# AtharvBhat/otters

Measured on AMD Instinct MI355X. Metric: GB/s scanned + queries/sec, exact cosine top-10 over 10M x 768 f32 rows per GPU, higher is better.
Workload: dtype f32; 1 GPU; 10000000x768 f32 VecStore per GPU, single query, Metric::Cosine, take(10); rows_per_gpu=10000000, dim=768, k=10, nq=1, processes=1

## Files before the change

bindings/rust/otters-hip-sys/src/lib.rs:

```rust
#![allow(non_camel_case_types)]

use std::os::raw::{c_char, c_int, c_void};

pub const OTT_ABI_VERSION: c_int = 4;
pub const OTT_COMM_ID_BYTES: usize = 128;
pub const OTT_GROUP_SIZE_MAX: u32 = 16;
pub const OTT_MAXSIM_BATCH_MAX: u32 = 4096;
pub const OTT_MMR_MAX_FETCH: u32 = 1024;
pub const OTT_RECOMMEND_MAX_EXAMPLES: u32 = 64;
pub const OTT_DISCOVER_MAX_PAIRS: u32 = 32;
pub const OTT_NO_ROW: u64 = u64::MAX;
pub const OTT_NO_MASK: u32 = 4294967295;
pub const OTT_MASK_SLOT_BASE: u32 = 2147483648;
pub const OTT_MASK_SLOTS: u32 = 64;
pub const OTT_MASKS_MAX_QUERIES: u32 = 1024;
pub const OTT_BOOST_MAX_TERMS: u32 = 8;
pub const OTT_BOOST_MAX_QUERIES: u32 = 1024;
pub const OTT_FUSE_MAX_LEGS: u32 = 16;
pub const OTT_FUSE_MAX_FETCH: u32 = 512;
pub const OTT_FUSE_MAX_ENTRIES: u32 = 8192;
pub const OTT_FUSE_MAX_REQUESTS: u32 = 1024;
pub const OTT_FUSE_RRF: u32 = 0;
pub const OTT_FUSE_DBSF: u32 = 1;
pub const OTT_FUSE_MINMAX: u32 = 2;
// ... 81 lines not shown
    pub vectors_compared: u64,
    pub prune_ns: u64,
    pub score_ns: u64,
    pub merge_ns: u64,
    pub total_ns: u64,
    pub bytes_scanned: u64,
    pub path_used: u32,
    pub passes: u32,
    pub rescored: u64,
    pub retries: u32,
    pub refined: u32,
    pub err_ratio_max: f32,
    pub gate_failed: u32,
    pub bound_violations: u32,
    pub i8_refined: u32,
    pub exchange_ns: u64,
}

#[repr(C)]
#[derive(Clone, Copy, Debug)]
pub struct ott_leaf {
    pub column: u32,
    pub op: u32,
    pub clause: u32,
    pub reserved: u32,
    pub lit_i64: i64,
    pub lit_f64: f64,
}

#[repr(C)]
#[derive(Clone, Copy, Debug)]
pub struct ott_boost_term {
    pub kind: u32,
    pub source: u32,
    pub weight: f32,
    pub scale: f32,
    pub origin: f64,
    pub missing: f32,
    pub reserved: u32,
}

#[repr(C)]
pub struct ott_store {
    _opaque: [u8; 0],
}

#[repr(C)]
pub struct ott_comm {
    _opaque: [u8; 0],
}

pub type ott_allgather_fn = Option<unsafe extern "C" fn(user: *mut c_void, send: *const c_void, recv: *mut c_void, bytes: u64) -> c_int>;

extern "C" {
    pub fn ott_abi_version() -> c_int;
    pub fn ott_last_error() -> *const c_char;
    pub fn ott_device_count(out: *mut c_int) -> c_int;

    pub fn ott_store_create(dim: u32, device: c_int, out: *mut *mut ott_store) -> c_int;
    pub fn ott_store_create_multi(dim: u32, n_dev: u32, dev_ids: *const c_int, out: *mut *mut ott_store) -> c_int;
    pub fn ott_multi_plan(n_rows: u64, chunk_size: u64, n_dev: u32, out_first_rows: *mut u64) -> c_int;
    pub fn ott_store_shard_count(s: *const ott_store) -> c_int;
    pub fn ott_store_shard_info(s: *const ott_store, shard: u32, device: *mut c_int, first_row: *mut u64, n_rows: *mut u64) -> c_int;
    pub fn ott_store_transport(s: *const ott_store) -> *const c_char;
    pub fn ott_store_destroy(s: *mut ott_store) -> c_int;
    pub fn ott_store_reserve(s: *mut ott_store, n_rows: u64) -> c_int;
    pub fn ott_store_append(s: *mut ott_store, rows_host: *const f32, n_rows: u64) -> c_int;
    pub fn ott_store_append_device(s: *mut ott_store, rows_dev: *const c_void, n_rows: u64) -> c_int;
    pub fn ott_store_append_random(s: *mut ott_store, n_rows: u64, seed: u64) -> c_int;
    pub fn ott_store_append_clustered(s: *mut ott_store, n_rows: u64, seed: u64, n_clusters: u32, spread: f32, aniso: f32) -> c_int;
    pub fn ott_store_write_rows(s: *mut ott_store, first_row: u64, rows_host: *const f32, n_rows: u64) -> c_int;
    pub fn ott_store_len(s: *const ott_store) -> u64;
    pub fn ott_store_delete_rows(s: *mut ott_store, rows_host: *const u64, n: u64, n_changed: *mut u64) -> c_int;
    pub fn ott_store_restore_rows(s: *mut ott_store, rows_host: *const u64, n: u64, n_changed: *mut u64) -> c_int;
    pub fn ott_store_live_len(s: *const ott_store) -> u64;
    pub fn ott_store_read_live_mask(s: *const ott_store, out_host: *mut u64) -> c_int;
    pub fn ott_store_compact(s: *mut ott_store, out_new_index: *mut u64) -> c_int;
    pub fn ott_store_dim(s: *const ott_store) -> u32;
    pub fn ott_store_device(s: *const ott_store) -> c_int;
    pub fn ott_store_set_chunk_size(s: *mut ott_store, chunk_size: u64) -> c_int;
    pub fn ott_store_set_batch_image(s: *mut ott_store, enabled: c_int) -> c_int;
    pub fn ott_store_prepare_batch(s: *mut ott_store) -> c_int;
    pub fn ott_store_batch_ready(s: *const ott_store) -> c_int;
    pub fn ott_store_set_option(s: *mut ott_store, name: *const c_char, value: i64) -> c_int;
    pub fn ott_store_set_base_offset(s: *mut ott_store, base: u64) -> c_int;
    pub fn ott_store_set_reduce_order(s: *mut ott_store, reduce: u32) -> c_int;
    pub fn ott_store_read_rows(s: *const ott_store, first_row: u64, n_rows: u64, out_host: *mut f32) -> c_int;
    pub fn ott_store_read_inv_norms(s: *const ott_store, first_row: u64, n_rows: u64, out_host: *mut f32) -> c_int;
    pub fn ott_store_add_column(s: *mut ott_store, dtype: u32, values_host: *const c_void, nulls: *const u64, n: u64, out_column_id: *mut u32) -> c_int;
    pub fn ott_store_zone_stats(s: *mut ott_store, column: u32, chunk_size: u64, out_min: *mut c_void, out_max: *mut c_void, out_non_null: *mut u64) -> c_int;
    pub fn ott_store_eval_row_mask(s: *mut ott_store, leaves: *const ott_leaf, n_leaves: u32, n_clauses: u32, out_host: *mut u64) -> c_int;

    pub fn ott_query(s: *mut ott_store, d: *const ott_query_desc, out: *mut ott_hit, cap: u64, n_out: *mut u64, n_per_query: *mut u64, stats: *mut ott_stats) -> c_int;
    pub fn ott_query_masks(s: *mut ott_store, d: *const ott_query_desc, masks: *const u64, n_masks: u32, mask_bits: u64, mask_of_query: *const c_void, out: *mut ott_hit, cap: u64, n_out: *mut u64, n_per_query: *mut u64, stats: *mut ott_stats) -> c_int;
    pub fn ott_store_eval_row_mask_slot(s: *mut ott_store, slot: u32, leaves: *const ott_leaf, n_leaves: u32, n_clauses: u32, out_host: *mut u64) -> c_int;
    pub fn ott_store_write_row_mask_slot(s: *mut ott_store, slot: u32, bits: *const u64, n_bits: u64) -> c_int;
    pub fn ott_store_clear_row_mask_slots(s: *mut ott_store) -> c_int;
    pub fn ott_query_boost(s: *mut ott_store, d: *const ott_query_desc, combine: u32, score_weight: f32, terms: *const c_void, n_terms: u32, out: *mut ott_hit, cap: u64, n_out: *mut u64, n_per_query: *mut u64, stats: *mut ott_stats) -> c_int;
    pub fn ott_query_ids(s: *mut ott_store, d: *const ott_query_desc, ids: *const u64, n_ids: u64, out: *mut ott_hit, cap: u64, n_out: *mut u64, n_per_query: *mut u64, stats: *mut ott_stats) -> c_int;
    pub fn ott_store_score_rows(s: *mut ott_store, queries: *const f32, nq: u32, metric: u32, ids: *const u64, n_ids: u64, out_scores: *mut f32) -> c_int;
    pub fn ott_query_fuse(s: *mut ott_store, d: *const ott_query_desc, legs_per_request: *const c_void, n_requests: u32, fusion: u32, rrf_k: f32, leg_weights: *const f32, fetch: u64, out: *mut ott_hit, cap: u64, n_out: *mut u64, n_per_request: *mut u64, stats: *mut ott_stats) -> c_int;
    pub fn ott_store_set_sparse(s: *mut ott_store, indptr: *const u64, indices: *const c_void, values: *const f32, n: u64, vocab: u32) -> c_int;
    pub fn ott_store_clear_sparse(s: *mut ott_store) -> c_int;
    pub fn ott_store_sparse_info(s: *const ott_store, vocab: *mut u32, nnz: *mut u64, padded_entries: *mut u64, bytes: *mut u64) -> c_int;
    pub fn ott_store_read_sparse(s: *const ott_store, first_row: u64, n_rows: u64, indptr_out: *mut u64, indices_out: *mut c_void, values_out: *mut f32, entry_cap: u64) -> c_int;
    pub fn ott_query_sparse(s: *mut ott_store, d: *const ott_query_desc, q_indptr: *const u64, q_indices: *const c_void, q_values: *const f32, out: *mut ott_hit, cap: u64, n_out: *mut u64, n_per_query: *mut u64, stats: *mut ott_stats) -> c_int;
    pub fn ott_query_mmr(s: *mut ott_store, d: *const ott_query_desc, ids: *const u64, n_ids: u64, fetch_k: u64, lambda: f32, out: *mut ott_hit, cap: u64, n_out: *mut u64, n_per_query: *mut u64, out_values: *mut f32, stats: *mut ott_stats) -> c_int;
    pub fn ott_query_recommend(s: *mut ott_store, d: *const ott_query_desc, positive: *const u64, n_positive: u64, negative: *const u64, n_negative: u64, flags: u32, out: *mut ott_hit, cap: u64, n_out: *mut u64, side_of_hit: *mut u32, stats: *mut ott_stats) -> c_int;
    pub fn ott_query_recommend_strategy(s: *mut ott_store, d: *const ott_query_desc, strategy: u32, positive: *const u64, n_positive: u64, negative: *const u64, n_negative: u64, flags: u32, out: *mut ott_hit, cap: u64, n_out: *mut u64, side_of_hit: *mut u32, stats: *mut ott_stats) -> c_int;
    pub fn ott_query_discover(s: *mut ott_store, d: *const ott_query_desc, target_row: u64, positive: *const u64, negative: *const u64, n_pairs: u64, min_wins: u32, flags: u32, out: *mut ott_hit, cap: u64, n_out: *mut u64, wins_of_hit: *mut u32, stats: *mut ott_stats) -> c_int;
    pub fn ott_store_set_groups(s: *mut ott_store, gid_host: *const c_void, n: u64, n_groups: u32) -> c_int;
    pub fn ott_store_clear_groups(s: *mut ott_store) -> c_int;
    pub fn ott_store_group_count(s: *const ott_store) -> u32;
    pub fn ott_query_groups(s: *mut ott_store, d: *const ott_query_desc, out: *mut ott_hit, cap: u64, n_out: *mut u64, n_per_query: *mut u64, stats: *mut ott_stats) -> c_int;
    pub fn ott_query_groups_top(s: *mut ott_store, d: *const ott_query_desc, group_size: u32, out: *mut ott_hit, cap: u64, n_out: *mut u64, n_per_query: *mut u64, group_of_hit: *mut u32, stats: *mut ott_stats) -> c_int;
    pub fn ott_query_maxsim(s: *mut ott_store, d: *const ott_query_desc, out: *mut ott_hit, cap: u64, n_out: *mut u64, stats: *mut ott_stats) -> c_int;
    pub fn ott_query_maxsim_groups(s: *mut ott_store, d: *const ott_query_desc, groups: *const c_void, n_groups_listed: u64, out: *mut ott_hit, cap: u64, n_out: *mut u64, stats: *mut ott_stats) -> c_int;
    pub fn ott_store_group_index_builds(s: *const ott_store) -> u64;
    pub fn ott_query_maxsim_groups_batch(s: *mut ott_store, d: *const ott_query_desc, tokens_per_query: *const c_void, listed_per_query: *const u64, n_queries: u32, groups: *const c_void, out: *mut ott_hit, cap: u64, n_out: *mut u64, n_per_query: *mut u64, stats: *mut ott_stats) -> c_int;
    pub fn ott_query_device(s: *mut ott_store, d: *const ott_query_desc, out_dev: *mut c_void, cap: u64, n_out_dev: *mut c_void, stats: *mut ott_stats) -> c_int;
    pub fn ott_store_sync(s: *mut ott_store) -> c_int;
    pub fn ott_store_stream(s: *mut ott_store) -> *mut c_void;
    pub fn ott_merge_hits_device(s: *mut ott_store, lists_dev: *const c_void, n_lists: u64, list_len: u64, take: u32, k: u64, out_host: *mut ott_hit, n_out: *mut u64) -> c_int;
    pub fn ott_merge_hits_device_grouped(s: *mut ott_store, lists_dev: *const c_void, n_lists: u64, n_groups: u64, list_len: u64, take: u32, k: u64, out_host: *mut ott_hit, n_out: *mut u64, n_per_group: *mut u64) -> c_int;

    pub fn ott_comm_unique_id(id_out: *mut c_void) -> c_int;
    pub fn ott_comm_create(unique_id: *const c_void, rank: c_int, world: c_int, device: c_int, out: *mut *mut ott_comm) -> c_int;
    pub fn ott_comm_create_host(rank: c_int, world: c_int, r#fn: ott_allgather_fn, user: *mut c_void, out: *mut *mut ott_comm) -> c_int;
    pub fn ott_comm_destroy(c: *mut ott_comm) -> c_int;
    pub fn ott_comm_rank(c: *const ott_comm) -> c_int;
    pub fn ott_comm_world(c: *const ott_comm) -> c_int;
    pub fn ott_comm_transport(c: *const ott_comm) -> *const c_char;
    pub fn ott_comm_info(c: *const ott_comm, nranks: *mut c_int, version: *mut c_int) -> c_int;
    pub fn ott_comm_set_timeout_ms(c: *mut ott_comm, timeout_ms: i64) -> c_int;
    pub fn ott_comm_all_gather_host(c: *mut ott_comm, send_host: *const c_void, recv_host: *mut c_void, bytes: u64) -> c_int;
    pub fn ott_query_sharded(s: *mut ott_store, c: *mut ott_comm, d: *const ott_query_desc, out: *mut ott_hit, cap: u64, n_out: *mut u64, n_per_query: *mut u64, stats: *mut ott_stats) -> c_int;
}

pub fn last_error() -> String {
    unsafe {
        let p = ott_last_error();
        if p.is_null() {
            String::new()
        } else {
            std::ffi::CStr::from_ptr(p).to_string_lossy().into_owned()
        }
    }
}

pub fn check(rc: c_int) -> Result<(), String> {
    if rc == OTT_OK {
        Ok(())
    } else {
        Err(last_error())
    }
}

const _: () = {
    assert!(std::mem::size_of::<ott_hit>() == 16);
    assert!(std::mem::size_of::<ott_query_desc>() == 72);
    assert!(std::mem::size_of::<ott_stats>() == 120);
    assert!(std::mem::size_of::<ott_leaf>() == 32);
    assert!(std::mem::size_of::<ott_boost_term>() == 32);
};

#[cfg(test)]
// ... 9 lines not shown
```

include/otters_hip.h:

```cpp
#ifndef OTTERS_HIP_H
#define OTTERS_HIP_H

#include <stddef.h>
#include <stdint.h>

#ifdef __cplusplus
extern "C" {
#endif

#define OTT_ABI_VERSION 4

typedef enum {
    OTT_OK = 0,
    OTT_ERR_INVALID = -1,
    OTT_ERR_HIP = -2,
    OTT_ERR_OOM = -3,
    OTT_ERR_UNSUPPORTED = -4
} ott_status;

typedef enum { OTT_METRIC_COSINE = 0, OTT_METRIC_EUCLIDEAN = 1, OTT_METRIC_DOT = 2, OTT_METRIC_MANHATTAN = 3 } ott_metric;
typedef enum { OTT_TAKE_MIN = 0, OTT_TAKE_MAX = 1 } ott_take;
typedef enum { OTT_CMP_NONE = 0, OTT_CMP_LT = 1, OTT_CMP_GT = 2, OTT_CMP_LTE = 3, OTT_CMP_GTE = 4, OTT_CMP_EQ = 5 } ott_cmp;
typedef enum { OTT_OP_EQ = 0, OTT_OP_NEQ = 1, OTT_OP_LT = 2, OTT_OP_LTE = 3, OTT_OP_GT = 4, OTT_OP_GTE = 5 } ott_op;
typedef enum { OTT_DT_INT32 = 0, OTT_DT_INT64 = 1, OTT_DT_FLOAT32 = 2, OTT_DT_FLOAT64 = 3, OTT_DT_DATETIME = 5 } ott_dtype;
// ... 2 lines not shown

typedef enum { OTT_PATH_AUTO = 0, OTT_PATH_EXACT = 1, OTT_PATH_MFMA = 2 } ott_path;

typedef enum { OTT_REDUCE_AVX = 0, OTT_REDUCE_SEQ4 = 1 } ott_reduce;

typedef struct {
    uint64_t index;
    float score;
    uint32_t query;
} ott_hit;

typedef struct {
    const float* queries;
    uint32_t nq;
    uint32_t metric;
    uint32_t take;
    uint32_t filter_cmp;
    float filter_thr;
    uint32_t mode;
    uint64_t k;
    const uint64_t* chunk_mask;
    const uint64_t* row_mask;
    uint64_t row_mask_bits;
    uint32_t use_device_row_mask;
    uint32_t path;
} ott_query_desc;

typedef struct {
    uint64_t total_chunks, pruned_chunks, evaluated_chunks, vectors_compared;
    uint64_t prune_ns, score_ns, merge_ns, total_ns;
    uint64_t bytes_scanned;
    uint32_t path_used;
    uint32_t passes;
    uint64_t rescored;
    uint32_t retries;
    uint32_t refined;
    float err_ratio_max;
    uint32_t gate_failed;
    uint32_t bound_violations;
    uint32_t i8_refined;
    uint64_t exchange_ns;
} ott_stats;

typedef struct {
    uint32_t column;
    uint32_t op;
    uint32_t clause;
    uint32_t reserved;
    int64_t lit_i64;
    double lit_f64;
} ott_leaf;

typedef struct ott_store ott_store;

int ott_abi_version(void);
const char* ott_last_error(void);
int ott_device_count(int* out);

int ott_store_create(uint32_t dim, int device, ott_store** out);
int ott_store_create_multi(uint32_t dim, uint32_t n_dev, const int* dev_ids, ott_store** out);
int ott_multi_plan(uint64_t n_rows, uint64_t chunk_size, uint32_t n_dev, uint64_t* out_first_rows);
int ott_store_shard_count(const ott_store* s);
int ott_store_shard_info(const ott_store* s, uint32_t shard, int* device, uint64_t* first_row, uint64_t* n_rows);
const char* ott_store_transport(const ott_store* s);
int ott_store_destroy(ott_store* s);
int ott_store_reserve(ott_store* s, uint64_t n_rows);
int ott_store_append(ott_store* s, const float* rows_host, uint64_t n_rows);
int ott_store_append_device(ott_store* s, const void* rows_dev, uint64_t n_rows);
int ott_store_append_random(ott_store* s, uint64_t n_rows, uint64_t seed);
int ott_store_append_clustered(ott_store* s, uint64_t n_rows, uint64_t seed, uint32_t n_clusters, float spread, float aniso);
int ott_store_write_rows(ott_store* s, uint64_t first_row, const float* rows_host, uint64_t n_rows);
uint64_t ott_store_len(const ott_store* s);
uint32_t ott_store_dim(const ott_store* s);
int ott_store_device(const ott_store* s);
int ott_store_delete_rows(ott_store* s, const uint64_t* rows_host, uint64_t n, uint64_t* n_changed);
int ott_store_restore_rows(ott_store* s, const uint64_t* rows_host, uint64_t n, uint64_t* n_changed);
uint64_t ott_store_live_len(const ott_store* s);
int ott_store_read_live_mask(const ott_store* s, uint64_t* out_host);
int ott_store_compact(ott_store* s, uint64_t* out_new_index);
int ott_store_set_chunk_size(ott_store* s, uint64_t chunk_size);
int ott_store_set_batch_image(ott_store* s, int enabled);
int ott_store_prepare_batch(ott_store* s);
int ott_store_batch_ready(const ott_store* s);

int ott_store_set_option(ott_store* s, const char* name, int64_t value);

int ott_store_set_base_offset(ott_store* s, uint64_t base);
int ott_store_set_reduce_order(ott_store* s, uint32_t reduce );
int ott_store_read_rows(const ott_store* s, uint64_t first_row, uint64_t n_rows, float* out_host);
int ott_store_read_inv_norms(const ott_store* s, uint64_t first_row, uint64_t n_rows, float* out_host);

int ott_store_add_column(ott_store* s, uint32_t dtype, const void* values_host, const uint64_t* nulls,
                         uint64_t n, uint32_t* out_column_id);
int ott_store_zone_stats(ott_store* s, uint32_t column, uint64_t chunk_size, void* out_min, void* out_max,
                         uint64_t* out_non_null);

int ott_store_eval_row_mask(ott_store* s, const ott_leaf* leaves, uint32_t n_leaves, uint32_t n_clauses,
                            uint64_t* out_host);

int ott_query(ott_store* s, const ott_query_desc* d, ott_hit* out, uint64_t cap, uint64_t* n_out,
              uint64_t* n_per_query, ott_stats* stats);

int ott_query_ids(ott_store* s, const ott_query_desc* d, const uint64_t* ids, uint64_t n_ids, ott_hit* out, uint64_t cap,
                  uint64_t* n_out, uint64_t* n_per_query, ott_stats* stats);
int ott_store_score_rows(ott_store* s, const float* queries, uint32_t nq, uint32_t metric, const uint64_t* ids, uint64_t n_ids,
                         float* out_scores);

#define OTT_NO_MASK 4294967295u
#define OTT_MASK_SLOT_BASE 2147483648u
#define OTT_MASK_SLOTS 64
#define OTT_MASKS_MAX_QUERIES 1024
int ott_query_masks(ott_store* s, const ott_query_desc* d, const uint64_t* masks, uint32_t n_masks, uint64_t mask_bits,
                    const void* mask_of_query , ott_hit* out, uint64_t cap, uint64_t* n_out, uint64_t* n_per_query,
                    ott_stats* stats);
int ott_store_eval_row_mask_slot(ott_store* s, uint32_t slot, const ott_leaf* leaves, uint32_t n_leaves, uint32_t n_clauses,
                                 uint64_t* out_host);
int ott_store_write_row_mask_slot(ott_store* s, uint32_t slot, const uint64_t* bits, uint64_t n_bits);
int ott_store_clear_row_mask_slots(ott_store* s);

#define OTT_BOOST_MAX_TERMS 8
#define OTT_BOOST_MAX_QUERIES 1024
typedef enum { OTT_BOOST_SUM = 0, OTT_BOOST_MULT = 1 } ott_boost_combine;
typedef enum { OTT_BOOST_VALUE = 0, OTT_BOOST_LIN_DECAY = 1, OTT_BOOST_MASK = 2 } ott_boost_kind;
typedef struct {
    uint32_t kind;
    uint32_t source;
    float    weight;
    float    scale;
    double   origin;
    float    missing;
    uint32_t reserved;
} ott_boost_term;
int ott_query_boost(ott_store* s, const ott_query_desc* d, uint32_t combine, float score_weight,
                    const void* terms , uint32_t n_terms,
                    ott_hit* out, uint64_t cap, uint64_t* n_out, uint64_t* n_per_query, ott_stats* stats);

typedef enum { OTT_FUSE_RRF = 0, OTT_FUSE_DBSF = 1, OTT_FUSE_MINMAX = 2 } ott_fusion;
#define OTT_FUSE_MAX_LEGS 16
#define OTT_FUSE_MAX_FETCH 512
#define OTT_FUSE_MAX_ENTRIES 8192
#define OTT_FUSE_MAX_REQUESTS 1024
int ott_query_fuse(ott_store* s, const ott_query_desc* d, const void* legs_per_request , uint32_t n_requests,
                   uint32_t fusion , float rrf_k, const float* leg_weights , uint64_t fetch,
                   ott_hit* out, uint64_t cap, uint64_t* n_out, uint64_t* n_per_request, ott_stats* stats);

#define OTT_MMR_MAX_FETCH 1024
int ott_query_mmr(ott_store* s, const ott_query_desc* d, const uint64_t* ids, uint64_t n_ids,
                  uint64_t fetch_k, float lambda, ott_hit* out, uint64_t cap, uint64_t* n_out, uint64_t* n_per_query,
                  float* out_values , ott_stats* stats);

#define OTT_RECOMMEND_MAX_EXAMPLES 64
#define OTT_RECOMMEND_FILL 1u
int ott_query_recommend(ott_store* s, const ott_query_desc* d, const uint64_t* positive, uint64_t n_positive, const uint64_t* negative,
                        uint64_t n_negative, uint32_t flags, ott_hit* out, uint64_t cap, uint64_t* n_out,
                        uint32_t* side_of_hit , ott_stats* stats);

typedef enum { OTT_RECOMMEND_BEST_SCORE = 0, OTT_RECOMMEND_AVERAGE_VECTOR = 1, OTT_RECOMMEND_SUM_SCORES = 2 } ott_recommend_strategy;
int ott_query_recommend_strategy(ott_store* s, const ott_query_desc* d, uint32_t strategy, const uint64_t* positive,
                                 uint64_t n_positive, const uint64_t* negative, uint64_t n_negative, uint32_t flags, ott_hit* out,
                                 uint64_t cap, uint64_t* n_out, uint32_t* side_of_hit , ott_stats* stats);

#define OTT_DISCOVER_MAX_PAIRS 32
#define OTT_NO_ROW UINT64_MAX
int ott_query_discover(ott_store* s, const ott_query_desc* d, uint64_t target_row, const uint64_t* positive, const uint64_t* negative,
                       uint64_t n_pairs, uint32_t min_wins, uint32_t flags, ott_hit* out, uint64_t cap, uint64_t* n_out,
                       uint32_t* wins_of_hit , ott_stats* stats);
// ... 68 lines not shown
```

otters_amd/_native.py:

```python
from __future__ import annotations

import ctypes as C
import os
import subprocess

import numpy as np

_CSRC = os.path.join(os.path.dirname(os.path.abspath(__file__)), "csrc")
LIB_PATH = os.environ.get("OTT_LIB_PATH") or os.path.join(_CSRC, "libotters_hip.so")


class OttersError(Exception):
    """Error type of the host layer: str(e) is the reference's `Err(String)` payload."""


class Hit(C.Structure):
    _fields_ = [("index", C.c_uint64), ("score", C.c_float), ("query", C.c_uint32)]


HIT_DTYPE = np.dtype([("index", "<u8"), ("score", "<f4"), ("query", "<u4")])


class QueryDesc(C.Structure):
    _fields_ = [
# ... 42 lines not shown
FUSE_MAX_LEGS = 16
FUSE_MAX_FETCH = 512
FUSE_MAX_ENTRIES = 8192
FUSE_MAX_REQUESTS = 1024
FUSE_RRF, FUSE_DBSF, FUSE_MINMAX = 0, 1, 2
SPARSE_MAX_VOCAB = 1 << 20
SPARSE_MAX_QUERIES = 1024

_lib = None


def build(force: bool = False) -> str:
    srcs = [os.path.join(_CSRC, f) for f in os.listdir(_CSRC) if f.endswith((".hip", ".h", ".inc"))]
    srcs.append(os.path.join(_CSRC, "..", "..", "include", "otters_hip.h"))
    stale = not os.path.exists(LIB_PATH) or any(os.path.getmtime(s) > os.path.getmtime(LIB_PATH) for s in srcs)
    if force or stale:
        subprocess.check_call(["make", "-C", _CSRC, "-j", "8", "-s"])
    return LIB_PATH


def _preload_torch_hip() -> None:
    try:
        import importlib.util
        spec = importlib.util.find_spec("torch")
        if spec is None or not spec.submodule_search_locations:
            return
        libdir = os.path.join(list(spec.submodule_search_locations)[0], "lib")
        cand = os.path.join(libdir, "libamdhip64.so")
        if os.path.exists(cand):
            C.CDLL(cand, mode=C.RTLD_GLOBAL)
    except Exception:
        pass


def preload_torch_rccl() -> None:
    try:
        import torch
    except Exception:
        pass


def lib() -> C.CDLL:
    global _lib
    if _lib is not None:
        return _lib
    if not os.path.exists(LIB_PATH):
        raise OttersError(
            f"libotters_hip.so not found at {LIB_PATH}: build it with `python -c 'import __graft_entry__ as g; g.build()'` "
            "(there is no CPU fallback)")
    _preload_torch_hip()
    L = C.CDLL(LIB_PATH)
    vp, u64, u32, i32 = C.c_void_p, C.c_uint64, C.c_uint32, C.c_int
    sig = {
        "ott_abi_version": (i32, []),
        "ott_last_error": (C.c_char_p, []),
        "ott_device_count": (i32, [vp]),
        "ott_store_create": (i32, [u32, i32, vp]),
        "ott_store_create_multi": (i32, [u32, u32, vp, vp]),
        "ott_multi_plan": (i32, [u64, u64, u32, vp]),
        "ott_store_shard_count": (i32, [vp]),
        "ott_store_shard_info": (i32, [vp, u32, vp, vp, vp]),
        "ott_store_transport": (C.c_char_p, [vp]),
        "ott_store_destroy": (i32, [vp]),
        "ott_store_reserve": (i32, [vp, u64]),
        "ott_store_append": (i32, [vp, vp, u64]),
        "ott_store_append_device": (i32, [vp, vp, u64]),
        "ott_store_append_random": (i32, [vp, u64, u64]),
        "ott_store_append_clustered": (i32, [vp, u64, u64, u32, C.c_float, C.c_float]),
        "ott_store_write_rows": (i32, [vp, u64, vp, u64]),
        "ott_store_delete_rows": (i32, [vp, vp, u64, vp]),
        "ott_store_restore_rows": (i32, [vp, vp, u64, vp]),
        "ott_store_live_len": (u64, [vp]),
        "ott_store_read_live_mask": (i32, [vp, vp]),
        "ott_store_compact": (i32, [vp, vp]),
        "ott_store_len": (u64, [vp]),
        "ott_store_dim": (u32, [vp]),
        "ott_store_device": (i32, [vp]),
        "ott_store_set_chunk_size": (i32, [vp, u64]),
        "ott_store_set_base_offset": (i32, [vp, u64]),
        "ott_store_set_reduce_order": (i32, [vp, u32]),
        "ott_store_set_batch_image": (i32, [vp, i32]),
        "ott_store_prepare_batch": (i32, [vp]),
        "ott_store_batch_ready": (i32, [vp]),
        "ott_store_read_rows": (i32, [vp, u64, u64, vp]),
        "ott_store_read_inv_norms": (i32, [vp, u64, u64, vp]),
        "ott_store_add_column": (i32, [vp, u32, vp, vp, u64, vp]),
        "ott_store_eval_row_mask": (i32, [vp, vp, u32, u32, vp]),
        "ott_store_zone_stats": (i32, [vp, u32, u64, vp, vp, vp]),
        "ott_query": (i32, [vp, vp, vp, u64, vp, vp, vp]),
        "ott_query_ids": (i32, [vp, vp, vp, u64, vp, u64, vp, vp, vp]),
        "ott_store_score_rows": (i32, [vp, vp, u32, u32, vp, u64, vp]),
        "ott_query_masks": (i32, [vp, vp, vp, u32, u64, vp, vp, u64, vp, vp, vp]),
        "ott_store_eval_row_mask_slot": (i32, [vp, u32, vp, u32, u32, vp]),
        "ott_store_write_row_mask_slot": (i32, [vp, u32, vp, u64]),
        "ott_store_clear_row_mask_slots": (i32, [vp]),
        "ott_query_boost": (i32, [vp, vp, u32, C.c_float, vp, u32, vp, u64, vp, vp, vp]),
        "ott_query_fuse": (i32, [vp, vp, vp, u32, u32, C.c_float, vp, u64, vp, u64, vp, vp, vp]),
        "ott_query_mmr": (i32, [vp, vp, vp, u64, u64, C.c_float, vp, u64, vp, vp, vp, vp]),
        "ott_query_recommend": (i32, [vp, vp, vp, u64, vp, u64, u32, vp, u64, vp, vp, vp]),
        "ott_query_recommend_strategy": (i32, [vp, vp, u32, vp, u64, vp, u64, u32, vp, u64, vp, vp, vp]),
        "ott_query_discover": (i32, [vp, vp, u64, vp, vp, u64, u32, u32, vp, u64, vp, vp, vp]),
        "ott_store_set_groups": (i32, [vp, vp, u64, u32]),
        "ott_store_clear_groups": (i32, [vp]),
        "ott_store_group_count": (u32, [vp]),
        "ott_query_groups": (i32, [vp, vp, vp, u64, vp, vp, vp]),
        "ott_query_groups_top": (i32, [vp, vp, u32, vp, u64, vp, vp, vp, vp]),
        "ott_query_maxsim": (i32, [vp, vp, vp, u64, vp, vp]),
        "ott_query_maxsim_groups": (i32, [vp, vp, vp, u64, vp, u64, vp, vp]),
        "ott_store_group_index_builds": (u64, [vp]),
        "ott_query_maxsim_groups_batch": (i32, [vp, vp, vp, vp, u32, vp, vp, u64, vp, vp, vp]),
        "ott_query_device": (i32, [vp, vp, vp, u64, vp, vp]),
        "ott_store_sync": (i32, [vp]),
        "ott_store_stream": (vp, [vp]),
        "ott_merge_hits_device": (i32, [vp, vp, u64, u64, u32, u64, vp, vp]),
        "ott_merge_hits_device_grouped": (i32, [vp, vp, u64, u64, u64, u32, u64, vp, vp, vp]),
        "ott_store_set_option": (i32, [vp, C.c_char_p, C.c_int64]),
        "ott_comm_unique_id": (i32, [vp]),
        "ott_comm_create": (i32, [vp, i32, i32, i32, vp]),
        "ott_comm_create_host": (i32, [i32, i32, ALLGATHER_FN, vp, vp]),
        "ott_comm_destroy": (i32, [vp]),
        "ott_comm_rank": (i32, [vp]),
        "ott_comm_world": (i32, [vp]),
        "ott_comm_transport": (C.c_char_p, [vp]),
        "ott_comm_info": (i32, [vp, vp, vp]),
        "ott_comm_set_timeout_ms": (i32, [vp, C.c_int64]),
        "ott_comm_all_gather_host": (i32, [vp, vp, vp, u64]),
        "ott_query_sharded": (i32, [vp, vp, vp, vp, u64, vp, vp, vp]),
        "ott_store_set_sparse": (i32, [vp, vp, vp, vp, u64, u32]),
        "ott_store_clear_sparse": (i32, [vp]),
        "ott_store_sparse_info": (i32, [vp, vp, vp, vp, vp]),
        "ott_store_read_sparse": (i32, [vp, u64, u64, vp, vp, vp, u64]),
        "ott_query_sparse": (i32, [vp, vp, vp, vp, vp, vp, u64, vp, vp, vp]),
    }
    for name, (res, args) in sig.items():
        fn = getattr(L, name)
        fn.restype = res
        fn.argtypes = args
    if L.ott_abi_version() != ABI_VERSION:
        raise OttersError("libotters_hip.so ABI version mismatch")
    _lib = L
    return L


def check(rc: int) -> None:
    if rc != 0:
        msg = lib().ott_last_error()
        err = OttersError(msg.decode("utf-8", "replace") if msg else f"libotters_hip error {rc}")
        err.status = int(rc)
        raise err


def ptr(a):
    return None if a is None else a.ctypes.data_as(C.c_void_p)


def pack_bits(bools) -> np.ndarray:
    b = np.ascontiguousarray(bools, dtype=bool).ravel()
    n = b.size
    nwords = max((n + 63) // 64, 1)
    buf = np.zeros(nwords * 8, dtype=np.uint8)
    if n:
        by = np.packbits(b, bitorder="little")
        buf[: by.size] = by
    return buf.view("<u8")


# ... 3 lines not shown
```

otters_amd/csrc/ott_api.hip:

```cpp
#include <math.h>
#include <string.h>

#include <algorithm>

#include "ott_internal.h"
#include "ott_prune.h"

using namespace ott;

namespace ott {

float host_inv_norm_exact(const float* v, uint32_t dim) {
    volatile float s = 0.0f;
    for (uint32_t i = 0; i < dim; i++) {
        volatile float sq = v[i] * v[i];
        s = s + sq;
    }
    float norm = sqrtf(s);
    return norm != 0.0f ? 1.0f / norm : 0.0f;
}

std::vector<uint32_t> tile_prefix(const RunPlan& pl, uint32_t tile_rows) {
    std::vector<uint32_t> pre;
    pre.push_back(0);
    uint64_t tiles = 0;
    for (const auto& r : pl.runs) {
        tiles += (r.count + tile_rows - 1) / tile_rows;
        pre.push_back((uint32_t)tiles);
    }
    return pre;
}

}


namespace ott {

int upload_exact_inputs(ott_store* s, const float* queries, uint32_t nq, const RunPlan& pl, const std::vector<uint32_t>& prefix) {
    const uint32_t nq_pad = (nq + 7u) & ~7u;
    const size_t q_bytes = (size_t)nq_pad * s->dimq * 4, qi_bytes = (size_t)nq_pad * 4;
    const size_t run_bytes = pl.runs.size() * sizeof(ott_run), pre_bytes = prefix.size() * 4;
    size_t off_q = 0, off_qi = off_q + q_bytes, off_run = (off_qi + qi_bytes + 15) & ~(size_t)15;
    size_t off_pre = off_run + run_bytes, total = off_pre + pre_bytes;
    int rc = s->h_stage.ensure(total);
    if (rc) return rc;
    char* hs = (char*)s->h_stage.p;
    float* hq = (float*)(hs + off_q);
    memset(hq, 0, q_bytes + qi_bytes);
    for (uint32_t i = 0; queries != nullptr && i < nq; i++) {
        memcpy(hq + (size_t)i * s->dimq, queries + (size_t)i * s->dim, (size_t)s->dim * 4);
        ((float*)(hs + off_qi))[i] = host_inv_norm_exact(queries + (size_t)i * s->dim, s->dim);
    }
    memcpy(hs + off_run, pl.runs.data(), run_bytes);
    memcpy(hs + off_pre, prefix.data(), pre_bytes);
    if ((rc = s->d_queries.ensure(total))) return rc;
    OTT_HIP(hipMemcpyAsync(s->d_queries.p, hs, total, hipMemcpyHostToDevice, s->stream));
    s->in_off_qinv = off_qi;
    s->in_off_runs = off_run;
    s->in_off_prefix = off_pre;
    return OTT_OK;
}

void fill_exact_params(ott_store* s, const ott_query_desc* d, const RunPlan& pl, uint32_t nq, const uint64_t* d_mask, uint64_t mask_bits,
                       uint32_t n_tiles, ExactParams& p) {
    memset(&p, 0, sizeof(p));
    p.rows = s->d_rows;
    p.inv = s->d_inv;
    p.queries = (const float*)s->d_queries.p;
    p.qinv = (const float*)((const char*)s->d_queries.p + s->in_off_qinv);
    p.row_mask = d_mask;
    p.row_mask_bits = mask_bits;
    p.runs = (const ott_run*)((const char*)s->d_queries.p + s->in_off_runs);
    p.tile_prefix = (const uint32_t*)((const char*)s->d_queries.p + s->in_off_prefix);
    p.ld = s->ld;
    p.dim = s->dim;
    p.dimq = s->dimq;
    p.n_runs = (uint32_t)pl.runs.size();
    p.n_tiles = n_tiles;
    p.nq_total = nq;
    p.metric = d->metric;
    p.take_max = d->take == OTT_TAKE_MAX;
    p.cmp = d->filter_cmp;
    p.thr = d->filter_thr;
    p.reduce = s->reduce;
    p.tie_sh = s->cur_tie_sh;
    p.tie_off = s->cur_tie_off;
    p.flat = s->cur_flat ? 1u : 0u;
}

// ... 31 lines not shown
        if (keep) {
            const uint64_t start = c * cs;
            const uint64_t len = (n - start) < cs ? (n - start) : cs;
            if (open) pl.runs.back().count += len;
            else pl.runs.push_back({start, len});
            open = true;
            pl.evaluated++;
            pl.rows_scored += len;
        } else {
            open = false;
        }
    }
}

}

namespace ott {
void make_run_plan(const ott_store* s, const uint64_t* chunk_mask, RunPlan& pl) { build_plan(s, chunk_mask, pl); }

int check_desc_enums(const char* who, const ott_query_desc* d) {
    const auto unknown = [who](const char* what) { return fail(OTT_ERR_INVALID, std::string(who) + ": unknown " + what); };
    if (d->metric > OTT_METRIC_MANHATTAN) return unknown("metric");
    if (d->take > OTT_TAKE_MAX) return unknown("take type");
    if (d->filter_cmp > OTT_CMP_EQ) return unknown("filter comparator");
    if (d->mode > OTT_MODE_PER_QUERY) return unknown("mode");
    if (d->path > OTT_PATH_MFMA) return unknown("path");
    return OTT_OK;
}

int check_device_row_mask(const char* who, const ott_store* s, const ott_query_desc* d) {
    if (d->use_device_row_mask && s->evalmask_bits == 0 && s->n)
        return fail(OTT_ERR_INVALID, std::string(who) + ": use_device_row_mask set but ott_store_eval_row_mask was not called");
    return OTT_OK;
}

int validate_query(const ott_store* s, const ott_query_desc* d) {
    int rc;
    if (!s) return fail(OTT_ERR_INVALID, "ott_query: store is NULL");
    if (!d) return fail(OTT_ERR_INVALID, "ott_query: desc is NULL");
    if (d->nq == 0) return fail(OTT_ERR_INVALID, "No queries provided");
    if (!d->queries) return fail(OTT_ERR_INVALID, "ott_query: queries is NULL");
    if ((rc = check_desc_enums("ott_query", d))) return rc;
    if (d->path == OTT_PATH_MFMA && d->metric == OTT_METRIC_MANHATTAN)
        return fail(OTT_ERR_UNSUPPORTED, "ott_query: the MFMA path does not score the Manhattan metric; use path AUTO or EXACT");
    return check_device_row_mask("ott_query", s, d);
}

void read_exact_events(ott_store* s, ott_stats* st) {
    float ms = 0.f;
    if (hipEventElapsedTime(&ms, s->ev[3], s->ev[4]) == hipSuccess) st->score_ns = (uint64_t)(ms * 1e6);
    if (hipEventElapsedTime(&ms, s->ev[4], s->ev[5]) == hipSuccess) st->merge_ns = (uint64_t)(ms * 1e6);
}
}

namespace {

__global__ void sum_counts_kernel(const uint64_t* counts, uint32_t n, uint64_t* out) {
    uint64_t t = 0;
    for (uint32_t i = threadIdx.x; i < n; i += 64) t += counts[i];
    for (int o = 32; o > 0; o >>= 1) t += __shfl_xor(t, o);
    if (threadIdx.x == 0) *out = t;
}

struct ExactCtx {
    ott_store* s;
    const float* queries;
    uint32_t nq;
    const ott_query_desc* d;
    bool perq;
    const RunPlan& pl;
    uint64_t k_eff;
    bool fetch, timing;
    const std::vector<uint32_t>& prefix;
    ExactPlan x;
    uint32_t groups;
    PrunePlan prune{0, false, 0};
    RunPlan plA, plB;
    std::vector<uint32_t> preA, preB;
    int gridA = 0, gridB = 0;
    double qt = 0.0, qn = 0.0, q1 = 0.0;
    PruneQuant qq{0, 0.0f, 0.0f, 0.0, 0};
    bool head = false;
    bool seed_est = false;
    ExactResult res{0, 0, 0};
    uint64_t* d_counts = nullptr;
    ott_hit* d_hits = nullptr;
    ExactParams p;
};

void plan_pruned_sweep(ExactCtx& c) {
    ott_store* s = c.s;
    const PruneIn in{s->dim, s->ld, c.d->metric, c.perq, c.x.lean, s->cur_flat, c.x.variant, s->opt.exact_prune, s->opt.exact_sketch,
                     SketchState{s->d_sketch != nullptr, s->sk_n >= s->n, s->sk_bits, s->sk_words, s->sk_stage0}, c.pl.rows_scored, c.x.E};
    PrunePlan pp = prune_plan(in);
    bool quant_ok = false;
    if (prune_plan_needs_quant(in, pp) && !(quant_ok = prune_query_quant(c.queries, s->dim, pp.c * 32, &c.qq))) pp = prune_plan_quant_refused(in);
    if (!pp.c) return;
#ifdef OTT_SK4_DECODE_F32
    const bool head = false;
#else
    const bool head = prune_plan_head(in, pp, quant_ok, HeadState{s->d_head != nullptr, s->head_n >= s->n, s->opt.exact_sketch_head});
#endif
    const uint32_t m = head ? 0u : pp.c * 32;
    if (head) (void)prune_query_quant(c.queries, s->dim, 0, &c.qq);
    const uint64_t est_rows = prune_plan_seed_est(in, pp, head, c.d->filter_cmp != OTT_CMP_NONE);
    split_plan(c.pl, est_rows ? est_rows : pp.seed, c.plA, c.plB);
    const bool two_runs_each = c.plA.runs.size() <= 2 && c.plB.runs.size() <= 2 && c.plB.rows_scored > 0;
    if (!two_runs_each || !prune_query_bounds(c.queries, s->dim, m, &c.qt, &c.qn)) return;
    c.prune = pp;
    c.head = head;
    c.seed_est = est_rows != 0;
    if (c.seed_est) c.plB = c.pl;
    c.q1 = prune_query_l1(c.queries, s->dim, m);
    c.preA = tile_prefix(c.plA, 64);
    c.preB = tile_prefix(c.plB, 64);
    c.gridA = exact_grid(s, c.preA.back());
    c.gridB = exact_grid(s, c.preB.back());
}

int ensure_exact_result(ExactCtx& c) {
    ott_store* s = c.s;
    int rc;
    if (!c.x.lean && (rc = upload_exact_inputs(s, c.queries, c.nq, c.pl, c.prefix))) return rc;
    const size_t n_lists_total = exact_n_lists(c.x, c.nq, c.perq, c.prune.c != 0, c.gridA, c.gridB);
    if ((rc = s->d_lists.ensure(n_lists_total * c.x.KS * sizeof(Cand)))) return rc;
    c.res = exact_result_layout(c.groups, c.x.KS);
    char* res_dev = nullptr;
    if (c.fetch) {
        if ((rc = s->h_hits.ensure(c.res.host_bytes))) return rc;
        void* mapped = nullptr;
        OTT_HIP(hipHostGetDevicePointer(&mapped, s->h_hits.p, 0));
        res_dev = (char*)mapped;
    } else {
        if ((rc = s->d_hits.ensure(c.res.bytes))) return rc;
        res_dev = (char*)s->d_hits.p;
    }
    c.d_counts = (uint64_t*)res_dev;
    c.d_hits = (ott_hit*)(res_dev + c.res.cnt_pad);
    return OTT_OK;
}

void fill_exact_call(ExactCtx& c, const uint64_t* d_mask, uint64_t mask_bits) {
    ott_store* s = c.s;
    fill_exact_params(s, c.d, c.pl, c.nq, d_mask, mask_bits, c.prefix.back(), c.p);
    c.p.k = (uint32_t)c.k_eff;
    c.p.perq = c.perq;
    c.p.list_stride = c.x.KS;
    c.p.small = c.x.variant;
    if (c.x.lean) embed_exact_inputs(c.p, c.queries, (size_t)s->dim * 4, host_inv_norm_exact(c.queries, s->dim), c.pl, c.prefix);
}

ExactParams part_params(const ExactCtx& c, const RunPlan& sub, const std::vector<uint32_t>& pre, Cand* dst) {
    ExactParams q = c.p;
    q.n_runs = (uint32_t)sub.runs.size();
    q.n_tiles = pre.back();
    embed_exact_inputs(q, c.queries, (size_t)c.s->dim * 4, c.p.eqinv, sub, pre);
    q.lists = dst;
    return q;
}

int pruned_sweep(ExactCtx& c) {
    ott_store* s = c.s;
    const uint32_t KS = c.x.KS;
    int rc;
    if ((rc = s->d_prune.ensure(64 + (size_t)KS * sizeof(ott_hit)))) return rc;
    uint64_t* seed_res = (uint64_t*)s->d_prune.p;
    unsigned long long* tails_dev = nullptr;
    if (c.fetch) {
        if (!s->d_tails.p) {
            if ((rc = s->d_tails.ensure(8))) return rc;
            OTT_HIP(hipMemsetAsync(s->d_tails.p, 0, 8, s->stream));
            s->tails_seen = 0;
        }
        tails_dev = (unsigned long long*)s->d_tails.p;
    }
    ExactParams pa = part_params(c, c.plA, c.preA, (Cand*)s->d_lists.p);
    auto sketch_inputs = [&](ExactParams& q) {
        q.prune_stage = c.prune.c;
        q.prune_qt = c.qt;
        q.prune_qn = c.qn;
        if (!c.prune.sketch) return;
        q.prune_sketch = s->d_sketch;
        q.sk_pitch = s->sk_pitch;
        q.sk_stage0 = s->sk_stage0;
        q.sk_bits = s->sk_bits;
        q.prune_q1 = c.q1;
        q.prune_qe1 = c.qq.qe1;
        q.prune_qscale = c.qq.scale;
        q.prune_qinv_scale = c.qq.inv_scale;
        q.prune_qsum = c.qq.qsum;
        if (c.head) {
            q.prune_head_codes = reinterpret_cast<const uint32_t*>(s->d_head);
            q.prune_head_rho = reinterpret_cast<const float*>(s->d_head + s->cap * (size_t)16);
        }
    };
    if (c.seed_est) {
        sketch_inputs(pa);
        pa.seed_est = 1;
        pa.seed_keep = prune_seed_keep(c.k_eff);
    }
    if ((rc = launch_exact(s, pa, 1, c.x.E, c.gridA))) return rc;
    if ((rc = launch_merge(s, (const Cand*)s->d_lists.p, (uint32_t)c.gridA, KS, 0, 1, (uint32_t)c.k_eff, c.x.E, c.p.take_max != 0, tie_base(s),
                           (ott_hit*)(seed_res + 8), KS, seed_res, s->cur_tie_sh)))
        return rc;
    ExactParams pb = part_params(c, c.plB, c.preB, (Cand*)s->d_lists.p + (size_t)c.gridA * KS);
    sketch_inputs(pb);
    pb.prune_seed = seed_res;
    pb.prune_tails = tails_dev;
    return launch_exact(s, pb, 1, c.x.E, c.gridB);
}

int plain_passes(ExactCtx& c) {
    ott_store* s = c.s;
    const uint32_t tile = c.x.tile;
    int rc;
    for (uint32_t ps = 0; ps < c.x.passes; ps++) {
        c.p.q0 = ps * tile;
        c.p.lists = (Cand*)s->d_lists.p + ((c.perq && tile > 1) ? 0 : (size_t)ps * c.x.grid * c.x.KS);
        if ((rc = launch_exact(s, c.p, (int)tile, c.x.E, c.x.grid))) return rc;
    }
    return OTT_OK;
}

int merge_exact(ExactCtx& c) {
    ott_store* s = c.s;
    const uint32_t KS = c.x.KS, grid = (uint32_t)c.x.grid;
    if (c.seed_est)
        return launch_merge(s, (const Cand*)s->d_lists.p + (size_t)c.gridA * KS, (uint32_t)c.gridB, KS, 0, c.groups, (uint32_t)c.k_eff, c.x.E,
                            c.p.take_max != 0, tie_base(s), c.d_hits, KS, c.d_counts, s->cur_tie_sh);
    const uint32_t n_lists = c.perq ? grid : (uint32_t)exact_n_lists(c.x, c.nq, false, c.prune.c != 0, c.gridA, c.gridB);
    return launch_merge(s, (const Cand*)s->d_lists.p, n_lists, KS, c.perq ? (uint64_t)grid * KS : 0, c.groups, (uint32_t)c.k_eff, c.x.E,
                        c.p.take_max != 0, tie_base(s), c.d_hits, KS, c.d_counts, s->cur_tie_sh);
}

int fetch_exact(ExactCtx& c, std::vector<std::vector<ott_hit>>& lists, ott_stats& st) {
    ott_store* s = c.s;
    const uint32_t KS = c.x.KS;
    char* hh = (char*)s->h_hits.p;
    if (c.prune.c) OTT_HIP(hipMemcpyAsync(hh + c.res.bytes, s->d_tails.p, 8, hipMemcpyDeviceToHost, s->stream));
    OTT_HIP(hipStreamSynchronize(s->stream));
    if (c.prune.c) {
        uint64_t total;
        memcpy(&total, hh + c.res.bytes, 8);
        st.rescored += total - s->tails_seen;
        s->tails_seen = total;
    }
    const uint64_t* counts = (const uint64_t*)hh;
    const ott_hit* hits = (const ott_hit*)(hh + c.res.cnt_pad);
    lists.assign(c.groups, {});
    for (uint32_t g = 0; g < c.groups; g++) lists[g].assign(hits + (size_t)g * KS, hits + (size_t)g * KS + counts[g]);
    float ms = 0.f;
    if (c.timing && hipEventElapsedTime(&ms, s->ev[3], s->ev[4]) == hipSuccess) st.score_ns += (uint64_t)(ms * 1e6);
    if (c.timing && hipEventElapsedTime(&ms, s->ev[4], s->ev[5]) == hipSuccess) st.merge_ns += (uint64_t)(ms * 1e6);
    return OTT_OK;
}

int run_exact(ott_store* s, const float* queries, uint32_t nq, const ott_query_desc* d, bool perq, const RunPlan& pl, uint64_t k_eff,
              const uint64_t* d_mask, uint64_t mask_bits, bool fetch, std::vector<std::vector<ott_hit>>& lists, ott_stats& st,
              bool timing = true, ott_hit* hits_dev_direct = nullptr, uint32_t direct_stride = 0) {
    switch (lists_or_sort(k_eff, nq, pl.rows_scored, s->opt.large_k_from, fetch)) {
        case EXACT_REFUSED: return fail(OTT_ERR_UNSUPPORTED, "ott_query_device: k > 512 is host-output only");
        case EXACT_SORT: return run_large_k(s, queries, nq, d, perq, pl, k_eff, d_mask, mask_bits, lists, st);
        case EXACT_LISTS: break;
    }
    const std::vector<uint32_t> prefix = tile_prefix(pl, 64);
    ExactCtx c{s, queries, nq, d, perq, pl, k_eff, fetch, timing, prefix,
               exact_plan(k_eff, nq, perq, s->dimq, prefix.back(), pl.runs.size(), s->opt.exact_small, exact_grid(s, prefix.back())), perq ? nq : 1u};
    plan_pruned_sweep(c);
    int rc;
    if ((rc = ensure_exact_result(c))) return rc;
    if (!fetch && hits_dev_direct != nullptr && direct_stride == c.x.KS) c.d_hits = hits_dev_direct;
    fill_exact_call(c, d_mask, mask_bits);

    if (timing) OTT_HIP(hipEventRecord(s->ev[3], s->stream));
    if ((rc = c.prune.c ? pruned_sweep(c) : plain_passes(c))) return rc;
    if (timing) OTT_HIP(hipEventRecord(s->ev[4], s->stream));
    if ((rc = merge_exact(c))) return rc;
    if (timing) OTT_HIP(hipEventRecord(s->ev[5], s->stream));
    st.passes += c.x.passes;
    st.bytes_scanned += exact_bytes_scanned(c.x.passes, pl.rows_scored, s->dim, d->metric);
    return fetch ? fetch_exact(c, lists, st) : OTT_OK;
}

}

int ott::compose_row_mask(ott_store* s, const ott_query_desc* d, const uint64_t** d_mask_out, uint64_t* mask_bits_out) {
    int rc;
    const uint64_t* d_mask = nullptr;
    uint64_t mask_bits = 0;
    if (d->use_device_row_mask) {
        d_mask = (const uint64_t*)s->d_evalmask.p;
        mask_bits = s->evalmask_bits;
    } else if (d->row_mask && d->row_mask_bits) {
        const size_t words = (size_t)((d->row_mask_bits + 63) / 64);
        if ((rc = s->d_rowmask.ensure(words * 8))) return rc;
        OTT_HIP(hipMemcpyAsync(s->d_rowmask.p, d->row_mask, words * 8, hipMemcpyHostToDevice, s->stream));
        d_mask = (const uint64_t*)s->d_rowmask.p;
        mask_bits = d->row_mask_bits;
    }
    if (s->cur_idmask) {
        if (d_mask) {
            uint64_t* both = s->cur_idmask + (s->n + 63) / 64;
            if ((rc = mask_and(s, s->cur_idmask, d_mask, mask_bits, s->n, both))) return rc;
            d_mask = both;
        } else {
            d_mask = s->cur_idmask;
        }
        mask_bits = s->n;
    }
    if (s->cur_qmask && (rc = masks_join(s, &d_mask, &mask_bits))) return rc;
    if (s->n_dead && (rc = live_compose(s, &d_mask, &mask_bits))) return rc;
    *d_mask_out = d_mask;
    *mask_bits_out = mask_bits;
    return OTT_OK;
}

int ott::query_on(ott_store* s, const ott_query_desc* d, ott_hit* out_host, void* out_dev, uint64_t cap, uint64_t* n_out,
                  uint64_t* n_per_query, void* n_out_dev, ott_stats* stats_out, bool nosync, bool* events_pending) {
    CoreOpts co;
    if (s->opt.tie_order != 0) {
        if (out_host && !out_dev) {
            if (events_pending) *events_pending = false;
            return query_ref_ties(s, d, out_host, cap, n_out, n_per_query, stats_out);
        }
        co.tie_sh = 3;
    }
    return query_core(s, d, out_host, out_dev, cap, n_out, n_per_query, n_out_dev, stats_out, nosync, events_pending, co);
}
// ... 483 lines not shown
```

otters_amd/csrc/ott_exact.hip:

```cpp
#include <atomic>

#include "ott_internal.h"
#include "ott_prune.h"
#include "ott_exact_dev.h"

namespace ott {

constexpr int KC = 32;
constexpr int WAVES = 4;
constexpr int STAGE_FLOATS = 64 * KC;
constexpr int EXACT_SMEM = WAVES * STAGE_FLOATS * 4;
constexpr int DUMP_QCAP = 128;
constexpr int EXACT_SMEM_DUMP = EXACT_SMEM + WAVES * DUMP_QCAP * 12;
constexpr int PQ_CAP = 128;
constexpr int PQ_WORDS = 10;
constexpr int QD_WORDS = (int)(OTT_QEMB_MAX / KC) * 12;
constexpr int EXACT_SMEM_PRUNE = EXACT_SMEM + WAVES * PQ_CAP * PQ_WORDS * 4 + QD_WORDS * 4;
#ifdef OTT_SK4_DECODE_F32
constexpr bool SK4_INT = false;
#else
constexpr bool SK4_INT = true;
#endif
constexpr int SK_MAXW = (int)OTT_SKETCH1_MAX_WORDS;
constexpr int SK3_MAXST = (int)OTT_SKETCH_MAX_WORDS / 3;
constexpr int SK3_XP = ((int)OTT_SKETCH_MAX_WORDS + 2 + 3) / 4 - 8;
#ifndef OTT_X_BLOCKS_PER_CU
#define OTT_X_BLOCKS_PER_CU 2
#endif
constexpr int BLOCKS_PER_CU = OTT_X_BLOCKS_PER_CU;
constexpr int SMALL_RING = 8;
constexpr uint32_t SMALL_QMAX = 2048;
[[maybe_unused]] constexpr int EXACT_SMEM_SMALL = SMALL_RING * STAGE_FLOATS * 4 + SMALL_QMAX * 4;

__device__ __forceinline__ void exact_glds16(const char* sbase, uint32_t voff, uint32_t lds_addr) {
    uint32_t keep;
    lds_addr = (uint32_t)__builtin_amdgcn_readfirstlane((int)lds_addr);
    asm volatile(
        "s_nop 4\n\t"
        "s_mov_b32 %0, m0\n\t"
        "s_mov_b32 m0, %3\n\t"
        "s_nop 0\n\t"
        "global_load_lds_dwordx4 %1, %2\n\t"
        "s_mov_b32 m0, %0"
        : "=&s"(keep)
        : "v"(voff), "s"(sbase), "s"(lds_addr)
        : "memory");
}


template <int MK, int NQ, int E, bool PERQ, bool DUMP = false, bool SMALL = false, bool BLK = (E > 1), bool I8 = false, bool PRUNE = false, int SK = 0, bool SEED = false>
__global__ __launch_bounds__(SMALL ? 64 : 256) void exact_kernel(ExactParams p) {
    static_assert(!I8 || (NQ == 1 && MK == MK_DOT && !PERQ && !DUMP && !SMALL), "the int8 sweep takes one query, cosine / dot, merged");
    static_assert(!PRUNE || (NQ == 1 && MK == MK_DOT && !PERQ && !DUMP && !SMALL && !I8), "the pruned sweep takes one query, cosine / dot, merged");
    static_assert((SK == 0 || PRUNE) && (SK == 0 || SK == 1 || SK == 3 || SK == 4 || SK == 5), "the sketch is the pruned sweep's: none, one, three or four bits per dim (5: four with a head)");
    constexpr bool HD = SK == 5;
    constexpr bool SK4 = SK == 4 || SK == 5;
    static_assert(!HD || SK4_INT, "the head form decodes by integer dot products only");
    static_assert(!SEED || (HD && E == 1), "the estimate pass is the head form's, one list entry per lane");
    extern __shared__ __attribute__((aligned(16))) float smem[];
    const int lane = threadIdx.x & 63;
    const int wave = __builtin_amdgcn_readfirstlane(threadIdx.x >> 6);
    constexpr int BW = SMALL ? 1 : WAVES;
    float* st = SMALL ? smem : smem + wave * STAGE_FLOATS;
    float* sQ = smem + SMALL_RING * STAGE_FLOATS;
    constexpr int NL = PERQ ? NQ : 1;
    constexpr int KS = 64 * E;

    WaveList<E> L[NL];
    uint64_t tk[NL];
    uint32_t tq[NL];
    bool fresh[NL];
#pragma unroll
    for (int i = 0; i < NL; i++) {
        wl_init(L[i]);
        tk[i] = 0;
        tq[i] = 0xFFFFFFFFu;
        fresh[i] = true;
    }

    const bool take_max = p.take_max != 0;
    const uint32_t nq_here = (p.nq_total - p.q0) < (uint32_t)NQ ? (p.nq_total - p.q0) : (uint32_t)NQ;
    typedef __attribute__((address_space(4))) const float* CF32;
    typedef __attribute__((address_space(4))) const uint32_t* CU32;
    typedef __attribute__((address_space(4))) const ott_run* CRUN;
    typedef __attribute__((address_space(4))) const char* CCH;
    const CCH karg = (CCH)__builtin_amdgcn_kernarg_segment_ptr();
    const CF32 Q = p.embedded ? (CF32)(karg + __builtin_offsetof(ExactParams, qemb)) : (CF32)(p.queries + (size_t)p.q0 * p.dimq);
    const CU32 tile_prefix = p.embedded ? (CU32)(karg + __builtin_offsetof(ExactParams, eprefix)) : (CU32)p.tile_prefix;
    const CRUN runs = p.embedded ? (CRUN)(karg + __builtin_offsetof(ExactParams, eruns)) : (CRUN)p.runs;
    float qinv[NQ];
#pragma unroll
    for (int q = 0; q < NQ; q++) qinv[q] = (uint32_t)q < nq_here ? (p.embedded ? p.eqinv : p.qinv[p.q0 + q]) : 0.0f;
    uint32_t dgate[NQ];
#pragma unroll
    for (int q = 0; q < NQ; q++) dgate[q] = (DUMP && p.dump_gate != nullptr && (uint32_t)q < nq_here) ? p.dump_gate[p.q0 + q] : 0u;
    uint64_t* dq_key = reinterpret_cast<uint64_t*>(smem + WAVES * STAGE_FLOATS) + wave * DUMP_QCAP;
    uint32_t* dq_q = reinterpret_cast<uint32_t*>(smem + WAVES * STAGE_FLOATS + WAVES * DUMP_QCAP * 2) + wave * DUMP_QCAP;
    uint32_t dqn = 0;
    auto dq_flush = [&]() {
        if (dqn == 0) return;
        wave_sync();
        unsigned long long base = 0;
        if (lane == 0) base = atomicAdd(p.dump_cursor, (unsigned long long)dqn);
        base = rl64(base, 0);
        for (uint32_t i = lane; i < dqn; i += 64) {
            const uint64_t at = base + i;
            if (at < p.dump_cap) {
                p.dump_keys[at] = dq_key[i];
                p.dump_q[at] = dq_q[i];
            }
        }
        wave_sync();
        dqn = 0;
    };

    if constexpr (SMALL) {
        for (uint32_t i = threadIdx.x; i < p.dimq; i += 64 * BW) sQ[i] = Q[i];
        __syncthreads();
    }
    const uint32_t gw = blockIdx.x * BW + wave, nw = gridDim.x * BW;
    const int sw = (lane >> 1) & 7;
    const uint32_t nstages = (p.ld + KC - 1) / KC;
    [[maybe_unused]] uint32_t* qd = reinterpret_cast<uint32_t*>(smem + WAVES * STAGE_FLOATS + WAVES * PQ_CAP * PQ_WORDS);
    if constexpr (SK4 && SK4_INT) {
        const uint32_t nqs = nstages < (uint32_t)(QD_WORDS / 12) ? nstages : (uint32_t)(QD_WORDS / 12);
        for (uint32_t i = threadIdx.x; i < nqs * 4; i += 64 * BW) {
            float q8[8];
#pragma unroll
            for (int j = 0; j < 8; j++) q8[j] = (8 * i + j < p.dim) ? Q[8 * i + j] : 0.0f;
            uint32_t d3[3];
            prune_quant_word(q8, p.prune_qinv_scale, d3);
#pragma unroll
            for (int d = 0; d < 3; d++) qd[(i >> 2) * 12 + d * 4 + (i & 3)] = d3[d];
        }
        __syncthreads();
    }
    const int lrow = lane >> 3;
    const int lslot = lane & 7;
    const uint32_t lsl4 = ((uint32_t)lslot * 4 < p.ld) ? (uint32_t)lslot * 4 : 0u;

    const uint32_t pstage = HD ? 0u : p.prune_stage;
    const uint32_t s_end = PRUNE ? pstage : nstages;
    uint32_t theta = 0;
    if constexpr (PRUNE && !SEED) {
        if (p.prune_seed[0] >= p.k) theta = ord_of(reinterpret_cast<const ott_hit*>(p.prune_seed + 8)[p.k - 1].score, take_max);
    }
    float* pq = smem + WAVES * STAGE_FLOATS + wave * (PQ_CAP * PQ_WORDS);
    uint32_t* pq_row = reinterpret_cast<uint32_t*>(pq + 9 * PQ_CAP);
    uint32_t pq_head = 0, pq_n = 0;
    uint32_t tails_done = 0;
    auto pq_finish = [&](uint32_t n) {
        wave_sync();
        const bool valid = (uint32_t)lane < n;
        const uint32_t e = (pq_head + (valid ? (uint32_t)lane : 0u)) & (PQ_CAP - 1);
        float acc[8];
#pragma unroll
        for (int l = 0; l < 8; l++) acc[l] = pq[l * PQ_CAP + e];
        const float vinv = pq[8 * PQ_CAP + e];
        const uint32_t my_row = pq_row[e];
        float tail = 0.0f;
        const float* rp[8];
        bool rok[8];
#pragma unroll
        for (int m = 0; m < 8; m++) {
            const uint32_t i = 8 * m + lrow;
            rok[m] = i < n;
            rp[m] = p.rows + (uint64_t)pq_row[(pq_head + (rok[m] ? i : 0u)) & (PQ_CAP - 1)] * p.ld + lsl4;
        }
        v4f R[8];
        auto load_stage = [&](uint32_t s) {
            const uint32_t soff = (s * KC + lslot * 4 < p.ld) ? s * KC : 0u;
#pragma unroll
            for (int m = 0; m < 8; m++) R[m] = __builtin_nontemporal_load(reinterpret_cast<const v4f*>(rp[m] + soff));
        };
        load_stage(pstage);
        for (uint32_t s = pstage; s < nstages; s++) {
            const bool cok = s * KC + lslot * 4 < p.ld;
#pragma unroll
            for (int m = 0; m < 8; m++) {
                const int row = 8 * m + lrow;
                const bool ok = rok[m] & cok;
                const v4f v = R[m];
                *reinterpret_cast<float4*>(st + row * KC + ((lslot ^ ((row >> 1) & 7)) << 2)) =
                    make_float4(ok ? v.x : 0.f, ok ? v.y : 0.f, ok ? v.z : 0.f, ok ? v.w : 0.f);
            }
            wave_sync();
            if (s + 1 < nstages) load_stage(s + 1);
#pragma unroll
            for (int j = 0; j < KC / 8; j++) {
                const uint32_t col = s * KC + 8 * j;
                if (col < p.dim) {
                    const float4 a = *reinterpret_cast<const float4*>(st + lane * KC + (((2 * j) ^ sw) << 2));
                    const float4 b = *reinterpret_cast<const float4*>(st + lane * KC + (((2 * j + 1) ^ sw) << 2));
                    const float x[8] = {a.x, a.y, a.z, a.w, b.x, b.y, b.z, b.w};
                    if (col + 8 <= p.dim) {
#pragma unroll
                        for (int l = 0; l < 8; l++) acc[l] = __fadd_rn(acc[l], exact_term<MK>(Q[col + l], x[l]));
                    } else {
                        const uint32_t nt = p.dim - col;
#pragma unroll
                        for (int l = 0; l < 7; l++)
                            if ((uint32_t)l < nt) tail = __fadd_rn(tail, exact_term<MK>(Q[col + l], x[l]));
                    }
                }
            }
            wave_sync();
        }
        float sc = __fadd_rn(reduce8(acc, p.reduce), tail);
        if (p.metric == OTT_METRIC_COSINE) sc = __fmul_rn(__fmul_rn(sc, qinv[0]), vinv);
        const bool pass = valid && !(sc != sc) && cmp_holds(sc, p.cmp, p.thr);
        const uint64_t key = ((uint64_t)ord_of(sc, take_max) << 32) | (uint32_t)(~(my_row + p.tie_off));
        if (fresh[0]) {
            wl_fill_sorted(L[0], tk[0], tq[0], p.k, pass, key, p.q0, lane, p.tie_sh);
            fresh[0] = false;
        } else if constexpr (!BLK) {
            wl_offer(L[0], tk[0], tq[0], p.k, pass, key, p.q0, lane, p.tie_sh);
        } else {
            wl_offer_block(L[0], tk[0], tq[0], p.k, pass, key, p.q0, lane, p.tie_sh);
        }
        pq_head = (pq_head + n) & (PQ_CAP - 1);
        pq_n -= n;
        tails_done += n;
    };

    if constexpr (HD) {
        typedef uint32_t v4u __attribute__((ext_vector_type(4)));
        const uint32_t np = p.sk_pitch >> 2;
        auto locate = [&](uint32_t t, uint64_t& row0, uint32_t& cnt, uint64_t& vm) {
            uint32_t lo = 0, hi = p.n_runs;
            while (hi - lo > 1) {
                uint32_t mid = (lo + hi) >> 1;
                if (tile_prefix[mid] <= t) lo = mid;
                else hi = mid;
            }
            const uint64_t rs = runs[lo].start, rc = runs[lo].count;
            const uint64_t off = (uint64_t)(t - tile_prefix[lo]) * 64;
            row0 = rs + off;
            cnt = (rc - off) < 64 ? (uint32_t)(rc - off) : 64u;
            const uint64_t r = row0 + lane;
            bool valid = (uint32_t)lane < cnt;
            if (p.row_mask != nullptr && valid && r < p.row_mask_bits) valid = (p.row_mask[r >> 6] >> (r & 63)) & 1;
            vm = __ballot(valid);
        };
        auto next_tile = [&](uint32_t t, uint64_t& row0, uint32_t& cnt, uint64_t& vm) -> uint32_t {
            for (; t < p.n_tiles; t += nw) {
                locate(t, row0, cnt, vm);
                if (vm != 0) break;
            }
            return t;
        };
        v4f R[8];
        v4u hc = {0u, 0u, 0u, 0u};
        float hrho = __builtin_inff(), hinv = 0.0f;
        auto load_line = [&](uint64_t row0, uint32_t cnt, uint32_t f) {
            const uint32_t pc = (8 * f + (uint32_t)lslot < np) ? 8 * f + (uint32_t)lslot : np - 1;
            const uint32_t* lb = p.prune_sketch + row0 * (uint64_t)p.sk_pitch + 4 * pc;
#pragma unroll
            for (int m = 0; m < 8; m++) {
                const uint32_t row = 8 * m + lrow;
                R[m] = __builtin_nontemporal_load(reinterpret_cast<const v4f*>(lb + (row < cnt ? row : cnt - 1) * p.sk_pitch));
            }
        };
        auto load_head = [&](uint64_t row0, uint32_t cnt) {
            const uint64_t r = row0 + ((uint32_t)lane < cnt ? (uint32_t)lane : cnt - 1);
            hc = __builtin_nontemporal_load(reinterpret_cast<const v4u*>(p.prune_head_codes) + r);
            hrho = __builtin_nontemporal_load(p.prune_head_rho + r);
            hinv = __builtin_nontemporal_load(p.inv + r);
        };
        uint64_t row0 = 0, vm = 0;
        uint32_t cnt = 0;
        uint32_t t = next_tile(gw, row0, cnt, vm);
        bool pf = false;
        while (t < p.n_tiles) {
            uint32_t gate = theta;
            const uint32_t own = (uint32_t)(tk[0] >> 32);
            if (own > gate) gate = own;
            const uint64_t my_row = row0 + lane;
            const bool valid = (vm >> lane) & 1;
            uint64_t row0n = 0, vmn = 0;
            uint32_t cntn = 0;
            const uint32_t tn = next_tile(t + nw, row0n, cntn, vmn);
            bool keep = valid;
            float vinv = 0.0f;
            if (SEED || gate != 0) {
                if (!pf) {
                    load_line(row0, cnt, 0);
                    load_head(row0, cnt);
                }
                const v4u c0 = hc;
                const float rho_all = hrho;
                vinv = hinv;
                pf = false;
                int K0 = 0, K1 = 0, K2 = 0;
                float sk_a = 0.0f;
                for (uint32_t f = 0; 8 * f < np; f++) {
#pragma unroll
                    for (int m = 0; m < 8; m++) {
                        const int row = 8 * m + lrow;
                        const v4f v = R[m];
                        *reinterpret_cast<float4*>(st + row * KC + ((lslot ^ ((row >> 1) & 7)) << 2)) = make_float4(v.x, v.y, v.z, v.w);
                    }
                    wave_sync();
                    if (8 * (f + 1) < np) {
                        load_line(row0, cnt, f + 1);
                    } else if (tn < p.n_tiles) {
                        load_line(row0n, cntn, 0);
                        load_head(row0n, cntn);
                        pf = true;
                    }
                    for (uint32_t j = 0; j < 8 && 8 * f + j < np; j++) {
                        const float4 w4 = *reinterpret_cast<const float4*>(st + lane * KC + (((int)j ^ sw) << 2));
                        const uint32_t piece = 8 * f + j;
                        if (piece == 0) {
                            sk_a = w4.x;
                            continue;
                        }
                        const uint32_t sj = p.sk_stage0 + piece - 1u;
                        if (sj < nstages) {
                            const uint32_t w[4] = {__float_as_uint(w4.x), __float_as_uint(w4.y), __float_as_uint(w4.z), __float_as_uint(w4.w)};
                            const v4u* dp = reinterpret_cast<const v4u*>(qd + sj * 12);
                            const v4u d0 = dp[0], d1 = dp[1], d2 = dp[2];
#pragma unroll
                            for (int i = 0; i < 4; i++) {
                                K0 = __builtin_amdgcn_sdot8((int)w[i], (int)d0[i], K0, false);
                                K1 = __builtin_amdgcn_sdot8((int)w[i], (int)d1[i], K1, false);
                                K2 = __builtin_amdgcn_sdot8((int)w[i], (int)d2[i], K2, false);
                            }
                        }
                    }
                    wave_sync();
                }
                {
                    const v4u* dp = reinterpret_cast<const v4u*>(qd);
                    const v4u d0 = dp[0], d1 = dp[1], d2 = dp[2];
#pragma unroll
                    for (int i = 0; i < 4; i++) {
                        K0 = __builtin_amdgcn_sdot8((int)c0[i], (int)d0[i], K0, false);
                        K1 = __builtin_amdgcn_sdot8((int)c0[i], (int)d1[i], K1, false);
                        K2 = __builtin_amdgcn_sdot8((int)c0[i], (int)d2[i], K2, false);
                    }
                }
                if constexpr (SEED) {
                    const int K = 2 * (256 * K2 + 16 * K1 + K0) + p.prune_qsum;
                    const float est = prune_score_est_sketchq(vinv, sk_a, rho_all, K, p.prune_qscale, qinv[0], p.metric == OTT_METRIC_COSINE);
                    const bool offer = valid && est - est == 0.0f;
                    const uint64_t key = ((uint64_t)ord_of(est, take_max) << 32) | (uint32_t)(~(uint32_t)my_row);
                    if (fresh[0]) {
                        wl_fill_sorted(L[0], tk[0], tq[0], p.seed_keep, offer, key, p.q0, lane, 0u);
                        fresh[0] = false;
                    } else {
                        wl_offer(L[0], tk[0], tq[0], p.seed_keep, offer, key, p.q0, lane, 0u);
                    }
                    keep = false;
                } else if (valid) {
                    const float zero[8] = {0.f, 0.f, 0.f, 0.f, 0.f, 0.f, 0.f, 0.f};
                    const int K = 2 * (256 * K2 + 16 * K1 + K0) + p.prune_qsum;
                    const float b = prune_score_bound_sketchq(zero, vinv, sk_a, rho_all, K, p.prune_qscale, p.dim, p.prune_qt, p.prune_qe1, p.prune_qn, qinv[0],
                                                              p.metric == OTT_METRIC_COSINE, take_max);
                    keep = !(b == b && ord_of(b, take_max) < gate);
                }
            } else if (valid) {
                vinv = p.inv[my_row];
            }
            const uint64_t km = SEED ? 0ull : __ballot(keep);
            if (!SEED && keep) {
                const uint32_t at = (pq_head + pq_n + (uint32_t)__popcll(km & ((1ull << lane) - 1ull))) & (PQ_CAP - 1);
#pragma unroll
                for (int l = 0; l < 8; l++) pq[l * PQ_CAP + at] = 0.0f;
                pq[8 * PQ_CAP + at] = vinv;
                pq_row[at] = (uint32_t)my_row;
            }
            pq_n += (uint32_t)__popcll(km);
            if (!SEED && pq_n >= 64) {
                pq_finish(64);
                if (pf) {
                    load_line(row0n, cntn, 0);
                    load_head(row0n, cntn);
                }
            }
            t = tn;
            row0 = row0n;
            cnt = cntn;
            vm = vmn;
        }
        if constexpr (SEED) {
            const bool have = (uint32_t)lane < p.seed_keep && L[0].key[0] != 0ull;
            const uint64_t hm = __ballot(have);
            if (have) {
                const uint32_t r = ~(uint32_t)L[0].key[0];
                const uint32_t at = (uint32_t)__popcll(hm & ((1ull << lane) - 1ull));
#pragma unroll
                for (int l = 0; l < 8; l++) pq[l * PQ_CAP + at] = 0.0f;
                pq[8 * PQ_CAP + at] = p.inv[r];
                pq_row[at] = r;
            }
            pq_n = (uint32_t)__popcll(hm);
            wl_init(L[0]);
            tk[0] = 0;
            tq[0] = 0xFFFFFFFFu;
            fresh[0] = true;
        }
    } else
    for (uint32_t t = gw; t < p.n_tiles; t += nw) {
        uint32_t lo = 0, hi = p.n_runs;
        while (hi - lo > 1) {
            uint32_t mid = (lo + hi) >> 1;
            if (tile_prefix[mid] <= t) lo = mid;
            else hi = mid;
        }
        ott_run run;
        run.start = runs[lo].start;
        run.count = runs[lo].count;
        const uint64_t off = (uint64_t)(t - tile_prefix[lo]) * 64;
        const uint64_t row0 = run.start + off;
        const uint32_t cnt = (run.count - off) < 64 ? (uint32_t)(run.count - off) : 64u;
        const uint64_t my_row = row0 + lane;
        bool valid = (uint32_t)lane < cnt;
        if (p.row_mask != nullptr && valid && my_row < p.row_mask_bits)
            valid = (p.row_mask[my_row >> 6] >> (my_row & 63)) & 1;
        if (__ballot(valid) == 0) continue;

        float vinv = 0.0f;
        if ((PRUNE || p.metric == OTT_METRIC_COSINE) && valid) vinv = p.inv[my_row];
        float vsq = 0.0f;
        typedef uint32_t v4u __attribute__((ext_vector_type(4)));
        [[maybe_unused]] uint32_t skl[2 + SK_MAXW];
        [[maybe_unused]] uint32_t gate3 = 0;
        if constexpr (SK >= 3) {
            gate3 = theta;
            const uint32_t own = (uint32_t)(tk[0] >> 32);
            if (own > gate3) gate3 = own;
        }
        if constexpr (SK == 1) {
#pragma unroll
            for (int i = 0; i < 2 + SK_MAXW; i++) skl[i] = 0u;
            skl[1] = 0x7F800000u;
            if (valid) {
                const v4u* sp = reinterpret_cast<const v4u*>(p.prune_sketch + my_row * (uint64_t)p.sk_pitch);
                const v4u l0 = __builtin_nontemporal_load(sp);
                v4u l1 = {0u, 0u, 0u, 0u}, l2 = {0u, 0u, 0u, 0u};
                if (p.sk_pitch > 4) l1 = __builtin_nontemporal_load(sp + 1);
                if (p.sk_pitch > 8) l2 = __builtin_nontemporal_load(sp + 2);
                skl[0] = l0.x; skl[1] = l0.y; skl[2] = l0.z; skl[3] = l0.w;
                skl[4] = l1.x; skl[5] = l1.y; skl[6] = l1.z; skl[7] = l1.w;
                skl[8] = l2.x; skl[9] = l2.y; skl[10] = l2.z; skl[11] = l2.w;
            }
        }
        float i8_rf = 0.0f;
        bool i8_forced = false;
        if constexpr (I8) {
            if (valid) {
                i8_rf = ((p.metric == OTT_METRIC_COSINE ? vinv : 1.0f) * p.i8_scale[my_row]) * p.i8_qscale;
                i8_forced = (p.flag[my_row] & 5u) != 0;
            }
        }
        int iacc[2] = {0, 0};
        float acc[NQ][8];
// ... 264 lines not shown
            } else if constexpr (SK == 1) {
                if (gate != 0) {
                    float D = 0.0f;
#pragma unroll
                    for (int j = 0; j < SK_MAXW; j++) {
                        const uint32_t sj = p.sk_stage0 + (uint32_t)j;
                        if (sj >= p.prune_stage && sj < nstages) {
                            const uint32_t w = skl[2 + j];
#pragma unroll
                            for (int b = 0; b < 32; b++) {
                                const float sg = __uint_as_float(((w << (31 - b)) & 0x80000000u) | 0x3F800000u);
                                D = fmaf(sg, Q[sj * KC + b], D);
                            }
                        }
                    }
                    if (valid) {
                        const float b = prune_score_bound_sketch(acc[0], vinv, __uint_as_float(skl[0]), __uint_as_float(skl[1]), D, p.prune_stage * KC,
                                                                 p.dim, p.prune_qt, p.prune_q1, p.prune_qn, qinv[0], p.metric == OTT_METRIC_COSINE, take_max);
                        keep = !(b == b && ord_of(b, take_max) < gate);
                    }
                }
            } else if (valid && gate != 0) {
                const float b = prune_score_bound(acc[0], vsq, vinv, p.prune_stage * KC, p.dim, p.prune_qt, p.prune_qn, qinv[0],
                                                  p.metric == OTT_METRIC_COSINE, take_max);
                keep = !(b == b && ord_of(b, take_max) < gate);
            }
            const uint64_t km = __ballot(keep);
            if (keep) {
                const uint32_t at = (pq_head + pq_n + (uint32_t)__popcll(km & ((1ull << lane) - 1ull))) & (PQ_CAP - 1);
#pragma unroll
                for (int l = 0; l < 8; l++) pq[l * PQ_CAP + at] = acc[0][l];
                pq[8 * PQ_CAP + at] = vinv;
                pq_row[at] = (uint32_t)my_row;
            }
            pq_n += (uint32_t)__popcll(km);
            if (pq_n >= 64) pq_finish(64);
            continue;
        }

#pragma unroll
        for (int q = 0; q < NQ; q++) {
            if ((uint32_t)q < nq_here) {
                float s = __fadd_rn(reduce8(acc[q], p.reduce), tail[q]);
                if (p.metric == OTT_METRIC_COSINE) s = __fmul_rn(__fmul_rn(s, qinv[q]), vinv);
                bool pass = valid && !(s != s) && cmp_holds(s, p.cmp, p.thr);
                if constexpr (I8) {
                    s = (float)(iacc[0] + iacc[1]) * i8_rf;
                    pass = valid && !(s != s) && cmp_holds(s, p.cmp, p.thr);
                    if (i8_forced) {
                        s = take_max ? __builtin_inff() : -__builtin_inff();
                        pass = valid;
                    }
                }
                const uint64_t key = ((uint64_t)ord_of(p.flat ? 0.0f : s, take_max) << 32) | (uint32_t)(~((uint32_t)my_row + p.tie_off));
                if (DUMP) {
                    const bool keep = pass && (uint32_t)(key >> 32) >= dgate[q];
                    const uint64_t m = __ballot(keep);
                    if (m) {
                        const uint32_t c = (uint32_t)__popcll(m);
                        if (dqn + c > DUMP_QCAP) dq_flush();
                        if (keep) {
                            const uint32_t at = dqn + (uint32_t)__popcll(m & ((1ull << lane) - 1ull));
                            dq_key[at] = key;
                            dq_q[at] = p.q0 + q;
                        }
                        dqn += c;
                    }
                } else {
                    constexpr int li_max = NL - 1;
                    const int li = PERQ ? q : 0;
                    const int lx = li <= li_max ? li : 0;
                    if (fresh[lx]) {
                        wl_fill_sorted(L[lx], tk[lx], tq[lx], p.k, pass, key, p.q0 + q, lane, p.tie_sh);
                        fresh[lx] = false;
                        continue;
                    }
                    if constexpr (!BLK) wl_offer(L[lx], tk[lx], tq[lx], p.k, pass, key, p.q0 + q, lane, p.tie_sh);
                    else wl_offer_block(L[lx], tk[lx], tq[lx], p.k, pass, key, p.q0 + q, lane, p.tie_sh);
                }
            }
        }
    }

    if constexpr (PRUNE) {
        if (pq_n) pq_finish(pq_n);
        if (p.prune_tails != nullptr && tails_done != 0 && lane == 0) atomicAdd(p.prune_tails, (unsigned long long)tails_done);
    }
    if (DUMP) {
        dq_flush();
        return;
    }
    Cand* sl = reinterpret_cast<Cand*>(smem);
#pragma unroll
    for (int i = 0; i < NL; i++) {
        __syncthreads();
        if (wave > 0) {
#pragma unroll
            for (int e = 0; e < E; e++) {
                Cand c;
                c.key = L[i].key[e];
                c.q = L[i].q[e];
                c.pad = 0;
                sl[(wave - 1) * KS + e * 64 + lane] = c;
            }
        }
        __syncthreads();
        if (wave == 0) {
            for (int w = 0; w < BW - 1; w++) {
#pragma unroll
                for (int e = 0; e < E; e++) {
                    const uint32_t ppos = e * 64 + lane;
                    const Cand c = sl[w * KS + ppos];
                    const bool real = ppos < p.k && c.key != 0;
                    if constexpr (!BLK) {
                        wl_offer(L[i], tk[i], tq[i], p.k, real, c.key, c.q, lane, p.tie_sh);
                    } else {
                        const bool pass = real && before(c.key, c.q, tk[i], tq[i], p.tie_sh);
                        if (__popcll(__ballot(pass)) < WL_BLOCK_MIN) {
                            wl_offer(L[i], tk[i], tq[i], p.k, pass, c.key, c.q, lane, p.tie_sh);
                        } else {
                            wl_merge_sorted(L[i], real ? c.key : 0ull, real ? c.q : 0xFFFFFFFFu, lane, p.tie_sh);
                            wl_tau(L[i], p.k, tk[i], tq[i]);
                        }
                    }
                }
            }
            Cand* dst;
            if (PERQ) dst = p.lists + ((size_t)(p.q0 + i) * gridDim.x + blockIdx.x) * p.list_stride;
            else dst = p.lists + (size_t)blockIdx.x * p.list_stride;
            if (!PERQ || (uint32_t)i < nq_here) {
#pragma unroll
                for (int e = 0; e < E; e++) {
                    Cand c;
                    c.key = L[i].key[e];
                    c.q = L[i].q[e];
                    c.pad = 0;
                    dst[e * 64 + lane] = c;
                }
            }
        }
    }
}

constexpr int R8_WAVES = 8;
constexpr int R8_UNROLL = 12;
constexpr int R8_SMEM_MAX = (8 * (int)SMALL_QMAX + 8 * 64 + 64) * 4;

template <int MK, int E, int NQ, bool PERQ>
__global__ __launch_bounds__(64 * R8_WAVES) void exact_rows8_kernel(ExactParams p) {
    extern __shared__ __attribute__((aligned(16))) float smem[];
    float* sQ = smem;
    float* sS = smem + (size_t)NQ * p.dimq;
    uint32_t* sV = reinterpret_cast<uint32_t*>(sS + NQ * 64);
    const int lane = threadIdx.x & 63;
    const int wave = __builtin_amdgcn_readfirstlane(threadIdx.x >> 6);
    const int grp = lane >> 3, c = lane & 7;
    typedef __attribute__((address_space(4))) const float* CF32;
    typedef __attribute__((address_space(4))) const uint32_t* CU32;
    typedef __attribute__((address_space(4))) const ott_run* CRUN;
    typedef __attribute__((address_space(4))) const char* CCH;
    const CCH karg = (CCH)__builtin_amdgcn_kernarg_segment_ptr();
    const CF32 Q = p.embedded ? (CF32)(karg + __builtin_offsetof(ExactParams, qemb)) : (CF32)(p.queries + (size_t)p.q0 * p.dimq);
    const CU32 tile_prefix = p.embedded ? (CU32)(karg + __builtin_offsetof(ExactParams, eprefix)) : (CU32)p.tile_prefix;
    const CRUN runs = p.embedded ? (CRUN)(karg + __builtin_offsetof(ExactParams, eruns)) : (CRUN)p.runs;
    const uint32_t nq_here = (p.nq_total - p.q0) < (uint32_t)NQ ? (p.nq_total - p.q0) : (uint32_t)NQ;
    float qinv[NQ];
#pragma unroll
// ... 587 lines not shown
            s_ctl[3] = 0;
        }
        __syncthreads();
        const uint32_t sel = n_vals >= kk ? block_select_kth_largest(s_vals, n_vals, kk, s_hist, s_ctl, tid) : 0u;
        if (tid == 0) s_ctl[0] = sel;
        __syncthreads();
        const uint32_t bound = s_ctl[0];
        for (uint32_t l = tid; l < n_lists; l += 1024) {
            for (uint32_t pos = 0; pos < depth_max; pos++) {
                const ott_hit h = lists[(size_t)l * gstride + pos];
                if (h.index == ~0ull) break;
                if (h.score != h.score) {
                    s_ctl[3] = 1u;
                    break;
                }
                const uint32_t o = ord_of(h.score, take_max != 0);
                if (o < bound) break;
                const uint32_t at = atomicAdd(&s_ctl[2], 1u);
                if (at < MS_CAP) s_key[at] = ((uint64_t)o << 32) | (uint32_t)(~(l * list_len + pos));
            }
        }
        __syncthreads();
        const uint32_t C = s_ctl[2];
        if (C <= MS_CAP && s_ctl[3] == 0) {
            for (uint32_t i = tid; i < C; i += 1024) {
                const uint64_t me = s_key[i];
                uint32_t r = 0;
#pragma unroll 8
                for (uint32_t x = 0; x < C; x++) r += s_key[x] > me ? 1u : 0u;
                if (r < kk) {
                    const uint32_t id = ~(uint32_t)(me & 0xFFFFFFFFull);
                    out_all[(size_t)grp * KS + r] = lists[(size_t)(id / list_len) * gstride + id % list_len];
                }
            }
            const uint32_t total = C < kk ? C : kk;
            for (uint32_t i = total + tid; i < KS; i += 1024) {
                ott_hit h;
                h.index = ~0ull;
                h.score = __uint_as_float(0xFFFFFFFFu);
                h.query = 0xFFFFFFFFu;
                out_all[(size_t)grp * KS + i] = h;
            }
            if (tid == 0) count[grp] = total;
            return;
        }
        __syncthreads();
    }
    merge_hits_walk<E>(smem, lists_all, n_lists, n_groups, list_len, k, take_max, out_all, count, gstride);
}

int launch_merge_hits(ott_store* s, const ott_hit* lists, uint32_t n_lists, uint32_t n_groups, uint32_t list_len, uint32_t k, int E,
                      bool take_max, ott_hit* out, uint64_t* count, uint32_t hdr_slots, ott_hit* hdr_out) {
    const uint32_t rank_stride = n_groups * list_len + hdr_slots;
    const size_t smem_w = (size_t)(MERGE_WAVES - 1) * 64 * E * sizeof(Cand);
    const size_t smem_r = (size_t)(MS_NVAL + 256 + 8) * 4 + (size_t)MS_CAP * 8;
    const size_t smem = smem_w > smem_r ? smem_w : smem_r;
    const uint32_t walk = s->opt.merge_walk ? 1u : 0u;
#define OTT_MH(Ev)                                                                                                   \
    if (E == Ev) {                                                                                                   \
        if (smem > 64 * 1024) {                                                                                      \
            static std::atomic<uint64_t> attr_set{0};                                                                \
            if (ott::attr_needed(attr_set, s->device)) {                                                         \
                OTT_HIP(hipFuncSetAttribute((const void*)merge_hits_kernel<Ev>, hipFuncAttributeMaxDynamicSharedMemorySize, (int)smem)); \
                ott::attr_done(attr_set, s->device);                                                     \
            }                                                                                                        \
        }                                                                                                            \
        hipLaunchKernelGGL((merge_hits_kernel<Ev>), dim3(n_groups), dim3(64 * MERGE_WAVES), smem, s->stream, lists, n_lists, \
                           n_groups, list_len, k, take_max ? 1u : 0u, out, count, walk, rank_stride, hdr_slots, hdr_out); \
        OTT_HIP(hipGetLastError());                                                                                  \
        return OTT_OK;                                                                                               \
    }
    OTT_MH(1) OTT_MH(2) OTT_MH(4) OTT_MH(8)
#undef OTT_MH
    return fail(OTT_ERR_INVALID, "launch_merge_hits: bad E");
}

int exact_grid(const ott_store* s, uint32_t n_tiles) {
    uint32_t want = (n_tiles + WAVES - 1) / WAVES;
    uint32_t cap = (uint32_t)s->n_cu * BLOCKS_PER_CU;
    if (want < 1) want = 1;
    return (int)(want < cap ? want : cap);
}

template <int E, bool BLK, int SK, bool SEED = false>
static int launch_prune(ott_store* s, const ExactParams& p, int grid) {
    auto kern = exact_kernel<MK_DOT, 1, E, false, false, false, BLK, false, true, SK, SEED>;
    static std::atomic<uint64_t> attr_set{0};
    if (ott::attr_needed(attr_set, s->device)) {
        OTT_HIP(hipFuncSetAttribute((const void*)kern, hipFuncAttributeMaxDynamicSharedMemorySize, EXACT_SMEM_PRUNE));
        ott::attr_done(attr_set, s->device);
    }
    hipLaunchKernelGGL(kern, dim3(grid), dim3(256), EXACT_SMEM_PRUNE, s->stream, p);
    OTT_HIP(hipGetLastError());
    return OTT_OK;
}

template <int E, bool BLK>
static int launch_prune_head(ott_store* s, const ExactParams& p, int grid) {
    if constexpr (SK4_INT && E == 1) {
        if (p.seed_est != 0) return launch_prune<E, BLK, 5, true>(s, p, grid);
    }
    if (p.seed_est != 0) return fail(OTT_ERR_INVALID, "launch_exact: the estimate pass needs the integer decode and a list of k <= 64");
    if constexpr (SK4_INT && E <= 4) return launch_prune<E, BLK, 5>(s, p, grid);
    else return fail(OTT_ERR_INVALID, "launch_exact: the head form needs the integer decode and a list of k <= 256");
}

template <int MK, int NQ, int E, bool PERQ>
static int launch_one(ott_store* s, const ExactParams& p, int grid) {
    if constexpr (MK == MK_DOT && NQ == 1 && !PERQ) {
        if (p.prune_stage != 0) {
            uint32_t sk = p.prune_sketch != nullptr ? p.sk_bits : 0u;
            if (p.prune_head_codes != nullptr) {
                if (sk != 4 || p.prune_head_rho == nullptr || !SK4_INT) return fail(OTT_ERR_INVALID, "launch_exact: the head belongs to the four-bit sketch and its integer decode");
                sk = 5;
            }
            if (sk != 0 && sk != 1 && sk != 3 && sk != 4 && sk != 5) return fail(OTT_ERR_INVALID, "launch_exact: a tail sketch has one, three or four bits per dim");
            if constexpr (E == 1) {
                if (p.k > 16)
                    return sk == 5 ? launch_prune_head<1, true>(s, p, grid) : sk == 4 ? launch_prune<1, true, 4>(s, p, grid) : sk == 3 ? launch_prune<1, true, 3>(s, p, grid) : sk == 1 ? launch_prune<1, true, 1>(s, p, grid) : launch_prune<1, true, 0>(s, p, grid);
            }
            return sk == 5 ? launch_prune_head<E, (E > 1)>(s, p, grid) : sk == 4 ? launch_prune<E, (E > 1), 4>(s, p, grid) : sk == 3 ? launch_prune<E, (E > 1), 3>(s, p, grid) : sk == 1 ? launch_prune<E, (E > 1), 1>(s, p, grid) : launch_prune<E, (E > 1), 0>(s, p, grid);
        }
    }
    if (p.prune_stage != 0) return fail(OTT_ERR_INVALID, "launch_exact: the pruned sweep takes one query, cosine / dot, merged");
#ifdef OTT_MFMA_DEBUG_BUILD
    if constexpr (NQ == 1 && E <= 2 && !PERQ) {
        if (p.small == 1) {
            static std::atomic<uint64_t> attr_set{0};
            auto kern = exact_kernel<MK, NQ, E, PERQ, false, true>;
            if (ott::attr_needed(attr_set, s->device)) {
                OTT_HIP(hipFuncSetAttribute((const void*)kern, hipFuncAttributeMaxDynamicSharedMemorySize, EXACT_SMEM_SMALL));
                ott::attr_done(attr_set, s->device);
            }
            hipLaunchKernelGGL(kern, dim3(grid), dim3(64), EXACT_SMEM_SMALL, s->stream, p);
            OTT_HIP(hipGetLastError());
            return OTT_OK;
        }
    }
#else
    if (p.small == 1) return fail(OTT_ERR_UNSUPPORTED, "exact_small = 1 (the one-wave LDS-DMA variant) exists in the diagnostic build only");
#endif
    if constexpr (E == 1) {
        if (p.k > 16) {
            hipLaunchKernelGGL((exact_kernel<MK, NQ, E, PERQ, false, false, true>), dim3(grid), dim3(256), EXACT_SMEM, s->stream, p);
            OTT_HIP(hipGetLastError());
            return OTT_OK;
        }
    }
    hipLaunchKernelGGL((exact_kernel<MK, NQ, E, PERQ>), dim3(grid), dim3(256), EXACT_SMEM, s->stream, p);
    OTT_HIP(hipGetLastError());
    return OTT_OK;
}

template <int MK>
static int launch_pass(ott_store* s, const ExactParams& p, int nq_tile, int E, int grid) {
    const bool perq = p.perq != 0 && nq_tile > 1;
#define OTT_CASE(NQv, Ev, PQ) \
    if (nq_tile == NQv && E == Ev && perq == PQ) return launch_one<MK, NQv, Ev, PQ>(s, p, grid);
    OTT_CASE(1, 1, false) OTT_CASE(2, 1, false) OTT_CASE(4, 1, false)
    OTT_CASE(1, 2, false) OTT_CASE(2, 2, false) OTT_CASE(4, 2, false)
    OTT_CASE(1, 4, false) OTT_CASE(1, 8, false)
    OTT_CASE(2, 1, true) OTT_CASE(4, 1, true)
    OTT_CASE(2, 2, true) OTT_CASE(4, 2, true)
#undef OTT_CASE
    return fail(OTT_ERR_INVALID, "launch_exact: no kernel for this (nq_tile, E, mode)");
}

int launch_exact_dump(ott_store* s, const ExactParams& p, int nq_tile, int grid) {
#define OTT_DUMP(MKv)                                                                                                                     \
    if (nq_tile == 1) hipLaunchKernelGGL((exact_kernel<MKv, 1, 1, false, true>), dim3(grid), dim3(256), EXACT_SMEM_DUMP, s->stream, p); \
    else hipLaunchKernelGGL((exact_kernel<MKv, 4, 1, false, true>), dim3(grid), dim3(256), EXACT_SMEM_DUMP, s->stream, p);
    switch (metric_kind(p.metric)) {
        case MK_L2: OTT_DUMP(MK_L2) break;
        case MK_L1: OTT_DUMP(MK_L1) break;
        default: OTT_DUMP(MK_DOT) break;
    }
#undef OTT_DUMP
    OTT_HIP(hipGetLastError());
    return OTT_OK;
}

template <int MK>
static int launch_rows8(ott_store* s, const ExactParams& p, int nq_tile, int E, int grid) {
    const bool perq = p.perq != 0 && nq_tile > 1;
    const size_t smem = ((size_t)nq_tile * p.dimq + (size_t)nq_tile * 64 + 64) * 4;
// ... 103 lines not shown
```

otters_amd/csrc/ott_exact_plan.h:

```cpp
#pragma once
#include <stddef.h>

#include "../../include/otters_hip.h"

namespace ott {

constexpr uint32_t OTT_QEMB_MAX = 896;
constexpr uint32_t OTT_SKETCH_MAX_WORDS = 54;
constexpr uint32_t OTT_SKETCH1_MAX_WORDS = 10;
constexpr uint32_t OTT_SKETCH4_MAX_WORDS = 108;

inline int list_E(uint64_t k) { return k <= 64 ? 1 : k <= 128 ? 2 : k <= 256 ? 4 : 8; }
inline uint32_t list_stride(int E) { return 64u * (uint32_t)E; }

enum ExactRoute {
    EXACT_LISTS,
    EXACT_SORT,
    EXACT_REFUSED,
};
inline ExactRoute lists_or_sort(uint64_t k_eff, uint32_t nq, uint64_t rows_scored, int large_k_from, bool fetch) {
    if (k_eff > 512) return fetch ? EXACT_SORT : EXACT_REFUSED;
    const uint64_t pairs = rows_scored * nq;
    const uint64_t from = large_k_from > 0 ? (uint64_t)large_k_from : ((nq == 1 || pairs <= (1ull << 19)) ? 512u : 128u);
    return k_eff > from && fetch && pairs <= (1ull << 28) ? EXACT_SORT : EXACT_LISTS;
// ... 18 lines not shown
    return p2 < most ? p2 : most;
}
inline bool exact_lean(uint32_t nq, uint32_t dimq, size_t n_runs) { return nq == 1 && dimq <= OTT_QEMB_MAX && n_runs <= 2; }

struct ExactPlan {
    int E;
    uint32_t KS;
    uint32_t variant;
    uint32_t tile;
    uint32_t passes;
    int grid;
    bool lean;
};
inline ExactPlan exact_plan(uint64_t k_eff, uint32_t nq, bool perq, uint32_t dimq, uint32_t n_tiles, size_t n_runs, int exact_small, int stream_grid) {
    ExactPlan x;
    x.E = list_E(k_eff);
    x.KS = list_stride(x.E);
    x.variant = exact_variant(exact_small, nq, perq, x.E, dimq, n_tiles);
    x.tile = queries_per_pass(nq, x.E, x.variant);
    x.passes = (nq + x.tile - 1) / x.tile;
    x.grid = x.variant ? (int)n_tiles : stream_grid;
    x.lean = exact_lean(nq, dimq, n_runs);
    return x;
}
inline size_t exact_n_lists(const ExactPlan& x, uint32_t nq, bool perq, bool pruned, int gridA, int gridB) {
    return pruned ? (size_t)(gridA + gridB) : perq ? (size_t)nq * x.grid : (size_t)x.passes * x.grid;
}

#ifndef OTT_X_SEED_DIV
#define OTT_X_SEED_DIV 32
#endif
struct SketchState {
    bool present;
    bool covers;
    uint32_t bits, words, stage0;
};
struct PruneIn {
    uint32_t dim, ld, metric;
    bool perq, lean, flat;
    uint32_t variant;
    int exact_prune, exact_sketch;
    SketchState sk;
    uint64_t rows_scored;
    int E;
};
struct PrunePlan {
    uint32_t c;
    bool sketch;
    uint64_t seed;
};
inline PrunePlan prune_plan(const PruneIn& in) {
    const PrunePlan off{0, false, 0};
    if (!(in.lean && !in.perq && in.variant == 0 && !in.flat && in.exact_prune != 0 && (in.metric == OTT_METRIC_COSINE || in.metric == OTT_METRIC_DOT)))
        return off;
    const uint32_t nst = (in.ld + 31) / 32;
    uint32_t c = nst * 7 / 8;
    while (c > 0 && c * 32 > in.dim - in.dim % 8) c--;
    bool sketch = false;
    if (in.exact_sketch != 0 && in.sk.present && in.sk.covers &&
        in.sk.words <= (in.sk.bits == 4 ? OTT_SKETCH4_MAX_WORDS : in.sk.bits == 3 ? OTT_SKETCH_MAX_WORDS : OTT_SKETCH1_MAX_WORDS)) {
        const uint32_t cs = in.sk.stage0;
        if (cs >= 1 && cs < nst && cs * 32 <= in.dim - in.dim % 8) {
            c = cs;
            sketch = true;
        }
    }
    const bool worth = in.exact_prune == 1 || (nst >= 8 && in.rows_scored >= (1ull << 20));
    if (!(worth && c >= 1 && c < nst)) return off;
    uint64_t seed = in.rows_scored / 10;
    if (sketch && in.sk.bits >= 3 && in.E == 1 && seed > 131072) seed = in.rows_scored / OTT_X_SEED_DIV > 131072 ? in.rows_scored / OTT_X_SEED_DIV : 131072;
    seed = (seed + 63) & ~63ull;
    if (seed < 64) seed = 64;
    return PrunePlan{c, sketch, seed};
}
inline bool prune_plan_needs_quant(const PruneIn& in, const PrunePlan& pp) { return pp.c != 0 && pp.sketch && in.sk.bits == 4; }
struct HeadState {
    bool present;
    bool covers;
    int option;
};
inline bool prune_plan_head(const PruneIn& in, const PrunePlan& pp, bool quant_ok, const HeadState& hd) {
    return prune_plan_needs_quant(in, pp) && quant_ok && hd.present && hd.covers && hd.option != 0 && in.E <= 4;
}
#ifndef OTT_X_SEED_EST
#define OTT_X_SEED_EST 1
#endif
#ifndef OTT_X_SEED_EST_DIV
#define OTT_X_SEED_EST_DIV 0
#endif
#ifndef OTT_X_SEED_KEEP
#define OTT_X_SEED_KEEP 0
#endif
constexpr uint64_t SEED_EST_MIN_ROWS = 131072;
constexpr uint32_t SEED_EST_KEEP_MAX = 16;
inline uint64_t prune_plan_seed_est(const PruneIn& in, const PrunePlan& pp, bool head, bool filtered) {
    if (!OTT_X_SEED_EST || !head || in.E != 1 || filtered || pp.c == 0 || in.rows_scored / 10 < SEED_EST_MIN_ROWS) return 0;
    uint64_t rows = pp.seed;
    if (OTT_X_SEED_EST_DIV > 0) {
        rows = (in.rows_scored / (uint64_t)(OTT_X_SEED_EST_DIV > 0 ? OTT_X_SEED_EST_DIV : 1) + 63) & ~63ull;
        if (rows < SEED_EST_MIN_ROWS) rows = SEED_EST_MIN_ROWS;
    }
    return rows;
}
inline uint32_t prune_seed_keep(uint64_t k) {
    if (OTT_X_SEED_KEEP > 0) return OTT_X_SEED_KEEP < 64 ? (uint32_t)OTT_X_SEED_KEEP : 64u;
    return k < SEED_EST_KEEP_MAX ? (uint32_t)k : SEED_EST_KEEP_MAX;
}
inline PrunePlan prune_plan_quant_refused(PruneIn in) {
    in.exact_sketch = 0;
    return prune_plan(in);
}

struct ExactResult {
    size_t cnt_pad;
    size_t bytes;
    size_t host_bytes;
};
inline ExactResult exact_result_layout(uint32_t groups, uint32_t KS) {
    const size_t cnt_pad = (((size_t)groups * sizeof(uint64_t)) + 63) & ~(size_t)63;
    const size_t bytes = cnt_pad + (size_t)groups * KS * sizeof(ott_hit);
    return ExactResult{cnt_pad, bytes, bytes + 8};
}

inline uint64_t exact_bytes_scanned(uint32_t passes, uint64_t rows_scored, uint32_t dim, uint32_t metric) {
    return (uint64_t)passes * rows_scored * ((uint64_t)dim * 4 + (metric == OTT_METRIC_COSINE ? 4 : 0));
}

}
```

otters_amd/csrc/ott_internal.h:

```cpp
#pragma once

#include <hip/hip_runtime.h>
#include <stdint.h>

#include <atomic>
#include <chrono>
#include <condition_variable>
#include <functional>
#include <mutex>
#include <shared_mutex>
#include <string>
#include <vector>

#include "../../include/otters_hip.h"
#include "ott_host.h"
#include "ott_policy.h"
#include "ott_plane_policy.h"
#include "ott_mfma_plan.h"
#include "ott_maxsim_gather_plan.h"
#include "ott_exact_plan.h"
#include "ott_discover_plan.h"
#include "ott_recommend_plan.h"
#include "ott_mmr_plan.h"
#include "ott_masks_plan.h"
#include "ott_sparse_plan.h"
#include "ott_sort_plan.h"
#ifdef OTT_DEVICE_AUDIT
#include "ott_audit.h"
#endif

namespace ott {

void set_error(const std::string& msg);
int fail(int code, const std::string& msg);

#define OTT_HIP(expr)                                                                              \
    do {                                                                                           \
        hipError_t _e = (expr);                                                                    \
        if (_e != hipSuccess) {                                                                    \
            (void)hipGetLastError();  \
            return ::ott::fail(_e == hipErrorOutOfMemory ? OTT_ERR_OOM : OTT_ERR_HIP,              \
                               std::string(#expr) + ": " + hipGetErrorString(_e));                 \
        }                                                                                          \
    } while (0)

#ifndef OTT_DEVICE_AUDIT
#define OTT_AUDIT_PTR(ptr, store) ((void)0)
inline hipError_t use_device_raw(int device, int ) { return hipSetDevice(device); }
#endif

inline bool attr_needed(const std::atomic<uint64_t>& seen, int device) {
    return device > 63 || !((seen.load(std::memory_order_acquire) >> (device & 63)) & 1ull);
}
inline void attr_done(std::atomic<uint64_t>& seen, int device) {
    if (device <= 63) seen.fetch_or(1ull << (device & 63), std::memory_order_release);
}

inline uint64_t now_ns() {
    return (uint64_t)std::chrono::duration_cast<std::chrono::nanoseconds>(std::chrono::steady_clock::now().time_since_epoch()).count();
}

inline uint32_t grid_blocks(uint64_t items, uint32_t per_block, int n_cu, uint32_t per_cu = 8) {
    const uint64_t want = (items + per_block - 1) / per_block, most = (uint64_t)n_cu * per_cu;
    return (uint32_t)(want < 1 ? 1 : want < most ? want : most);
}

struct DevBuf {
    void* p = nullptr;
    size_t cap = 0;
    int ensure(size_t bytes);
    void release();
};
struct PinBuf {
    void* p = nullptr;
    size_t cap = 0;
    int ensure(size_t bytes);
    void release();
};

struct Options {
    int exact_small = -1;
    int exact_prune = -1;
    int exact_sketch = -1;
    int exact_sketch_bits = 4;
    int exact_sketch_head = -1;
    int force_fallback = 0;
    bool mfma_f32 = false;
    bool no_hi_pass = false;
    bool no_batch_image = false;
    int mfma_wg = 0;
    int mfma_growth = 8;
    bool mfma_no_dense = false;
    bool mfma_debug = false;
    int mfma_abl = 0;
    int mfma_spec = -1;
    int mfma_coop = -1;
    int tie_order = 0;
    int hi_fmt = -1;
    int hi_tmin = 0;
    int merge_rank1 = -1;
    bool merge_walk = false;
    int large_k_from = 0;
    int large_k_pre = -1;
    int hi_prebuild = -1;
    int stage_appends = -1;
    int small_sort = -1;
    int eps_scale_ppm = 1000000;
    int multi_transport = 0;
    int multi_rebalance = 1;
    bool multi_fake_distinct = false;
    int id_gather = -1;
    int group_gather = -1;
    int masks_sweep = 2;
    int maxsim_fold = -1;
    int multi_min_shard_rows = 32768;
    int fuse_device = -1;
    int sparse_table = -1;
};
void options_from_env(Options& o);
int option_set(Options& o, const char* name, long long value);

struct NcclId {
    char internal[OTT_COMM_ID_BYTES];
};
struct Rccl {
    void* handle = nullptr;
    int (*GetUniqueId)(NcclId*) = nullptr;
    int (*CommInitRank)(void**, int, NcclId, int) = nullptr;
    int (*CommInitAll)(void**, int, const int*) = nullptr;
    int (*CommDestroy)(void*) = nullptr;
    int (*CommCount)(void*, int*) = nullptr;
    int (*GetVersion)(int*) = nullptr;
    int (*GroupStart)() = nullptr;
    int (*GroupEnd)() = nullptr;
    int (*AllGather)(const void*, void*, size_t, int, void*, hipStream_t) = nullptr;
    const char* (*GetErrorString)(int) = nullptr;
    std::string why;
};
constexpr int kNcclUint8 = 1;
Rccl* rccl();

struct Plane {
    void* d = nullptr;
    uint64_t rows = 0;
    bool off = false;
    uint32_t* d_rel = nullptr;
    float rel = 0.0f;
};
struct PlaneSet {
    std::mutex mu;
    Plane split;
    Plane hi;
    HiFormat hi_format{false, 1.0f};
    Plane i8;
    float* d_i8_scale = nullptr;
};

struct Column {
    uint32_t dtype;
    void* d_vals;
    uint64_t* d_nulls;
    uint64_t n;
};

}

struct ott_run {
    uint64_t start;
    uint64_t count;
};

struct ott_multi;

struct ott_store {
    ott_multi* multi = nullptr;
    int device = 0;
    int logical = 0;
    uint32_t dim = 0;
    uint32_t ld = 0;
    uint32_t dimq = 0;
    uint64_t n = 0, cap = 0;
    uint64_t chunk_size = 1024;
    uint64_t base_offset = 0;
    uint32_t reduce = OTT_REDUCE_AVX;
    int n_cu = 256;
    float min_pos_inv = __builtin_inff();
    ott::Options opt;

    float* d_rows = nullptr;
    float* d_inv = nullptr;
    uint32_t* d_sketch = nullptr;
    uint64_t sk_n = 0;
    uint32_t sk_words = 0, sk_pitch = 0, sk_stage0 = 0;
    uint32_t sk_bits = 0;
    char* d_head = nullptr;
    uint64_t head_n = 0;
    uint8_t* d_flag = nullptr;
    ott::PlaneSet planes;
    ott::CascadeState cascade;

    hipStream_t stream = nullptr;
    hipEvent_t ev[7] = {};

    ott::DevBuf d_queries, d_qinv, d_rowmask, d_runs, d_prefix, d_lists, d_lists2, d_hits, d_count, d_cand, d_misc;
    ott::DevBuf d_prune;
    ott::DevBuf d_tails;
    uint64_t tails_seen = 0;
    ott::DevBuf d_minpos;
    ott::DevBuf m_Q, m_qinv, m_qnorm, m_tau, m_cntA, m_cntB, m_candA, m_candB, m_over, m_out, m_outcnt, m_uncert, m_prefix;
    ott::DevBuf l_keysA, l_keysB, l_qA, l_qB, l_tmp, l_cursor, l_hist, l_gate;
    ott::DevBuf l_ctl;
    bool l_ctl_clean = false;
    ott_hit* direct_out = nullptr;
    uint64_t direct_cap = 0;
    bool direct_done = false;
    std::vector<uint64_t> direct_counts;
    ott::DevBuf x_send, x_recv;
    ott::DevBuf d_evalmask;
    uint64_t evalmask_bits = 0;
    ott::DevBuf d_mslot[OTT_MASK_SLOTS];
    uint64_t mslot_bits[OTT_MASK_SLOTS] = {};
    ott::DevBuf d_qmasks;
    const uint64_t* cur_qmask = nullptr;
    uint64_t cur_qmask_bits = 0;
    uint64_t* d_live = nullptr;
    uint64_t n_dead = 0;
    ott::DevBuf d_livefx;
    ott::DevBuf d_idmask, d_gather;
    uint64_t* cur_idmask = nullptr;
    ott::DevBuf d_mmr;
    ott::DevBuf d_rectable;
    bool rectable_clean = false;
    ott::DevBuf d_disc;
    ott::PinBuf h_disc;
    uint32_t* d_gid = nullptr;
    uint64_t gid_n = 0;
    uint32_t n_groups = 0;
    ott::DevBuf d_gtable, d_gctl;
    bool gtable_clean = false;
    ott::DevBuf d_mstable;
    bool mstable_clean = false;
    uint32_t* d_gix = nullptr;
    std::vector<uint32_t> gix_start;
    std::atomic<bool> gix_ready{false};
    std::atomic<uint64_t> gix_builds{0};
    ott::PinBuf h_pend;
    ott::host::StagedRows pend;
    ott::PinBuf h_stage, h_hits, h_hdr;
    size_t in_off_qinv = 0, in_off_runs = 0, in_off_prefix = 0;
    uint32_t cur_tie_sh = 0, cur_tie_off = 0;
    bool cur_flat = false;

    ott::host::QuietWorker* builder = nullptr;
    std::vector<ott::Column> columns;
    ott::host::RwGate rw;
    std::mutex mu;
    ott::host::ContextPool<ott_store> pool;
    bool is_worker = false;
    ott_store* owner = nullptr;
    ott::DevBuf d_fuse;
    ott::PinBuf h_fuse;
    char* d_sparse = nullptr;
    uint64_t sparse_n = 0, sparse_nnz = 0;
    uint32_t sparse_vocab = 0;
    ott::SparseLayout sparse_lay{};
    std::vector<uint64_t> sparse_base;
    ott::DevBuf d_spq, d_sptable;
    ott::PinBuf h_spq;
    bool sptable_clean = false;
};

namespace ott {
inline hipError_t use_device(const ott_store* s) { return use_device_raw(s->device, s->logical); }
int store_create(uint32_t dim, int device, int logical, ott_store** out);
enum AppendKind { APPEND_HOST = 0, APPEND_DEVICE = 1, APPEND_RANDOM = 2, APPEND_CLUSTERED = 3 };
struct AppendArgs {
    int kind = APPEND_HOST;
    const void* rows = nullptr;
    uint64_t seed = 0;
    uint32_t n_clusters = 0;
    float spread = 0.f, aniso = 0.f;
};
int multi_destroy(ott_store* ms);
int multi_reserve(ott_store* ms, uint64_t n_rows);
int multi_append(ott_store* ms, const AppendArgs& a, uint64_t n_rows);
int multi_write_rows(ott_store* ms, uint64_t first_row, const float* rows_host, uint64_t n_rows);
int multi_set_live(ott_store* ms, bool live, const uint64_t* rows_host, uint64_t n, uint64_t* n_changed);
uint64_t multi_live_len(const ott_store* ms);
int multi_read_live_mask(const ott_store* ms, uint64_t* out_host);
int multi_read(const ott_store* ms, bool inv_norms, uint64_t first_row, uint64_t n_rows, float* out_host);
int multi_set_chunk_size(ott_store* ms, uint64_t chunk_size);
int multi_set_base_offset(ott_store* ms, uint64_t base);
int multi_set_reduce_order(ott_store* ms, uint32_t reduce);
int multi_set_batch_image(ott_store* ms, int enabled);
int multi_set_option(ott_store* ms, const char* name, int64_t value);
int multi_prepare_batch(ott_store* ms);
int multi_sync(ott_store* ms);
int multi_batch_ready(ott_store* ms);
int multi_add_column(ott_store* ms, uint32_t dtype, const void* values_host, const uint64_t* nulls, uint64_t n, uint32_t* out_column_id);
int multi_eval_row_mask(ott_store* ms, const ott_leaf* leaves, uint32_t n_leaves, uint32_t n_clauses, uint64_t* out_host);
int multi_zone_stats(ott_store* ms, uint32_t column, uint64_t chunk_size, void* out_min, void* out_max, uint64_t* out_non_null);
int multi_query(ott_store* ms, const ott_query_desc* d, ott_hit* out, uint64_t cap, uint64_t* n_out, uint64_t* n_per_query, ott_stats* stats);
void mfma_warm(hipStream_t stream, int device);
void kick_plane_build(ott_store* s);
inline uint64_t store_rows(const ott_store* s) { return s->n + s->pend.count(); }
int store_flush(ott_store* s);
int store_flush_locked(ott_store* s);
int store_adopt(ott_store* s, float* rows, float* inv, uint8_t* flag, uint32_t* sketch, uint32_t sketch_bits, char* head, uint64_t n, uint64_t cap);

constexpr size_t OTT_MAX_WORKERS = 15;
ott_store* ctx_acquire(ott_store* s);
void ctx_release(ott_store* w);
struct CtxLease {
    ott_store* c;
    explicit CtxLease(ott_store* owner) : c(ctx_acquire(owner)) {}
    ~CtxLease() { ctx_release(c); }
    CtxLease(const CtxLease&) = delete;
    CtxLease& operator=(const CtxLease&) = delete;
};
inline int lock_store_shared(ott_store* s, ott::host::SharedLock& rd) {
    return ott::host::lock_shared_clean(s->rw, rd, [s] { return s->pend.count() != 0; }, [s] { return store_flush(s); });
}
struct IdMaskGuard {
    ott_store* c;
    ~IdMaskGuard() { c->cur_idmask = nullptr; }
};
void planes_drop(ott_store* own);
bool planes_any(ott_store* own);
void planes_release(ott_store* own);
int planes_rewrite(ott_store* s, uint64_t first, uint64_t n);
int planes_clear_marks(ott_store* s, uint64_t n);
void planes_enable(ott_store* own, bool enabled);
void planes_set_options(ott_store* own, const Options& o);
int ensure_batch_image(ott_store* ctx, const uint16_t** img_out);
int ensure_hi_plane(ott_store* ctx, const uint16_t** img_out, float* rel_max_out, bool* f16_out = nullptr, float* scale_out = nullptr);
bool hi_plane_ready(ott_store* ctx);
inline bool i8_wanted(const Options& o) { return i8_wanted(o.hi_fmt, o.mfma_f32, o.no_hi_pass, o.no_batch_image); }
int ensure_first_plane(ott_store* ctx);
bool first_plane_ready(ott_store* ctx);
struct PlaneSnapshot {
    bool have_i8, i8_off, have_hi, hi_f16, hi_off, img_off;
    uint64_t i8_rows, hi_rows;
};
PlaneSnapshot plane_snapshot(const ott_store* s);
int ensure_i8_plane(ott_store* ctx, const int8_t** img_out, const float** scale_out, float* rel_max_out);
bool i8_plane_ready(ott_store* ctx);
int launch_i8_rows(hipStream_t stream, const float* rows, uint32_t ld, uint32_t dim, uint32_t ld8, uint64_t first, uint64_t n, int8_t* out,
                   const float* pre, float common_scale, float* scale_out, float* rel_out, uint32_t* rel_max, const uint8_t* flag, float rel_flag,
                   uint8_t* flag_rw, int n_cu);
int launch_hi_rows(hipStream_t stream, const float* rows, uint32_t ld, uint32_t dim, uint32_t ldh, uint64_t n, uint16_t* out,
                   const float* scale, float* rel_out, int n_cu, bool f16 = false, float gscale = 1.0f);
int launch_split_rows(hipStream_t stream, const float* rows, uint32_t ld, uint32_t dim, uint32_t ldi, uint64_t n, uint16_t* out,
                      const float* scale, int n_cu);
}

namespace ott {

__host__ __device__ inline uint32_t total_key(float f) {
    uint32_t b;
#if defined(__HIP_DEVICE_COMPILE__)
    b = __float_as_uint(f);
#else
    __builtin_memcpy(&b, &f, 4);
#endif
    return (b & 0x80000000u) ? ~b : (b | 0x80000000u);
}
__host__ __device__ inline uint32_t ord_of(float f, bool take_max) {
    uint32_t k = total_key(f);
    return take_max ? k : ~k;
}
__host__ __device__ inline float score_of(uint32_t ord, bool take_max) {
    uint32_t k = take_max ? ord : ~ord;
    uint32_t b = (k & 0x80000000u) ? (k & 0x7FFFFFFFu) : ~k;
    float f;
#if defined(__HIP_DEVICE_COMPILE__)
    f = __uint_as_float(b);
#else
    __builtin_memcpy(&f, &b, 4);
#endif
    return f;
}

struct Cand {
    uint64_t key;
    uint32_t q;
    uint32_t pad;
};

struct ExactParams {
    const float* rows;
    const float* inv;
    const float* queries;
    const float* qinv;
    const uint64_t* row_mask;
    const ott_run* runs;
    const uint32_t* tile_prefix;
    Cand* lists;
    uint64_t row_mask_bits;
    uint32_t ld, dim, dimq;
    uint32_t n_runs, n_tiles;
    uint32_t q0, nq_total;
    uint32_t metric, take_max, cmp, reduce;
    float thr;
    uint32_t k;
    uint32_t perq;
    uint32_t list_stride;
    uint32_t tie_sh;
    uint32_t tie_off;
    uint32_t flat;
    uint32_t embedded;
    uint32_t small;
    float eqinv;
    uint32_t eprefix[3];
    ott_run eruns[2];
    uint64_t* dump_keys;
    uint32_t* dump_q;
    unsigned long long* dump_cursor;
    uint64_t dump_cap;
    const uint32_t* dump_gate;
    uint32_t i8;
    float i8_qscale;
    const float* i8_scale;
    const uint8_t* flag;
    uint32_t prune_stage;
    uint32_t sk_pitch, sk_stage0, sk_bits;
    const uint64_t* prune_seed;
    const uint32_t* prune_sketch;
    const uint32_t* prune_head_codes;
    const float* prune_head_rho;
    unsigned long long* prune_tails;
    double prune_qt, prune_qn, prune_q1;
    double prune_qe1;
    float prune_qscale, prune_qinv_scale;
    int32_t prune_qsum;
    uint32_t seed_est, seed_keep;
    float qemb[OTT_QEMB_MAX];
};
static_assert(sizeof(ExactParams) <= 4096, "kernel arguments are limited to 4 KB");

int launch_exact(ott_store* s, const ExactParams& p, int nq_tile, int E, int grid);
int launch_exact_i8(ott_store* s, const ExactParams& p, int E, int grid);
int launch_exact_dump(ott_store* s, const ExactParams& p, int nq_tile, int grid);
int exact_grid(const ott_store* s, uint32_t n_tiles);
int launch_merge(ott_store* s, const Cand* lists, uint32_t n_lists, uint32_t list_stride, uint64_t group_stride,
                 uint32_t groups, uint32_t k, int E, bool take_max, uint64_t base_offset, ott_hit* out_hits,
                 uint64_t out_stride, uint64_t* out_counts, uint32_t tie_sh);

int launch_merge_hits(ott_store* s, const ott_hit* lists, uint32_t n_lists, uint32_t n_groups, uint32_t list_len, uint32_t k, int E,
                      bool take_max, ott_hit* out, uint64_t* count, uint32_t hdr_slots = 0, ott_hit* hdr_out = nullptr);

int live_grow(ott_store* s, uint64_t ncap);
void live_drop(ott_store* s);
int live_load(ott_store* s, const uint64_t* words_host);
int live_read(const ott_store* s, uint64_t* out_host);
int live_compose(ott_store* ctx, const uint64_t** d_mask, uint64_t* mask_bits);
int mask_and(ott_store* ctx, const uint64_t* keep, const uint64_t* caller, uint64_t caller_bits, uint64_t n_bits, uint64_t* out);
int store_after_compact(ott_store* s, uint64_t new_n);
int launch_inv_norms(ott_store* s, uint64_t first_row, uint64_t n_rows);
bool store_wants_sketch(const ott_store* s);
int update_min_pos_inv(ott_store* s, uint64_t first_row, uint64_t n_rows);

struct RunPlan {
    std::vector<ott_run> runs;
    uint64_t rows_scored = 0, total_chunks = 0, evaluated = 0;
};
std::vector<uint32_t> tile_prefix(const RunPlan& pl, uint32_t tile_rows);
void split_plan(const RunPlan& pl, uint64_t m_rows, RunPlan& a, RunPlan& b);

int run_large_k(ott_store* s, const float* queries, uint32_t nq, const ott_query_desc* d, bool perq, const RunPlan& pl, uint64_t k_eff,
                const uint64_t* d_mask, uint64_t mask_bits, std::vector<std::vector<ott_hit>>& lists, ott_stats& st);
void fill_exact_params(ott_store* s, const ott_query_desc* d, const RunPlan& pl, uint32_t nq, const uint64_t* d_mask, uint64_t mask_bits,
                       uint32_t n_tiles, ExactParams& p);
float host_inv_norm_exact(const float* v, uint32_t dim);
void embed_exact_inputs(ExactParams& p, const void* query, size_t query_bytes, float inv_norm, const RunPlan& pl, const std::vector<uint32_t>& prefix);
int upload_exact_inputs(ott_store* s, const float* queries, uint32_t nq, const RunPlan& pl, const std::vector<uint32_t>& prefix);

int run_mfma(ott_store* s, const ott_query_desc* d, const RunPlan& pl, uint64_t k_q, const uint64_t* d_mask, uint64_t mask_bits,
             std::vector<std::vector<ott_hit>>& out, std::vector<uint32_t>& uncertified, ott_stats& st, int level, uint32_t t_min,
             bool spec_gate);
int launch_rand_fill(ott_store* s, uint64_t first_row, uint64_t n_rows, uint64_t seed);
int run_i8_single(ott_store* s, const ott_query_desc* d, const RunPlan& pl, uint64_t k_q, const uint64_t* d_mask, uint64_t mask_bits,
                  std::vector<std::vector<ott_hit>>& out, std::vector<uint32_t>& uncertified, ott_stats& st, uint32_t t_min);

struct CanonLess {
    bool tmax;
    uint32_t sh = 0;
    uint64_t base = 0;
    bool operator()(const ott_hit& a, const ott_hit& b) const {
        const uint32_t ka = ord_of(a.score, tmax), kb = ord_of(b.score, tmax);
        if (ka != kb) return ka > kb;
        if (sh) {
            const uint64_t ba = (a.index - base) >> sh, bb = (b.index - base) >> sh;
            if (ba != bb) return ba < bb;
            if (a.query != b.query) return a.query < b.query;
            return a.index < b.index;
        }
        if (a.index != b.index) return a.index < b.index;
        return a.query < b.query;
    }
};
inline void merge_heads(std::vector<const ott_hit*>& head, const std::vector<const ott_hit*>& end, const CanonLess& less, ott_hit* dst, uint64_t n) {
    const size_t G = head.size();
    std::vector<size_t> act(G);
    std::vector<uint32_t> key(G);
    size_t n_act = 0;
    for (size_t g = 0; g < G; g++)
        if (head[g] != end[g]) {
            key[n_act] = ~ord_of(head[g]->score, less.tmax);
            act[n_act++] = g;
        }
    for (uint64_t i = 0; i < n; i++) {
        size_t bi = 0;
        for (size_t a = 1; a < n_act; a++)
            if (key[a] < key[bi] || (key[a] == key[bi] && less(*head[act[a]], *head[act[bi]]))) bi = a;
        const size_t b = act[bi];
        dst[i] = *head[b]++;
        if (head[b] == end[b]) {
            --n_act;
// ... 119 lines not shown
```

otters_amd/csrc/ott_mfma.hip:

```cpp
#include <math.h>
#include <stdio.h>
#include <stdlib.h>
#include <string.h>
#include <time.h>

#include <algorithm>
#include <atomic>
#include <mutex>
#include <utility>
#include <vector>

#include "ott_internal.h"

namespace ott {

typedef float f32x16 __attribute__((ext_vector_type(16)));
typedef float f32x4 __attribute__((ext_vector_type(4)));
typedef __bf16 bf16x8 __attribute__((ext_vector_type(8)));
typedef _Float16 f16x8 __attribute__((ext_vector_type(8)));
typedef int i32x16 __attribute__((ext_vector_type(16)));
typedef int i32x4 __attribute__((ext_vector_type(4)));

template <bool MICRO, bool I8 = false> struct AccT { typedef f32x16 type; };
template <> struct AccT<true, false> { typedef f32x4 type; };
template <> struct AccT<false, true> { typedef i32x16 type; };
typedef __attribute__((address_space(1))) void* GPTR;
typedef __attribute__((address_space(3))) void* LPTR;

#ifndef OTT_STAGE_STAMPS
#define OTT_STAGE_STAMPS 1
#endif
constexpr int BM = 256;
constexpr int MKC = 32;
constexpr int A_FLOATS = BM * MKC;
__host__ __device__ constexpr uint32_t mfma_qw(int nb) { return nb == -1 ? 128u : nb == 0 ? 200u : nb == 1 ? 256u : nb == 2 ? 160u : 288u; }
__host__ __device__ constexpr int mfma_nbuf(int nb) { return nb <= 0 ? 4 : nb == 4 ? 2 : 3; }

constexpr uint32_t CNT_STRIDE = 32;

struct CandEntry {
    uint32_t row;
    float score;
};

struct MfmaParams {
    const float* rows;
    const uint16_t* img;
    const float* inv;
    const float* i8_scale;
    float i8_qscale;
    const uint8_t* flag;
    const float* Q;
    const float* qinv;
    const float* tau;
    uint32_t* cnt;
    CandEntry* cand;
    const ott_run* runs;
    const uint32_t* tile_prefix;
    const uint64_t* row_mask;
    uint64_t row_mask_bits;
    uint32_t cap;
    uint32_t ld, dim, ldq;
    uint32_t n_runs, tile_begin, tile_end;
    uint32_t q_base;
    uint32_t n_qblk;
    uint32_t coop;
    uint32_t dense;
    uint32_t metric, take_max;
    float flo, fhi;
    uint32_t dbg_wgs;
    uint32_t dbg_abl;
    unsigned long long* dbg;
};

template <bool NT = false>
__device__ __forceinline__ void glds16(const char* sbase, uint32_t voff, uint32_t lds_addr) {
    uint32_t keep;
    lds_addr = (uint32_t)__builtin_amdgcn_readfirstlane((int)lds_addr);
    {
        const unsigned long long b = (unsigned long long)sbase;
        const unsigned long long lo = (uint32_t)__builtin_amdgcn_readfirstlane((int)(uint32_t)b);
        const unsigned long long hi = (uint32_t)__builtin_amdgcn_readfirstlane((int)(uint32_t)(b >> 32));
        sbase = (const char*)((hi << 32) | lo);
    }
    if constexpr (NT) {
        asm volatile(
            "s_nop 4\n\t"
            "s_mov_b32 %0, m0\n\t"
            "s_mov_b32 m0, %3\n\t"
            "s_nop 0\n\t"
            "global_load_lds_dwordx4 %1, %2 nt\n\t"
            "s_mov_b32 m0, %0"
            : "=&s"(keep)
            : "v"(voff), "s"(sbase), "s"(lds_addr)
            : "memory");
// ... 1385 lines not shown
        std::swap(cnt_cur, cnt_oth);
        std::swap(cand_cur, cand_oth);
        width *= (begin == 0 && wg_per_cu == 2 && growth == 8) ? 16 : growth;
        begin = end;
    }
    OTT_HIP(hipEventRecord(s->ev[1], s->stream));
    if (dbg_on && (rc = dump_tile_timing(s, slots))) return rc;

    const FinalParams f = fill_final_params(s, d, level, nq, k, bud, ldq, em, mx_norm, qb, hh_dev, rb, cand_cur, cnt_cur);
    if ((rc = launch_finalize(s->stream, nq, bud.E, bud.wide, f))) return rc;
    OTT_HIP(hipEventRecord(s->ev[2], s->stream));
    const double hm2 = host_ms();
    OTT_HIP(hipStreamSynchronize(s->stream));
    const double hm3 = host_ms();
    unpack_results(s, d, rb, k, bud.T, qnorm.data(), g.passes(), pl.rows_scored, out, uncertified, st);
    if (dbg_on) fprintf(stderr, "[ott mfma dbg] host ms: prepare %.3f  enqueue %.3f  wait %.3f  unpack %.3f\n", hm1 - hm0, hm2 - hm1, hm3 - hm2, host_ms() - hm3);
    return OTT_OK;
}


static int launch_finalize(hipStream_t stream, uint32_t nq, int E, bool wide, const FinalParams& f) {
#define OTT_FIN(Ev, TCAPv) hipLaunchKernelGGL((finalize_kernel<Ev, TCAPv>), dim3(nq), dim3(64 * FIN_WAVES), 0, stream, f)
    switch (wide ? -E : E) {
        case -1: OTT_FIN(1, 4096); break;
        case -2: OTT_FIN(2, 4096); break;
        case -4: OTT_FIN(4, 4096); break;
        case -8: OTT_FIN(8, 4096); break;
        case 1: OTT_FIN(1, 64); break;
        case 2: OTT_FIN(2, 128); break;
        case 4: OTT_FIN(4, 256); break;
        default: OTT_FIN(8, 512); break;
    }
#undef OTT_FIN
    OTT_HIP(hipGetLastError());
    return OTT_OK;
}


__global__ void i8_hits_to_cand_kernel(const ott_hit* hits, const uint64_t* count, uint32_t T, uint32_t take_max, CandEntry* cand, uint32_t* cnt,
                                       float* tau, float* gate, uint32_t* overflow) {
    const uint32_t n = (uint32_t)(count[0] < T ? count[0] : T);
    for (uint32_t i = threadIdx.x; i < n; i += blockDim.x) {
        CandEntry e;
        e.row = (uint32_t)hits[i].index;
        e.score = hits[i].score;
        cand[i] = e;
    }
    if (threadIdx.x == 0) {
        cnt[0] = n;
        const float open = take_max ? -__builtin_inff() : __builtin_inff();
        float t = open;
        if (n == T && T > 0) {
            const float last = hits[T - 1].score;
            t = (last - last == 0.0f) ? last : __uint_as_float(0x7FC00000u);
        }
        tau[0] = t;
        gate[0] = t;
        overflow[0] = 0u;
    }
}

int run_i8_single(ott_store* s, const ott_query_desc* d, const RunPlan& pl, uint64_t k_q, const uint64_t* d_mask, uint64_t mask_bits,
                  std::vector<std::vector<ott_hit>>& out, std::vector<uint32_t>& uncertified, ott_stats& st, uint32_t t_min) {
    if (d->nq != 1 || d->metric == OTT_METRIC_EUCLIDEAN || d->filter_cmp == OTT_CMP_EQ) return fail(OTT_ERR_UNSUPPORTED, "run_i8_single: one query, cosine / dot, no equality filter");
    constexpr int level = 2;
    const int8_t* img8 = nullptr;
    const float* i8_scale = nullptr;
    float i8_rel = 0.0f;
    int rc = ensure_i8_plane(s, &img8, &i8_scale, &i8_rel);
    if (rc) return rc;
    if (!img8) return fail(OTT_ERR_UNSUPPORTED, "run_i8_single: the int8 plane is unavailable");
    const uint32_t dim = s->dim;
    const TileGeometry g = tile_geometry(1, level, dim);
    const uint32_t ld8 = g.ldh * 2;
    if (ld8 > OTT_QEMB_MAX * 4) return fail(OTT_ERR_UNSUPPORTED, "run_i8_single: the query does not fit the kernel arguments");
    const bool cosine = d->metric == OTT_METRIC_COSINE, tmax = d->take == OTT_TAKE_MAX;
    const uint32_t k = (uint32_t)k_q;
    const Budget bud = level_budget(level, k, t_min, pl.rows_scored, true);
    if (bud.k_too_large) return fail(OTT_ERR_UNSUPPORTED, "run_i8_single: k too large");
    const uint32_t T = bud.T;

    const float* q = d->queries;
    const float q_inv = host_inv_norm_exact(q, dim);
    double n2 = 0.0;
    float amax = 0.0f;
    for (uint32_t i = 0; i < dim; i++) {
        n2 += (double)q[i] * q[i];
        amax = fmaxf(amax, fabsf(q[i]));
    }
    const float qnorm = (float)(sqrt(n2) * (1.0 + 1e-6));
    out.assign(1, {});
    uncertified.assign(1, 1u);
    st.path_used = OTT_PATH_MFMA;
    if (!query_regular(qnorm)) return OTT_OK;
    const float pf = cosine ? q_inv : 1.0f;
    const float e_max = amax * pf;
    const float s_q = (e_max > 0.0f && e_max < __builtin_inff()) ? e_max / 127.0f : 1.0f;
    const float inv_sq = 1.0f / s_q;
    int8_t q8[OTT_QEMB_MAX * 4];
    memset(q8, 0, ld8);
    double se = 0.0, sx = 0.0;
    for (uint32_t i = 0; i < dim; i++) {
        const float xe = q[i] * pf;
        float t = rintf(xe * inv_sq);
        t = t == t ? fminf(fmaxf(t, -127.0f), 127.0f) : 0.0f;
        q8[i] = (int8_t)(int)t;
        const double df = (double)xe - (double)s_q * (double)(int)t;
        se += df * df;
        sx += (double)xe * (double)xe;
    }
    float qrel = sx > 0.0 ? (float)(sqrt(se / sx) * 1.0001) : 0.0f;
    if (!(qrel <= 1.0f)) qrel = 1.0f;

    const ErrorModel em = error_model(level, false, dim, d->metric, true, s->opt.eps_scale_ppm, i8_rel);
    const float mx_norm = max_norm(s->min_pos_inv);
    const float eps_max = em.eps_max(d->metric, qnorm, mx_norm);
    if (!(eps_max < __builtin_inff())) return fail(OTT_ERR_UNSUPPORTED, "run_i8_single: non-finite error bound");
    const FilterInterval fi = relaxed_filter(d->filter_cmp, d->filter_thr, eps_max);

    const std::vector<uint32_t> prefix = tile_prefix(pl, 64);
    const uint32_t n_tiles = prefix.back();
    const int grid = exact_grid(s, n_tiles);
    const QueryBlock qb = query_block(1, g.ldq, pl.runs.size(), prefix.size(), false);
    const size_t off_q8 = (qb.total + 15) & ~(size_t)15, tot = off_q8 + ld8;
    if ((rc = s->m_Q.ensure(tot))) return rc;
    if ((rc = s->h_stage.ensure(tot))) return rc;
    if ((rc = s->m_candA.ensure((size_t)T * sizeof(CandEntry)))) return rc;
    if ((rc = s->d_lists.ensure((size_t)grid * T * sizeof(Cand)))) return rc;
    const size_t cnt_pad = 64;
    if ((rc = s->d_hits.ensure(cnt_pad + (size_t)T * sizeof(ott_hit)))) return rc;
    const ResultBlock rb(1, k);
    if ((rc = s->h_hits.ensure(rb.total))) return rc;
    char* hh_dev = nullptr;
    OTT_HIP(hipHostGetDevicePointer((void**)&hh_dev, s->h_hits.p, 0));
    char* hs = (char*)s->h_stage.p;
    memset(hs, 0, tot);
    memcpy(hs, q, (size_t)dim * 4);
    *(float*)(hs + qb.qinv) = q_inv;
    *(float*)(hs + qb.qnorm) = qnorm;
    *(float*)(hs + qb.qrel) = qrel;
    memcpy(hs + qb.runs, pl.runs.data(), pl.runs.size() * sizeof(ott_run));
    memcpy(hs + qb.prefix, prefix.data(), prefix.size() * 4);
    memcpy(hs + off_q8, q8, ld8);
    OTT_HIP(hipMemcpyAsync(s->m_Q.p, hs, tot, hipMemcpyHostToDevice, s->stream));
    char* dblk = (char*)s->m_Q.p;

    ExactParams p;
    memset(&p, 0, sizeof(p));
    p.rows = reinterpret_cast<const float*>(img8);
    p.inv = s->d_inv;
    p.row_mask = d_mask;
    p.row_mask_bits = mask_bits;
    p.ld = p.dim = p.dimq = ld8 / 4;
    p.n_runs = (uint32_t)pl.runs.size();
    p.n_tiles = n_tiles;
    p.nq_total = 1;
    p.metric = d->metric;
    p.take_max = tmax;
    p.reduce = s->reduce;
    p.cmp = OTT_CMP_NONE;
    switch (d->filter_cmp) {
        case OTT_CMP_GT: case OTT_CMP_GTE: p.cmp = OTT_CMP_GTE; p.thr = fi.flo; break;
        case OTT_CMP_LT: case OTT_CMP_LTE: p.cmp = OTT_CMP_LTE; p.thr = fi.fhi; break;
        default: break;
    }
    p.k = T;
    p.list_stride = T;
    p.lists = (Cand*)s->d_lists.p;
    p.i8 = 1;
    p.i8_qscale = s_q;
    p.i8_scale = i8_scale;
    p.flag = s->d_flag;
    if (pl.runs.size() <= 2) {
        embed_exact_inputs(p, q8, ld8, 0.0f, pl, prefix);
    } else {
        p.queries = (const float*)(dblk + off_q8);
        p.qinv = (const float*)(dblk + qb.qinv);
        p.runs = (const ott_run*)(dblk + qb.runs);
        p.tile_prefix = (const uint32_t*)(dblk + qb.prefix);
    }
    OTT_HIP(hipEventRecord(s->ev[0], s->stream));
    if ((rc = launch_exact_i8(s, p, bud.E, grid))) return rc;
    ott_hit* d_hits = (ott_hit*)((char*)s->d_hits.p + cnt_pad);
    uint64_t* d_counts = (uint64_t*)s->d_hits.p;
    if ((rc = launch_merge(s, (const Cand*)s->d_lists.p, (uint32_t)grid, T, 0, 1, T, bud.E, tmax, 0, d_hits, T, d_counts, 0))) return rc;
    OTT_HIP(hipEventRecord(s->ev[1], s->stream));
    hipLaunchKernelGGL(i8_hits_to_cand_kernel, dim3(1), dim3(256), 0, s->stream, (const ott_hit*)d_hits, (const uint64_t*)d_counts, T, tmax ? 1u : 0u,
                       (CandEntry*)s->m_candA.p, (uint32_t*)(dblk + qb.cntA), (float*)(dblk + qb.tau), (float*)(dblk + qb.gate), (uint32_t*)(dblk + qb.over));
    OTT_HIP(hipGetLastError());

    const FinalParams f = fill_final_params(s, d, level, 1, k, bud, g.ldq, em, mx_norm, qb, hh_dev, rb, (const CandEntry*)s->m_candA.p, (const uint32_t*)(dblk + qb.cntA));
    if ((rc = launch_finalize(s->stream, 1, bud.E, false, f))) return rc;
    OTT_HIP(hipEventRecord(s->ev[2], s->stream));
    OTT_HIP(hipStreamSynchronize(s->stream));
    unpack_results(s, d, rb, k, T, &qnorm, 1, pl.rows_scored, out, uncertified, st);
// ... 24 lines not shown
```

otters_amd/csrc/ott_multi.hip:

```cpp
#include <string.h>

#include <algorithm>
#include <condition_variable>
#include <deque>
#include <functional>
#include <mutex>
#include <numeric>
#include <thread>
#include <vector>

#include "ott_internal.h"

using namespace ott;

namespace {

constexpr uint64_t NOT_YET = ~0ull;

using ott::host::ShardPool;

uint64_t gcd64(uint64_t a, uint64_t b) {
    while (b) {
        const uint64_t t = a % b;
        a = b;
// ... 924 lines not shown
        const ott_store* s = ms->multi->shards[pc.g];
        const uint64_t off = pc.first_global - first_row;
        const int rc = inv_norms ? ott_store_read_inv_norms(s, pc.first_local, pc.count, out_host + off)
                                 : ott_store_read_rows(s, pc.first_local, pc.count, out_host + off * ms->dim);
        if (rc) return rc;
    }
    return OTT_OK;
}

int multi_set_chunk_size(ott_store* ms, uint64_t chunk_size) {
    ott::host::ExclusiveLock wr(ms->rw);
    const uint64_t cs = chunk_size < 1 ? 1 : chunk_size;
    const uint64_t old = ms->chunk_size;
    ms->chunk_size = cs;
    for (ott_store* s : ms->multi->shards) s->chunk_size = cs;
    if (ms->n && !layout_aligned(ms, granule_of(cs))) {
        const int rc = ensure_layout(ms, true);
        if (rc) {
            ms->chunk_size = old;
            for (ott_store* s : ms->multi->shards) s->chunk_size = old;
            return rc;
        }
    } else if (ms->n == 0 && ms->multi->plan_rows) {
        ms->multi->start = ideal_starts(ms->multi->plan_rows, granule_of(cs), n_shards(ms), min_rows_of(ms));
        mark_unused(ms->multi->start, ms->multi->plan_rows, granule_of(cs));
        set_shard_bases(ms);
    }
    return OTT_OK;
}

int multi_set_base_offset(ott_store* ms, uint64_t base) {
    ott::host::ExclusiveLock wr(ms->rw);
    ms->base_offset = base;
    set_shard_bases(ms);
    return OTT_OK;
}

int multi_set_reduce_order(ott_store* ms, uint32_t reduce) {
    ott::host::ExclusiveLock wr(ms->rw);
    ms->reduce = reduce;
    for (ott_store* s : ms->multi->shards) s->reduce = reduce;
    return OTT_OK;
}

int multi_set_batch_image(ott_store* ms, int enabled) {
    ott::host::ExclusiveLock wr(ms->rw);
    for (ott_store* s : ms->multi->shards) {
        const int rc = ott_store_set_batch_image(s, enabled);
        if (rc) return rc;
    }
    return OTT_OK;
}

int multi_set_option(ott_store* ms, const char* name, int64_t value) {
    ott::host::ExclusiveLock wr(ms->rw);
    Options o = ms->opt;
    if (option_set(o, name, (long long)value)) return fail(OTT_ERR_INVALID, std::string("ott_store_set_option: unknown option or bad value: ") + name);
    if (std::string(name) == "multi_transport" && ms->multi->transport != 0 && o.multi_transport != ms->opt.multi_transport)
        return fail(OTT_ERR_INVALID, "ott_store_set_option: multi_transport is chosen before the first query of a multi-GPU store");
    if (o.multi_fake_distinct != ms->opt.multi_fake_distinct)
        return fail(OTT_ERR_INVALID, "ott_store_set_option: multi_fake_distinct is read when the store is created (OTT_MULTI_FAKE_DISTINCT=1)");
    ms->opt = o;
    for (ott_store* s : ms->multi->shards) {
        const int rc = ott_store_set_option(s, name, value);
        if (rc) return rc;
    }
    return OTT_OK;
}

int multi_prepare_batch(ott_store* ms) {
    ott::host::SharedLock rd;
    const int rcl = lock_clean(ms, rd);
    if (rcl) return rcl;
    return run_on_shards(ms, [&](size_t g) -> int { return ott_store_prepare_batch(ms->multi->shards[g]); });
}

int multi_batch_ready(ott_store* ms) {
    ott::host::SharedLock rd(ms->rw);
    for (ott_store* s : ms->multi->shards)
        if (store_rows(s) && !ott_store_batch_ready(s)) return 0;
    return ms->n ? 1 : 0;
}

int multi_sync(ott_store* ms) {
    for (ott_store* s : ms->multi->shards) {
        const int rc = ott_store_sync(s);
        if (rc) return rc;
    }
    return OTT_OK;
}

int multi_add_column(ott_store* ms, uint32_t dtype, const void* values_host, const uint64_t* nulls, uint64_t n, uint32_t* out_column_id) {
    size_t esz;
    switch (dtype) {
        case OTT_DT_INT32: case OTT_DT_FLOAT32: esz = 4; break;
        case OTT_DT_INT64: case OTT_DT_FLOAT64: case OTT_DT_DATETIME: esz = 8; break;
        default: return fail(OTT_ERR_INVALID, "ott_store_add_column: only numeric / datetime columns live on the GPU");
    }
    ott::host::ExclusiveLock wr(ms->rw);
    if (n != ms->n) return fail(OTT_ERR_INVALID, "ott_store_add_column: column length does not match the store length");
    if (n && !values_host) return fail(OTT_ERR_INVALID, "ott_store_add_column: values is NULL");
    ott_multi* m = ms->multi;
    int rc;
    if (m->layout_dirty) {
        if ((rc = ensure_layout(ms, false))) return rc;
        m->layout_dirty = false;
    }
    const size_t G = m->shards.size();
    std::vector<uint32_t> ids(G, 0);
    rc = run_on_shards(ms, [&](size_t g) -> int {
        ott_store* s = m->shards[g];
        const uint64_t s0 = start_of(ms, g), n_g = store_rows(s);
        std::vector<uint64_t> nl;
        if (nulls && n_g) slice_bits_bytes(nulls, s0, n_g, nl);
        return ott_store_add_column(s, dtype, n_g ? (const char*)values_host + s0 * esz : nullptr, (nulls && n_g) ? nl.data() : nullptr, n_g, &ids[g]);
    });
    if (rc) return rc;
    for (size_t g = 1; g < G; g++)
        if (ids[g] != ids[0]) return fail(OTT_ERR_INVALID, "multi-GPU store: internal error (column ids differ between shards)");
    *out_column_id = ids[0];
    return OTT_OK;
}

int multi_eval_row_mask(ott_store* ms, const ott_leaf* leaves, uint32_t n_leaves, uint32_t n_clauses, uint64_t* out_host) {
    ott::host::ExclusiveLock wr(ms->rw);
    ott_multi* m = ms->multi;
    const size_t G = m->shards.size();
    ms->evalmask_bits = 0;
    std::vector<std::vector<uint64_t>> part(G);
    int rc = run_on_shards(ms, [&](size_t g) -> int {
        ott_store* s = m->shards[g];
        if (out_host) part[g].assign((size_t)((store_rows(s) + 63) / 64) + 1, 0);
        return ott_store_eval_row_mask(s, leaves, n_leaves, n_clauses, out_host ? part[g].data() : nullptr);
    });
    if (rc) return rc;
    if (out_host) {
        memset(out_host, 0, (size_t)((ms->n + 63) / 64) * 8);
        for (size_t g = 0; g < G; g++) {
            const uint64_t n_g = store_rows(m->shards[g]);
            if (n_g) memcpy((uint8_t*)out_host + start_of(ms, g) / 8, part[g].data(), (size_t)((n_g + 7) / 8));
        }
    }
    ms->evalmask_bits = ms->n;
    return OTT_OK;
}

int multi_zone_stats(ott_store* ms, uint32_t column, uint64_t chunk_size, void* out_min, void* out_max, uint64_t* out_non_null) {
    ott::host::ExclusiveLock wr(ms->rw);
    ott_multi* m = ms->multi;
    const size_t G = m->shards.size();
    for (size_t g = 1; g < G; g++)
        if (store_rows(m->shards[g]) && m->start[g] % chunk_size != 0)
            return fail(OTT_ERR_UNSUPPORTED, "ott_store_zone_stats on a multi-GPU store: chunk_size must divide the shard boundaries (use the store's chunk size)");
    return run_on_shards(ms, [&](size_t g) -> int {
        ott_store* s = m->shards[g];
        if (!store_rows(s)) return OTT_OK;
        const uint64_t c0 = start_of(ms, g) / chunk_size;
        return ott_store_zone_stats(s, column, chunk_size, (char*)out_min + c0 * 8, (char*)out_max + c0 * 8, out_non_null + c0);
    });
}

int multi_query(ott_store* ms, const ott_query_desc* d, ott_hit* out, uint64_t cap, uint64_t* n_out, uint64_t* n_per_query, ott_stats* stats) {
    int rc = validate_query(ms, d);
    if (rc) return rc;
    ott_multi* m = ms->multi;
    const uint64_t t0 = now_ns();
// ... 349 lines not shown
```

otters_amd/csrc/ott_planes.hip:

```cpp
#include <string.h>

#include <chrono>

#include "ott_internal.h"

namespace ott {


__device__ __forceinline__ void plane_row_loss(double se, double sx, uint64_t i, uint64_t r, float* __restrict__ rel_out, uint32_t* __restrict__ rel_max,
                                               const uint8_t* flag, float rel_flag, uint8_t* flag_rw, uint8_t bit, bool unmark) {
    float rel = sx > 0.0 ? (float)(sqrt(se / sx) * 1.0001) : 0.0f;
    if (!(rel <= 1.0f)) rel = 1.0f;
    if (rel_out) rel_out[i] = rel;
    bool irregular = flag && (flag[r] & 1u);
    if (flag_rw && !irregular) {
        if (rel > rel_flag) {
            flag_rw[r] = (uint8_t)(flag_rw[r] | bit);
            irregular = true;
            if (rel_max) atomicAdd(rel_max + 1, 1u);
        } else if (unmark && (flag_rw[r] & bit)) {
            flag_rw[r] = (uint8_t)(flag_rw[r] & ~bit);
        }
    }
    if (rel_max && !irregular && __float_as_uint(rel) > __hip_atomic_load(rel_max, __ATOMIC_RELAXED, __HIP_MEMORY_SCOPE_AGENT))
// ... 360 lines not shown
            if ((rc = plane_extend(own, ctx->stream, p.hi, convert_hi, &marked))) return rc;
        }
        p.hi.rows = own->n;
    }
    *img_out = (const uint16_t*)p.hi.d;
    *rel_max_out = p.hi.rel;
    if (f16_out) *f16_out = p.hi_format.f16;
    if (scale_out) *scale_out = p.hi_format.scale;
    return OTT_OK;
}

static void i8_decline(PlaneSet& p) {
    (void)hipFree(p.i8.d);
    if (p.d_i8_scale) (void)hipFree(p.d_i8_scale);
    p.i8.d = nullptr;
    p.d_i8_scale = nullptr;
    p.i8.off = true;
}

int ensure_i8_plane(ott_store* ctx, const int8_t** img_out, const float** scale_out, float* rel_max_out) {
    *img_out = nullptr;
    *scale_out = nullptr;
    ott_store* own = owner_of(ctx);
    PlaneSet& p = own->planes;
    std::lock_guard<std::mutex> g(p.mu);
    if (p.i8.off || p.split.off || own->n == 0 || !i8_wanted(own->opt) || own->dim < 8) return OTT_OK;
    if (!p.i8.d) {
        if (!plane_alloc(p.i8, (size_t)own->cap * i8_pitch(own), (size_t)own->cap * 4, own->opt.no_batch_image || own->opt.no_hi_pass)) return OTT_OK;
        if (hipMalloc((void**)&p.d_i8_scale, (size_t)own->cap * 4) != hipSuccess) {
            p.d_i8_scale = nullptr;
            i8_decline(p);
            (void)hipGetLastError();
            return OTT_OK;
        }
    }
    int rc = plane_loss_words(p.i8, ctx->stream);
    if (rc) return rc;
    if (p.i8.rows < own->n) {
        const bool from_scratch = p.i8.rows == 0;
        const uint64_t cnt = own->n - p.i8.rows;
        uint32_t marked = 0;
        if ((rc = plane_extend(own, ctx->stream, p.i8, convert_i8, &marked))) return rc;
        if (from_scratch && format_rejected(marked, cnt)) {
            if ((rc = clear_flag_bits(own, ctx->stream, own->n, 0xFB))) return rc;
            OTT_HIP(hipStreamSynchronize(ctx->stream));
            i8_decline(p);
            return OTT_OK;
        }
        p.i8.rows = own->n;
    }
    *img_out = (const int8_t*)p.i8.d;
    *scale_out = p.d_i8_scale;
    *rel_max_out = p.i8.rel;
    return OTT_OK;
}

int ensure_first_plane(ott_store* ctx) {
    ott_store* own = owner_of(ctx);
    float rel = 0.f;
    if (i8_wanted(own->opt)) {
        const int8_t* i8 = nullptr;
        const float* i8s = nullptr;
        const int rc = ensure_i8_plane(ctx, &i8, &i8s, &rel);
        if (rc) return rc;
        if (i8 && !plane_snapshot(own).have_hi) return OTT_OK;
    }
    const uint16_t* img = nullptr;
    return ensure_hi_plane(ctx, &img, &rel);
}

PlaneSnapshot plane_snapshot(const ott_store* s) {
    ott_store* own = owner_of(s);
    const PlaneSet& p = own->planes;
    std::lock_guard<std::mutex> g(own->planes.mu);
    return PlaneSnapshot{p.i8.d != nullptr, p.i8.off, p.hi.d != nullptr, p.hi_format.f16, p.hi.off, p.split.off, p.i8.rows, p.hi.rows};
}

static bool plane_ready(ott_store* own, const Plane& pl) {
    std::lock_guard<std::mutex> g(own->planes.mu);
    return pl.d != nullptr && !pl.off && !own->planes.split.off && own->n != 0 && pl.rows == own->n;
}
bool hi_plane_ready(ott_store* ctx) { return plane_ready(owner_of(ctx), owner_of(ctx)->planes.hi); }
bool i8_plane_ready(ott_store* ctx) { return plane_ready(owner_of(ctx), owner_of(ctx)->planes.i8); }

bool first_plane_ready(ott_store* ctx) {
    ott_store* own = owner_of(ctx);
    bool i8_on;
    {
        std::lock_guard<std::mutex> g(own->planes.mu);
        i8_on = i8_wanted(own->opt) && !own->planes.i8.off && own->dim >= 8;
    }
    return i8_on ? i8_plane_ready(ctx) : hi_plane_ready(ctx);
}


static void plane_builder_run(ott_store* s) {
    ott::host::SharedLock rd(s->rw);
    if (use_device(s) != hipSuccess) return;
    if (s->opt.hi_prebuild < 0) {
        size_t free_b = 0, total_b = 0;
        const PlaneSnapshot ps = plane_snapshot(s);
        const bool i8 = i8_wanted(s->opt) && !ps.i8_off;
        const size_t bytes = i8 ? (size_t)s->cap * i8_pitch(s) : (size_t)s->cap * hi_pitch(s) * 2;
        if (!(i8 ? ps.have_i8 : ps.have_hi) && (hipMemGetInfo(&free_b, &total_b) != hipSuccess || bytes > free_b / 4)) return;
    }
    ott_store* ctx = ctx_acquire(s);
    mfma_warm(ctx->stream, s->device);
    (void)ensure_first_plane(ctx);
    ctx_release(ctx);
    (void)hipGetLastError();
}

void kick_plane_build(ott_store* s) {
    if (s->is_worker || s->multi) return;
    const int pol = s->opt.hi_prebuild;
    const PlaneSnapshot ps = plane_snapshot(s);
    if (pol == 0 || s->opt.no_hi_pass || s->opt.no_batch_image || s->opt.mfma_f32 || ps.hi_off || ps.img_off) return;
    if (pol < 0 && s->n < 262144) return;
    if (s->dim < 8) return;
    {
        const bool i8 = i8_wanted(s->opt) && !ps.i8_off;
        const bool i8_stale = i8 && ps.i8_rows < s->n, hi_stale = (!i8 || ps.have_hi) && ps.hi_rows < s->n;
        if (!i8_stale && !hi_stale) return;
    }
    if (!s->builder) s->builder = new ott::host::QuietWorker([s] { plane_builder_run(s); }, std::chrono::milliseconds(20));
    s->builder->kick();
}

}
```

otters_amd/csrc/ott_store.hip:

```cpp
#include <stdlib.h>
#include <string.h>

#include <thread>

#include <algorithm>

#include "ott_internal.h"
#include "ott_prune.h"

namespace ott {

static thread_local std::string g_err;

void set_error(const std::string& msg) { g_err = msg; }
int fail(int code, const std::string& msg) {
    g_err = msg;
    return code;
}
const char* last_error() { return g_err.c_str(); }

namespace {
struct OptName {
    const char* name;
    int kind;
};
const OptName kOptNames[] = {{"tie_order", 2},       {"hi_fmt", 1},          {"hi_prebuild", 1},          {"stage_appends", 1},       {"multi_transport", 2},
                             {"multi_rebalance", 0}, {"multi_min_shard_rows", 2}, {"exact_small", 1},     {"large_k_from", 2},        {"small_sort", 1},
                             {"mfma_f32", 0},        {"no_hi_pass", 0},      {"no_batch_image", 0},       {"force_fallback", 2},      {"eps_scale_ppm", 2},
                             {"multi_fake_distinct", 0}, {"exact_prune", 1},            {"exact_sketch", 1},
                             {"id_gather", 1},       {"exact_sketch_bits", 2},   {"group_gather", 1},         {"exact_sketch_head", 1},
                             {"masks_sweep", 2},     {"fuse_device", 1},         {"sparse_table", 1},
#ifdef OTT_MFMA_DEBUG_BUILD
                             {"mfma_wg", 2},         {"mfma_growth", 2},     {"mfma_debug", 0},           {"mfma_abl", 2},            {"hi_tmin", 2},
                             {"mfma_no_dense", 0},   {"mfma_coop", 1},       {"mfma_spec", 1},            {"large_k_pre", 1},         {"merge_walk", 0},
                             {"merge_rank1", 1},     {"maxsim_fold", 1},
#endif
};
static_assert(sizeof(kOptNames) / sizeof(kOptNames[0]) <= 25
#ifdef OTT_MFMA_DEBUG_BUILD
                                                            + 12
#endif
              , "the product library's option table stays at twenty-five entries");
}

int option_set(Options& o, const char* name, long long v) {
    if (!name) return -1;
    const std::string n(name);
    auto tri = [&](int& dst) { if (v < -1 || v > 1) return -1; dst = (int)v; return 0; };
    auto flag = [&](bool& dst) { if (v < 0 || v > 1) return -1; dst = v != 0; return 0; };
    if (n == "exact_small") {
#ifdef OTT_MFMA_DEBUG_BUILD
        if (v < -1 || v > 2) return -1;
#else
        if (v < -1 || v > 2 || v == 1) return -1;
#endif
        o.exact_small = (int)v;
        return 0;
    }
    if (n == "force_fallback") {
        if (v < 0 || v > 127) return -1;
        o.force_fallback = (int)v;
        o.merge_walk = (v & 1) != 0;
        o.merge_rank1 = (v & 2) ? 0 : -1;
        o.mfma_coop = (v & 4) ? 0 : -1;
        o.large_k_pre = (v & 8) ? 0 : -1;
        o.mfma_no_dense = (v & 16) != 0;
        o.mfma_spec = (v & 32) ? 0 : -1;
        return 0;
    }
    if (n == "mfma_f32") return flag(o.mfma_f32);
    if (n == "no_hi_pass") return flag(o.no_hi_pass);
    if (n == "no_batch_image") return flag(o.no_batch_image);
    if (n == "hi_fmt") { if (v < -1 || v > 2) return -1; o.hi_fmt = (int)v; return 0; }
    if (n == "small_sort") return tri(o.small_sort);
    if (n == "exact_prune") return tri(o.exact_prune);
    if (n == "exact_sketch") return tri(o.exact_sketch);
    if (n == "exact_sketch_bits") { if (v != 1 && v != 3 && v != 4) return -1; o.exact_sketch_bits = (int)v; return 0; }
    if (n == "exact_sketch_head") return tri(o.exact_sketch_head);
    if (n == "id_gather") return tri(o.id_gather);
    if (n == "group_gather") return tri(o.group_gather);
    if (n == "fuse_device") return tri(o.fuse_device);
    if (n == "sparse_table") return tri(o.sparse_table);
    if (n == "masks_sweep") { if (v < 0 || v > 2) return -1; o.masks_sweep = (int)v; return 0; }
#ifdef OTT_MFMA_DEBUG_BUILD
    if (n == "maxsim_fold") return tri(o.maxsim_fold);
    if (n == "mfma_coop") return tri(o.mfma_coop);
    if (n == "mfma_spec") return tri(o.mfma_spec);
    if (n == "mfma_no_dense") return flag(o.mfma_no_dense);
    if (n == "mfma_debug") return flag(o.mfma_debug);
    if (n == "merge_walk") return flag(o.merge_walk);
    if (n == "merge_rank1") return tri(o.merge_rank1);
    if (n == "large_k_pre") return tri(o.large_k_pre);
    if (n == "hi_tmin") { if (v < 0 || v > 512) return -1; o.hi_tmin = (int)v; return 0; }
    if (n == "mfma_abl") { if (v < 0 || v > 63) return -1; o.mfma_abl = (int)v; return 0; }
    if (n == "mfma_wg") { if (v < 0 || v > 8) return -1; o.mfma_wg = (int)v; return 0; }
    if (n == "mfma_growth") { if (v != 0 && (v < 2 || v > 64)) return -1; o.mfma_growth = v ? (int)v : 8; return 0; }
#endif
    if (n == "stage_appends") return tri(o.stage_appends);
    if (n == "hi_prebuild") return tri(o.hi_prebuild);
    if (n == "large_k_from") { if (v < 0 || v > 512) return -1; o.large_k_from = (int)v; return 0; }
    if (n == "eps_scale_ppm") { if (v < 1 || v > 1000000) return -1; o.eps_scale_ppm = (int)v; return 0; }
    if (n == "multi_transport") { if (v < 0 || v > 2) return -1; o.multi_transport = (int)v; return 0; }
    if (n == "multi_fake_distinct") return flag(o.multi_fake_distinct);
    if (n == "multi_rebalance") { if (v < 0 || v > 1) return -1; o.multi_rebalance = (int)v; return 0; }
    if (n == "multi_min_shard_rows") { if (v < 0 || v > 0x7FFFFFFF) return -1; o.multi_min_shard_rows = (int)v; return 0; }
    if (n == "tie_order") { if (v < 0 || v > 2) return -1; o.tie_order = (int)v; return 0; }
    return -1;
}

void options_from_env(Options& o) {
    for (const OptName& on : kOptNames) {
        std::string var = "OTT_";
        for (const char* c = on.name; *c; c++) var.push_back((char)(*c >= 'a' && *c <= 'z' ? *c - 32 : *c));
        const char* ev = getenv(var.c_str());
        if (!ev) continue;
        char* end = nullptr;
        long long v = strtoll(ev, &end, 10);
        if (end == ev) v = 1;
        (void)option_set(o, on.name, v);
    }
}

int DevBuf::ensure(size_t bytes) {
    if (bytes <= cap && p) return OTT_OK;
    size_t want = bytes < 256 ? 256 : bytes;
    if (p) (void)hipFree(p);
    p = nullptr;
    cap = 0;
    OTT_HIP(hipMalloc(&p, want));
    cap = want;
    return OTT_OK;
}
void DevBuf::release() {
    if (p) (void)hipFree(p);
    p = nullptr;
    cap = 0;
}
int PinBuf::ensure(size_t bytes) {
    if (bytes <= cap && p) return OTT_OK;
    size_t want = bytes < 4096 ? 4096 : bytes;
    if (p) (void)hipHostFree(p);
    p = nullptr;
    cap = 0;
    OTT_HIP(hipHostMalloc(&p, want, hipHostMallocDefault));
    cap = want;
    return OTT_OK;
}
void PinBuf::release() {
    if (p) (void)hipHostFree(p);
    p = nullptr;
    cap = 0;
}


constexpr int NKC = 32;
__global__ __launch_bounds__(256) void inv_norm_kernel(const float* __restrict__ rows, uint32_t ld, uint32_t dim,
                                                        uint64_t first, uint64_t n, float* __restrict__ inv, uint8_t* __restrict__ flag) {
    __shared__ __attribute__((aligned(16))) float smem[4 * 64 * NKC];
    const int lane = threadIdx.x & 63;
    const int wave = __builtin_amdgcn_readfirstlane(threadIdx.x >> 6);
    float* st = smem + wave * 64 * NKC;
// ... 851 lines not shown
        a.aniso = aniso;
        return multi_append(s, a, n_rows);
    }
    ott::host::ExclusiveLock wr(s->rw);
    std::lock_guard<std::mutex> g(s->mu);
    OTT_HIP(use_device(s));
    int rc = store_flush_locked(s);
    if (rc) return rc;
    if ((rc = grow(s, s->n + n_rows))) return rc;
    hipLaunchKernelGGL(clustered_fill_kernel, dim3((uint32_t)s->n_cu * 8), dim3(256), 0, s->stream, s->d_rows, s->ld, s->dim, s->n, n_rows,
                       s->base_offset + s->n, seed, n_clusters, spread, aniso);
    OTT_HIP(hipGetLastError());
    if ((rc = launch_inv_norms(s, s->n, n_rows))) return rc;
    if ((rc = update_min_pos_inv(s, s->n, n_rows))) return rc;
    s->n += n_rows;
    kick_plane_build(s);
    return OTT_OK;
}

int ott_store_set_batch_image(ott_store* s, int enabled) {
    if (!s) return fail(OTT_ERR_INVALID, "ott_store_set_batch_image: store is NULL");
    if (s->multi) return multi_set_batch_image(s, enabled);
    ott::host::ExclusiveLock wr(s->rw);
    if (!enabled && planes_any(s)) OTT_HIP(use_device(s));
    planes_enable(s, enabled != 0);
    return OTT_OK;
}

int ott_store_set_option(ott_store* s, const char* name, int64_t value) {
    if (!s || !name) return fail(OTT_ERR_INVALID, "ott_store_set_option: NULL argument");
    if (s->multi) return multi_set_option(s, name, value);
    ott::host::ExclusiveLock wr(s->rw);
    Options o = s->opt;
    if (option_set(o, name, (long long)value)) return fail(OTT_ERR_INVALID, std::string("ott_store_set_option: unknown option or bad value: ") + name);
    planes_set_options(s, o);
    return OTT_OK;
}

int ott_store_prepare_batch(ott_store* s) {
    if (!s) return fail(OTT_ERR_INVALID, "ott_store_prepare_batch: store is NULL");
    if (s->multi) return multi_prepare_batch(s);
    {
        const int rcf = store_flush(s);
        if (rcf) return rcf;
    }
    ott::host::SharedLock rd(s->rw);
    OTT_HIP(use_device(s));
    ott_store* ctx = ott::ctx_acquire(s);
    const int rc = ensure_first_plane(ctx);
    ott::ctx_release(ctx);
    return rc;
}

int ott_store_batch_ready(const ott_store* cs) {
    ott_store* s = const_cast<ott_store*>(cs);
    if (!s) return 0;
    if (s->multi) return multi_batch_ready(s);
    if (s->pend.count()) return 0;
    return first_plane_ready(s) ? 1 : 0;
}

int ott_store_write_rows(ott_store* s, uint64_t first_row, const float* rows_host, uint64_t n_rows) {
    if (!s) return fail(OTT_ERR_INVALID, "ott_store_write_rows: store is NULL");
    if (n_rows == 0) return OTT_OK;
    if (!rows_host) return fail(OTT_ERR_INVALID, "ott_store_write_rows: rows is NULL");
    if (s->multi) return multi_write_rows(s, first_row, rows_host, n_rows);
    ott::host::ExclusiveLock wr(s->rw);
    std::lock_guard<std::mutex> g(s->mu);
    {
        const int rcf = store_flush_locked(s);
        if (rcf) return rcf;
    }
    if (first_row + n_rows > s->n) return fail(OTT_ERR_INVALID, "ott_store_write_rows: range exceeds store length");
    OTT_HIP(use_device(s));
    OTT_HIP(hipMemcpy2DAsync(s->d_rows + first_row * s->ld, (size_t)s->ld * 4, rows_host, (size_t)s->dim * 4,
                             (size_t)s->dim * 4, n_rows, hipMemcpyHostToDevice, s->stream));
    int rc = launch_inv_norms(s, first_row, n_rows);
    if (rc) return rc;
    if ((rc = planes_rewrite(s, first_row, n_rows))) return rc;
    return update_min_pos_inv(s, first_row, n_rows);
}

uint64_t ott_store_len(const ott_store* s) { return s ? store_rows(s) : 0; }
uint32_t ott_store_dim(const ott_store* s) { return s ? s->dim : 0; }
int ott_store_device(const ott_store* s) { return s ? s->device : -1; }

int ott_store_set_chunk_size(ott_store* s, uint64_t chunk_size) {
    if (!s) return fail(OTT_ERR_INVALID, "ott_store_set_chunk_size: store is NULL");
    if (s->multi) return multi_set_chunk_size(s, chunk_size);
    s->chunk_size = chunk_size < 1 ? 1 : chunk_size;
    return OTT_OK;
}
int ott_store_set_base_offset(ott_store* s, uint64_t base) {
    if (!s) return fail(OTT_ERR_INVALID, "ott_store_set_base_offset: store is NULL");
    if (s->multi) return multi_set_base_offset(s, base);
    s->base_offset = base;
    return OTT_OK;
}
int ott_store_set_reduce_order(ott_store* s, uint32_t reduce) {
    if (!s) return fail(OTT_ERR_INVALID, "ott_store_set_reduce_order: store is NULL");
    if (reduce > OTT_REDUCE_SEQ4) return fail(OTT_ERR_INVALID, "ott_store_set_reduce_order: unknown order");
    if (s->multi) return multi_set_reduce_order(s, reduce);
    s->reduce = reduce;
    return OTT_OK;
}

int ott_store_read_rows(const ott_store* s, uint64_t first_row, uint64_t n_rows, float* out_host) {
    if (!s || !out_host) return fail(OTT_ERR_INVALID, "ott_store_read_rows: NULL argument");
    if (!s->multi && store_flush(const_cast<ott_store*>(s))) return OTT_ERR_HIP;
    if (first_row + n_rows > s->n) return fail(OTT_ERR_INVALID, "ott_store_read_rows: range exceeds store length");
    if (!n_rows) return OTT_OK;
    if (s->multi) return multi_read(s, false, first_row, n_rows, out_host);
    ott::host::SharedLock rd(const_cast<ott_store*>(s)->rw);
    if (first_row + n_rows > s->n) return fail(OTT_ERR_INVALID, "ott_store_read_rows: range exceeds store length");
    OTT_HIP(use_device(s));
    OTT_HIP(hipMemcpy2D(out_host, (size_t)s->dim * 4, s->d_rows + first_row * s->ld, (size_t)s->ld * 4, (size_t)s->dim * 4,
                        n_rows, hipMemcpyDeviceToHost));
    return OTT_OK;
}

int ott_store_read_inv_norms(const ott_store* s, uint64_t first_row, uint64_t n_rows, float* out_host) {
    if (!s || !out_host) return fail(OTT_ERR_INVALID, "ott_store_read_inv_norms: NULL argument");
    if (!s->multi && store_flush(const_cast<ott_store*>(s))) return OTT_ERR_HIP;
    if (first_row + n_rows > s->n) return fail(OTT_ERR_INVALID, "ott_store_read_inv_norms: range exceeds store length");
    if (!n_rows) return OTT_OK;
    if (s->multi) return multi_read(s, true, first_row, n_rows, out_host);
    ott::host::SharedLock rd(const_cast<ott_store*>(s)->rw);
    if (first_row + n_rows > s->n) return fail(OTT_ERR_INVALID, "ott_store_read_inv_norms: range exceeds store length");
    OTT_HIP(use_device(s));
    OTT_HIP(hipMemcpy(out_host, s->d_inv + first_row, n_rows * sizeof(float), hipMemcpyDeviceToHost));
    return OTT_OK;
}

int ott_store_sync(ott_store* s) {
    if (!s) return fail(OTT_ERR_INVALID, "ott_store_sync: store is NULL");
    if (s->multi) return multi_sync(s);
    OTT_HIP(use_device(s));
    OTT_HIP(hipStreamSynchronize(s->stream));
    return OTT_OK;
}

void* ott_store_stream(ott_store* s) { return s ? (void*)s->stream : nullptr; }

}
```

otters_amd/vec.py:

```python
from __future__ import annotations

import ctypes as C
import enum
import os
from dataclasses import dataclass
from typing import Optional, Sequence

import numpy as np

from . import _native as N
from ._native import OttersError


class Metric(enum.IntEnum):
    Cosine = 0
    Euclidean = 1
    DotProduct = 2
    Manhattan = 3


class TakeType(enum.IntEnum):
    Min = 0
    Max = 1

# ... 1303 lines not shown
        if idx.size and (idx.min() < 0 or idx.max() > 0xFFFFFFFF):
            raise OttersError("ott_store_set_sparse: an index is not a 32-bit unsigned integer")
        idx = np.ascontiguousarray(idx, dtype=np.uint32)
        val = np.ascontiguousarray(np.asarray(values).ravel(), dtype=np.float32)
        if ptr.size == 0 or idx.size != val.size or int(ptr[-1]) != idx.size:
            raise OttersError(f"ott_store_set_sparse: indptr ends at {int(ptr[-1]) if ptr.size else 0}, {idx.size} indices and {val.size} values were given")
        if not 0 <= int(vocab) <= 0xFFFFFFFF:
            raise OttersError(f"ott_store_set_sparse: vocab {vocab} is not in 1 .. OTT_SPARSE_MAX_VOCAB ({SPARSE_MAX_VOCAB}); remap the indices")
        N.check(N.lib().ott_store_set_sparse(self._handle(), N.ptr(ptr), N.ptr(idx), N.ptr(val), ptr.size - 1, int(vocab)))

    def set_sparse_rows(self, rows, vocab: int) -> None:
        self.set_sparse(*sparse_csr(rows), vocab)

    def clear_sparse(self) -> None:
        if self._h is not None:
            N.check(N.lib().ott_store_clear_sparse(self._h))

    def sparse_info(self) -> Optional[dict]:
        if self._h is None:
            return None
        vocab, nnz, padded, nbytes = C.c_uint32(0), C.c_uint64(0), C.c_uint64(0), C.c_uint64(0)
        N.check(N.lib().ott_store_sparse_info(self._h, C.byref(vocab), C.byref(nnz), C.byref(padded), C.byref(nbytes)))
        if vocab.value == 0:
            return None
        return {"vocab": int(vocab.value), "nnz": int(nnz.value), "padded_entries": int(padded.value), "bytes": int(nbytes.value)}

    def read_sparse(self, first: int = 0, n: Optional[int] = None):
        info = self.sparse_info()
        if info is None:
            raise OttersError("ott_store_read_sparse: no sparse rows are set (ott_store_set_sparse)")
        n = self._n - first if n is None else n
        ptr = np.zeros(max(n, 0) + 1, dtype=np.uint64)
        idx = np.zeros(max(info["nnz"], 1), dtype=np.uint32)
        val = np.zeros(max(info["nnz"], 1), dtype=np.float32)
        N.check(N.lib().ott_store_read_sparse(self._h, int(first), int(n), N.ptr(ptr), N.ptr(idx), N.ptr(val), info["nnz"]))
        nnz = int(ptr[-1])
        return ptr, idx[:nnz].copy(), val[:nnz].copy()

    def sparse_query(self, q) -> SparseQueryPlan:
        return SparseQueryPlan(self, q)

    def _run_sparse(self, rs: ResolvedSparse, chunk_mask: Optional[np.ndarray] = None, use_device_row_mask: bool = False):
        nq = int(rs.indptr.size - 1)
        cap = max(nq * min(rs.k, self._n), 1)
        out = np.empty(cap, dtype=N.HIT_DTYPE)
        d, keep = query_desc(rs, None, nq, Mode.PerQuery if nq > 1 else Mode.Merged, chunk_mask, use_device_row_mask)
        n_out, per, st = C.c_uint64(0), (C.c_uint64 * max(nq, 1))(), N.Stats()
        N.check(N.lib().ott_query_sparse(self._handle(), C.byref(d), N.ptr(rs.indptr), N.ptr(rs.indices) if rs.indices.size else None,
                                         N.ptr(rs.values) if rs.values.size else None, N.ptr(out), cap, C.byref(n_out), per, C.byref(st)))
        return out[: n_out.value].copy(), list(per)[:nq], st.as_dict()

    def shards(self):
        h = self._handle()
        out = []
        for g in range(N.lib().ott_store_shard_count(h)):
            dev, first, cnt = C.c_int(0), C.c_uint64(0), C.c_uint64(0)
            N.check(N.lib().ott_store_shard_info(h, g, C.byref(dev), C.byref(first), C.byref(cnt)))
            out.append((dev.value, first.value, cnt.value))
        return out

    def transport(self) -> str:
        return N.lib().ott_store_transport(self._handle()).decode()

    def set_chunk_size(self, chunk_size: int) -> None:
        self._chunk_size = max(int(chunk_size), 1)
        if self._h is not None:
            N.check(N.lib().ott_store_set_chunk_size(self._h, self._chunk_size))

    def set_base_offset(self, base: int) -> None:
        self._base_offset = int(base)
        if self._h is not None:
            N.check(N.lib().ott_store_set_base_offset(self._h, self._base_offset))

    def set_batch_image(self, enabled: bool) -> None:
        N.check(N.lib().ott_store_set_batch_image(self._handle(), 1 if enabled else 0))

    def prepare_batch(self) -> None:
        if self._n:
            N.check(N.lib().ott_store_prepare_batch(self._handle()))

    def batch_ready(self) -> bool:
        return bool(self._n) and bool(N.lib().ott_store_batch_ready(self._handle()))

    def set_option(self, name: str, value: int) -> None:
        self._options[name] = int(value)
        if self._h is not None:
            N.check(N.lib().ott_store_set_option(self._h, name.encode(), int(value)))

    def set_tie_order(self, order: str) -> None:
        self.set_option("tie_order", {"canonical": 0, "reference": 1, "reference_chunked": 2}[order])

    def set_reduce_order(self, order: int) -> None:
        self._reduce = int(order)
        if self._h is not None:
            N.check(N.lib().ott_store_set_reduce_order(self._h, self._reduce))

    def rows(self, first: int = 0, n: Optional[int] = None) -> np.ndarray:
        n = self._n - first if n is None else n
        out = np.empty((n, self.dim), dtype=np.float32)
        if n:
            N.check(N.lib().ott_store_read_rows(self._handle(), int(first), int(n), N.ptr(out)))
        return out

    def inv_norms(self, first: int = 0, n: Optional[int] = None) -> np.ndarray:
        n = self._n - first if n is None else n
        out = np.empty(n, dtype=np.float32)
        if n:
            N.check(N.lib().ott_store_read_inv_norms(self._handle(), int(first), int(n), N.ptr(out)))
        return out

    def len(self) -> int:
        return self._n

    def __len__(self) -> int:
        return self._n

    def is_empty(self) -> bool:
        return self._n == 0

    def query(self, queries, metric: Metric) -> VecQueryPlan:
        plan = VecQueryPlan()
        plan.query_vectors = QueryBatch(queries).queries
        plan.search_metric = Metric(metric)
        plan.vector_store = self
        return plan

    def _run(self, rq: ResolvedQuery, chunk_mask: Optional[np.ndarray] = None, use_device_row_mask: bool = False):
        nq = rq.queries.shape[0]
        ids = rq.row_ids
        if self._n == 0 and (ids is None or ids.size == 0):
            return np.zeros(0, dtype=N.HIT_DTYPE), [0] * nq, None
        perq = rq.mode == Mode.PerQuery
        rows = self._n if ids is None else int(np.unique(ids).size)
        pool = rows if perq else rows * nq
        k_eff = min(rq.k, pool)
        cap = max(k_eff * (nq if perq else 1), 1)
        if rq.grouped:
            cap = max(min(rq.k, self._n_groups) * nq, 1)
        if rq.group_size:
            cap = max(min(rq.k, self._n_groups) * nq * rq.group_size, 1)
        if rq.max_sim:
            cap = max(min(rq.k, self._n_groups), 1)
        if rq.group_list is not None:
            cap = max(min(rq.k, int(np.unique(rq.group_list).size)), 1)
        out = np.empty(cap, dtype=N.HIT_DTYPE)
        d, keep = query_desc(rq, rq.queries, nq, rq.mode, chunk_mask, use_device_row_mask)
        n_out, per, st = C.c_uint64(0), (C.c_uint64 * nq)(), N.Stats()
        if rq.group_list is not None:
            gl = rq.group_list
            N.check(N.lib().ott_query_maxsim_groups(self._handle(), C.byref(d), N.ptr(gl) if gl.size else None, gl.size, N.ptr(out), cap, C.byref(n_out), C.byref(st)))
            per[0] = n_out.value
        elif rq.max_sim:
            N.check(N.lib().ott_query_maxsim(self._handle(), C.byref(d), N.ptr(out), cap, C.byref(n_out), C.byref(st)))
            per[0] = n_out.value
        elif rq.group_size:
            gids = np.empty(cap, dtype=np.uint32)
            N.check(N.lib().ott_query_groups_top(self._handle(), C.byref(d), rq.group_size, N.ptr(out), cap, C.byref(n_out), per, N.ptr(gids), C.byref(st)))
            rq.group_of_hit = gids[: n_out.value].copy()
        elif rq.grouped:
            N.check(N.lib().ott_query_groups(self._handle(), C.byref(d), N.ptr(out), cap, C.byref(n_out), per, C.byref(st)))
        elif rq.mmr is not None:
            lam, fetch_k = rq.mmr
            vals = np.empty(cap, dtype=np.float32)
            N.check(N.lib().ott_query_mmr(self._handle(), C.byref(d), None if ids is None else N.ptr(ids), 0 if ids is None else ids.size, fetch_k,
                                          float(lam), N.ptr(out), cap, C.byref(n_out), per, N.ptr(vals), C.byref(st)))
            rq.mmr_values = vals[: n_out.value].copy()
# ... 95 lines not shown
```

Before: 37570 GB/s.

## Add int8 plane check to drop pruned-sweep candidates before exact f32 rescoring

Inside the gated head pruned sweep, queued candidates are first scored against the int8 plane with sdot4 using a quantized query held in shared memory. Candidates whose approximate score plus an error bound cannot beat the gate are dropped before the full f32 tail rescoring. The aim is to cut the f32 row reads spent on candidates that pass the sketch filter but cannot enter the top-k. In exchange it adds int8 plane loads, extra LDS, and a counter of finished rows. It only runs when the i8 plane is already built and the eps bound is valid.

```diff
diff --git a/bindings/rust/otters-hip-sys/src/lib.rs b/bindings/rust/otters-hip-sys/src/lib.rs
--- a/bindings/rust/otters-hip-sys/src/lib.rs
+++ b/bindings/rust/otters-hip-sys/src/lib.rs
@@ -187,6 +187,7 @@
     pub fn ott_store_set_batch_image(s: *mut ott_store, enabled: c_int) -> c_int;
     pub fn ott_store_prepare_batch(s: *mut ott_store) -> c_int;
     pub fn ott_store_batch_ready(s: *const ott_store) -> c_int;
+    pub fn ott_store_exact_finished(s: *const ott_store) -> u64;
     pub fn ott_store_set_option(s: *mut ott_store, name: *const c_char, value: i64) -> c_int;
     pub fn ott_store_set_base_offset(s: *mut ott_store, base: u64) -> c_int;
     pub fn ott_store_set_reduce_order(s: *mut ott_store, reduce: u32) -> c_int;
diff --git a/include/otters_hip.h b/include/otters_hip.h
--- a/include/otters_hip.h
+++ b/include/otters_hip.h
@@ -108,6 +108,7 @@
 int ott_store_set_batch_image(ott_store* s, int enabled);
 int ott_store_prepare_batch(ott_store* s);
 int ott_store_batch_ready(const ott_store* s);
+uint64_t ott_store_exact_finished(const ott_store* s);
 
 int ott_store_set_option(ott_store* s, const char* name, int64_t value);
 
diff --git a/otters_amd/_native.py b/otters_amd/_native.py
--- a/otters_amd/_native.py
+++ b/otters_amd/_native.py
@@ -148,6 +148,7 @@
         "ott_store_set_batch_image": (i32, [vp, i32]),
         "ott_store_prepare_batch": (i32, [vp]),
         "ott_store_batch_ready": (i32, [vp]),
+        "ott_store_exact_finished": (u64, [vp]),
         "ott_store_read_rows": (i32, [vp, u64, u64, vp]),
         "ott_store_read_inv_norms": (i32, [vp, u64, u64, vp]),
         "ott_store_add_column": (i32, [vp, u32, vp, vp, u64, vp]),
diff --git a/otters_amd/csrc/ott_api.hip b/otters_amd/csrc/ott_api.hip
--- a/otters_amd/csrc/ott_api.hip
+++ b/otters_amd/csrc/ott_api.hip
@@ -5,6 +5,7 @@
 
 #include "ott_internal.h"
 #include "ott_prune.h"
+#include "ott_i8_check.h"
 
 using namespace ott;
 
@@ -202,6 +203,19 @@
     PruneQuant qq{0, 0.0f, 0.0f, 0.0, 0};
     bool head = false;
     bool seed_est = false;
+    bool i8_check = false;
+    const int8_t* chk_plane = nullptr;
+    const float* chk_scale = nullptr;
+    float chk_qscale = 0.0f, chk_eps = 0.0f;
+    bool have_q_inv = false;
+    float q_inv = 0.0f;
+    float query_inv_norm() {
+        if (!have_q_inv) {
+            q_inv = host_inv_norm_exact(queries, s->dim);
+            have_q_inv = true;
+        }
+        return q_inv;
+    }
     ExactResult res{0, 0, 0};
     uint64_t* d_counts = nullptr;
     ott_hit* d_hits = nullptr;
@@ -236,6 +250,18 @@
     c.preB = tile_prefix(c.plB, 64);
     c.gridA = exact_grid(s, c.preA.back());
     c.gridB = exact_grid(s, c.preB.back());
+    if (head && c.x.E == 1 && s->opt.exact_i8_check != 0) {
+        I8CheckState ck{false, s->opt.exact_i8_check, false};
+        float rel = 0.0f;
+        if ((ck.plane_ready = i8_plane_peek(s, &c.chk_plane, &c.chk_scale, &rel))) {
+            const I8Query iq = i8_query_quant(c.queries, s->dim, c.d->metric == OTT_METRIC_COSINE, c.query_inv_norm(), nullptr);
+            const I8CheckEps e = i8_check_eps(s->dim, c.d->metric, s->opt.eps_scale_ppm, rel, iq, max_norm(s->min_pos_inv));
+            ck.eps_ok = e.ok;
+            c.chk_qscale = iq.s_q;
+            c.chk_eps = e.eps;
+        }
+        c.i8_check = prune_plan_i8_check(in, pp, head, ck);
+    }
 }
 
 int ensure_exact_result(ExactCtx& c) {
@@ -247,7 +273,7 @@
     c.res = exact_result_layout(c.groups, c.x.KS);
     char* res_dev = nullptr;
     if (c.fetch) {
-        if ((rc = s->h_hits.ensure(c.res.host_bytes))) return rc;
+        if ((rc = s->h_hits.ensure(c.res.host_bytes + 8))) return rc;
         void* mapped = nullptr;
         OTT_HIP(hipHostGetDevicePointer(&mapped, s->h_hits.p, 0));
         res_dev = (char*)mapped;
@@ -267,7 +293,7 @@
     c.p.perq = c.perq;
     c.p.list_stride = c.x.KS;
     c.p.small = c.x.variant;
-    if (c.x.lean) embed_exact_inputs(c.p, c.queries, (size_t)s->dim * 4, host_inv_norm_exact(c.queries, s->dim), c.pl, c.prefix);
+    if (c.x.lean) embed_exact_inputs(c.p, c.queries, (size_t)s->dim * 4, c.query_inv_norm(), c.pl, c.prefix);
 }
 
 ExactParams part_params(const ExactCtx& c, const RunPlan& sub, const std::vector<uint32_t>& pre, Cand* dst) {
@@ -288,9 +314,10 @@
     unsigned long long* tails_dev = nullptr;
     if (c.fetch) {
         if (!s->d_tails.p) {
-            if ((rc = s->d_tails.ensure(8))) return rc;
-            OTT_HIP(hipMemsetAsync(s->d_tails.p, 0, 8, s->stream));
+            if ((rc = s->d_tails.ensure(16))) return rc;
+            OTT_HIP(hipMemsetAsync(s->d_tails.p, 0, 16, s->stream));
             s->tails_seen = 0;
+            s->fin_seen = 0;
         }
         tails_dev = (unsigned long long*)s->d_tails.p;
     }
@@ -327,6 +354,13 @@
     sketch_inputs(pb);
     pb.prune_seed = seed_res;
     pb.prune_tails = tails_dev;
+    if (c.i8_check) {
+        pb.chk_plane = c.chk_plane;
+        pb.i8_scale = c.chk_scale;
+        pb.flag = s->d_flag;
+        pb.i8_qscale = c.chk_qscale;
+        pb.chk_eps = c.chk_eps;
+    }
     return launch_exact(s, pb, 1, c.x.E, c.gridB);
 }
 
@@ -357,13 +391,16 @@
     ott_store* s = c.s;
     const uint32_t KS = c.x.KS;
     char* hh = (char*)s->h_hits.p;
-    if (c.prune.c) OTT_HIP(hipMemcpyAsync(hh + c.res.bytes, s->d_tails.p, 8, hipMemcpyDeviceToHost, s->stream));
+    if (c.prune.c) OTT_HIP(hipMemcpyAsync(hh + c.res.bytes, s->d_tails.p, 16, hipMemcpyDeviceToHost, s->stream));
     OTT_HIP(hipStreamSynchronize(s->stream));
     if (c.prune.c) {
-        uint64_t total;
-        memcpy(&total, hh + c.res.bytes, 8);
-        st.rescored += total - s->tails_seen;
-        s->tails_seen = total;
+        uint64_t total[2];
+        memcpy(total, hh + c.res.bytes, 16);
+        const uint64_t passed = total[0] - s->tails_seen;
+        (s->owner ? s->owner : s)->exact_finished.fetch_add(c.i8_check ? total[1] - s->fin_seen : passed, std::memory_order_relaxed);
+        st.rescored += passed;
+        s->tails_seen = total[0];
+        s->fin_seen = total[1];
     }
     const uint64_t* counts = (const uint64_t*)hh;
     const ott_hit* hits = (const ott_hit*)(hh + c.res.cnt_pad);
diff --git a/otters_amd/csrc/ott_exact.hip b/otters_amd/csrc/ott_exact.hip
--- a/otters_amd/csrc/ott_exact.hip
+++ b/otters_amd/csrc/ott_exact.hip
@@ -2,6 +2,7 @@
 
 #include "ott_internal.h"
 #include "ott_prune.h"
+#include "ott_i8_check.h"
 #include "ott_exact_dev.h"
 
 namespace ott {
@@ -16,6 +17,8 @@
 constexpr int PQ_WORDS = 10;
 constexpr int QD_WORDS = (int)(OTT_QEMB_MAX / KC) * 12;
 constexpr int EXACT_SMEM_PRUNE = EXACT_SMEM + WAVES * PQ_CAP * PQ_WORDS * 4 + QD_WORDS * 4;
+constexpr int Q8_WORDS = (int)((OTT_QEMB_MAX + 127) / 128) * 32;
+constexpr int EXACT_SMEM_CHECK = EXACT_SMEM_PRUNE + Q8_WORDS * 4;
 #ifdef OTT_SK4_DECODE_F32
 constexpr bool SK4_INT = false;
 #else
@@ -48,8 +51,10 @@
 }
 
 
-template <int MK, int NQ, int E, bool PERQ, bool DUMP = false, bool SMALL = false, bool BLK = (E > 1), bool I8 = false, bool PRUNE = false, int SK = 0, bool SEED = false>
+template <int MK, int NQ, int E, bool PERQ, bool DUMP = false, bool SMALL = false, bool BLK = (E > 1), bool I8 = false, bool PRUNE = false, int SK = 0, bool SEED = false,
+          bool CHK = false>
 __global__ __launch_bounds__(SMALL ? 64 : 256) void exact_kernel(ExactParams p) {
+    static_assert(!CHK || (SK == 5 && !SEED && E == 1), "the int8 check is the gated head launch's, one list entry per lane");
     static_assert(!I8 || (NQ == 1 && MK == MK_DOT && !PERQ && !DUMP && !SMALL), "the int8 sweep takes one query, cosine / dot, merged");
     static_assert(!PRUNE || (NQ == 1 && MK == MK_DOT && !PERQ && !DUMP && !SMALL && !I8), "the pruned sweep takes one query, cosine / dot, merged");
     static_assert((SK == 0 || PRUNE) && (SK == 0 || SK == 1 || SK == 3 || SK == 4 || SK == 5), "the sketch is the pruned sweep's: none, one, three or four bits per dim (5: four with a head)");
@@ -122,6 +127,19 @@
     const int sw = (lane >> 1) & 7;
     const uint32_t nstages = (p.ld + KC - 1) / KC;
     [[maybe_unused]] uint32_t* qd = reinterpret_cast<uint32_t*>(smem + WAVES * STAGE_FLOATS + WAVES * PQ_CAP * PQ_WORDS);
+    [[maybe_unused]] uint32_t* q8w = qd + QD_WORDS;
+    [[maybe_unused]] const uint32_t ld8w = ((p.dim + 127u) & ~127u) >> 2;
+    if constexpr (CHK) {
+        const float pf8 = p.metric == OTT_METRIC_COSINE ? qinv[0] : 1.0f;
+        const float inv_sq = __fdiv_rn(1.0f, p.i8_qscale);
+        const uint32_t nw8 = ld8w < (uint32_t)Q8_WORDS ? ld8w : (uint32_t)Q8_WORDS;
+        for (uint32_t i = threadIdx.x; i < nw8; i += 64 * BW) {
+            float q4[4];
+#pragma unroll
+            for (int j = 0; j < 4; j++) q4[j] = (4 * i + j < p.dim) ? Q[4 * i + j] : 0.0f;
+            q8w[i] = i8_quant_word(q4, pf8, inv_sq);
+        }
+    }
     if constexpr (SK4 && SK4_INT) {
         const uint32_t nqs = nstages < (uint32_t)(QD_WORDS / 12) ? nstages : (uint32_t)(QD_WORDS / 12);
         for (uint32_t i = threadIdx.x; i < nqs * 4; i += 64 * BW) {
@@ -221,6 +239,71 @@
         pq_head = (pq_head + n) & (PQ_CAP - 1);
         pq_n -= n;
         tails_done += n;
+    };
+    [[maybe_unused]] uint32_t queued = 0;
+    [[maybe_unused]] auto pq_refine = [&](uint32_t n, uint32_t gate) __attribute__((always_inline)) -> uint32_t {
+        typedef uint32_t v4u __attribute__((ext_vector_type(4)));
+        wave_sync();
+        const bool valid = (uint32_t)lane < n;
+        const uint32_t e = (pq_head + (valid ? (uint32_t)lane : 0u)) & (PQ_CAP - 1);
+        const float vinv = pq[8 * PQ_CAP + e];
+        const uint32_t my_row = pq_row[e];
+        const float sv = p.i8_scale[my_row];
+        const uint32_t fl = p.flag[my_row];
+        const uint32_t* rp[8];
+#pragma unroll
+        for (int m = 0; m < 8; m++) {
+            const uint32_t i = 8 * m + lrow;
+            rp[m] = reinterpret_cast<const uint32_t*>(p.chk_plane) + (uint64_t)pq_row[(pq_head + (i < n ? i : 0u)) & (PQ_CAP - 1)] * ld8w + (uint32_t)lslot * 4;
+        }
+        v4f R[8];
+        auto load_stage = [&](uint32_t s) {
+#pragma unroll
+            for (int m = 0; m < 8; m++) R[m] = __builtin_nontemporal_load(reinterpret_cast<const v4f*>(rp[m] + s * KC));
+        };
+        const uint32_t nst8 = ld8w / KC;
+        int iacc[2] = {0, 0};
+        load_stage(0);
+        for (uint32_t s = 0; s < nst8; s++) {
+#pragma unroll
+            for (int m = 0; m < 8; m++) {
+                const int row = 8 * m + lrow;
+                const v4f v = R[m];
+                *reinterpret_cast<float4*>(st + row * KC + ((lslot ^ ((row >> 1) & 7)) << 2)) = make_float4(v.x, v.y, v.z, v.w);
+            }
+            wave_sync();
+            if (s + 1 < nst8) load_stage(s + 1);
+#pragma unroll
+            for (int j = 0; j < KC / 8; j++) {
+                const float4 a = *reinterpret_cast<const float4*>(st + lane * KC + (((2 * j) ^ sw) << 2));
+                const float4 b = *reinterpret_cast<const float4*>(st + lane * KC + (((2 * j + 1) ^ sw) << 2));
+                const int x[8] = {__float_as_int(a.x), __float_as_int(a.y), __float_as_int(a.z), __float_as_int(a.w),
+                                  __float_as_int(b.x), __float_as_int(b.y), __float_as_int(b.z), __float_as_int(b.w)};
+                const v4u* qp = reinterpret_cast<const v4u*>(q8w + s * KC + 8 * j);
+                const v4u q0 = qp[0], q1 = qp[1];
+#pragma unroll
+                for (int l = 0; l < 4; l++) {
+                    iacc[0] = __builtin_amdgcn_sdot4(x[l], (int)q0[l], iacc[0], false);
+                    iacc[1] = __builtin_amdgcn_sdot4(x[4 + l], (int)q1[l], iacc[1], false);
+                }
+            }
+            wave_sync();
+        }
+        const float approx = i8_approx_score(iacc[0] + iacc[1], i8_row_factor(p.metric == OTT_METRIC_COSINE, vinv, sv, p.i8_qscale));
+        const bool stay = valid && !i8_check_drops(approx, p.chk_eps, take_max, gate, (fl & 5u) != 0);
+        const uint64_t km = __ballot(stay);
+        if (stay) {
+            const uint32_t at = (pq_head + (uint32_t)__popcll(km & ((1ull << lane) - 1ull))) & (PQ_CAP - 1);
+            pq[8 * PQ_CAP + at] = vinv;
+            pq_row[at] = my_row;
+        }
+        return (uint32_t)__popcll(km);
+    };
+    [[maybe_unused]] auto pq_drain = [&](uint32_t n, uint32_t gate) __attribute__((always_inline)) {
+        const uint32_t stay = gate != 0 ? pq_refine(n, gate) : n;
+        if (stay) pq_finish(stay);
+        pq_head = (pq_head + (n - stay)) & (PQ_CAP - 1);
+        pq_n -= n - stay;
     };
 
     if constexpr (HD) {
@@ -371,8 +454,10 @@
                 pq_row[at] = (uint32_t)my_row;
             }
             pq_n += (uint32_t)__popcll(km);
+            if constexpr (CHK) queued += (uint32_t)__popcll(km);
             if (!SEED && pq_n >= 64) {
-                pq_finish(64);
+                if constexpr (CHK) pq_drain(64, gate);
+                else pq_finish(64);
                 if (pf) {
                     load_line(row0n, cntn, 0);
                     load_head(row0n, cntn);
@@ -803,7 +888,16 @@
         }
     }
 
-    if constexpr (PRUNE) {
+    if constexpr (CHK) {
+        if (pq_n) {
+            const uint32_t own = (uint32_t)(tk[0] >> 32);
+            pq_drain(pq_n, own > theta ? own : theta);
+        }
+        if (p.prune_tails != nullptr && lane == 0) {
+            if (queued != 0) atomicAdd(p.prune_tails, (unsigned long long)queued);
+            if (tails_done != 0) atomicAdd(p.prune_tails + 1, (unsigned long long)tails_done);
+        }
+    } else if constexpr (PRUNE) {
         if (pq_n) pq_finish(pq_n);
         if (p.prune_tails != nullptr && tails_done != 0 && lane == 0) atomicAdd(p.prune_tails, (unsigned long long)tails_done);
     }
@@ -1557,15 +1651,16 @@
     return (int)(want < cap ? want : cap);
 }
 
-template <int E, bool BLK, int SK, bool SEED = false>
+template <int E, bool BLK, int SK, bool SEED = false, bool CHK = false>
 static int launch_prune(ott_store* s, const ExactParams& p, int grid) {
-    auto kern = exact_kernel<MK_DOT, 1, E, false, false, false, BLK, false, true, SK, SEED>;
+    auto kern = exact_kernel<MK_DOT, 1, E, false, false, false, BLK, false, true, SK, SEED, CHK>;
+    constexpr int smem = CHK ? EXACT_SMEM_CHECK : EXACT_SMEM_PRUNE;
     static std::atomic<uint64_t> attr_set{0};
     if (ott::attr_needed(attr_set, s->device)) {
-        OTT_HIP(hipFuncSetAttribute((const void*)kern, hipFuncAttributeMaxDynamicSharedMemorySize, EXACT_SMEM_PRUNE));
+        OTT_HIP(hipFuncSetAttribute((const void*)kern, hipFuncAttributeMaxDynamicSharedMemorySize, smem));
         ott::attr_done(attr_set, s->device);
     }
-    hipLaunchKernelGGL(kern, dim3(grid), dim3(256), EXACT_SMEM_PRUNE, s->stream, p);
+    hipLaunchKernelGGL(kern, dim3(grid), dim3(256), smem, s->stream, p);
     OTT_HIP(hipGetLastError());
     return OTT_OK;
 }
@@ -1576,6 +1671,13 @@
         if (p.seed_est != 0) return launch_prune<E, BLK, 5, true>(s, p, grid);
     }
     if (p.seed_est != 0) return fail(OTT_ERR_INVALID, "launch_exact: the estimate pass needs the integer decode and a list of k <= 64");
+    if constexpr (SK4_INT && E == 1) {
+        if (p.chk_plane != nullptr) {
+            if (p.i8_scale == nullptr || p.flag == nullptr || p.dim > OTT_QEMB_MAX) return fail(OTT_ERR_INVALID, "launch_exact: the int8 check needs the plane's scales and flags and a query of up to 896 dims");
+            return launch_prune<E, BLK, 5, false, true>(s, p, grid);
+        }
+    }
+    if (p.chk_plane != nullptr) return fail(OTT_ERR_INVALID, "launch_exact: the int8 check needs the integer decode and a list of k <= 64");
     if constexpr (SK4_INT && E <= 4) return launch_prune<E, BLK, 5>(s, p, grid);
     else return fail(OTT_ERR_INVALID, "launch_exact: the head form needs the integer decode and a list of k <= 256");
 }
diff --git a/otters_amd/csrc/ott_exact_plan.h b/otters_amd/csrc/ott_exact_plan.h
--- a/otters_amd/csrc/ott_exact_plan.h
+++ b/otters_amd/csrc/ott_exact_plan.h
@@ -124,6 +124,17 @@
 inline bool prune_plan_head(const PruneIn& in, const PrunePlan& pp, bool quant_ok, const HeadState& hd) {
     return prune_plan_needs_quant(in, pp) && quant_ok && hd.present && hd.covers && hd.option != 0 && in.E <= 4;
 }
+#ifndef OTT_X_I8_CHECK
+#define OTT_X_I8_CHECK 1
+#endif
+struct I8CheckState {
+    bool plane_ready;
+    int option;
+    bool eps_ok;
+};
+inline bool prune_plan_i8_check(const PruneIn& in, const PrunePlan& pp, bool head, const I8CheckState& ck) {
+    return OTT_X_I8_CHECK != 0 && pp.c != 0 && head && in.E == 1 && ck.plane_ready && ck.option != 0 && ck.eps_ok;
+}
 #ifndef OTT_X_SEED_EST
 #define OTT_X_SEED_EST 1
 #endif
diff --git a/otters_amd/csrc/ott_i8_check.h b/otters_amd/csrc/ott_i8_check.h
--- /dev/null
+++ b/otters_amd/csrc/ott_i8_check.h
@@ -0,0 +1,93 @@
+#pragma once
+#include <math.h>
+#include <stdint.h>
+
+#include "ott_mfma_plan.h"
+#include "ott_prune.h"
+
+namespace ott {
+
+OTT_PRUNE_HD inline int32_t i8_quant_elem(float q, float pf, float inv_sq) {
+    const float xe = q * pf;
+    float t = xe * inv_sq;
+    t = t == t ? (t < -127.0f ? -127.0f : t > 127.0f ? 127.0f : t) : 0.0f;
+    const float biased = t + 12582912.0f;
+    return (int32_t)(biased - 12582912.0f);
+}
+OTT_PRUNE_HD inline uint32_t i8_quant_word(const float q4[4], float pf, float inv_sq) {
+    uint32_t w = 0;
+    for (int j = 0; j < 4; j++) w |= ((uint32_t)i8_quant_elem(q4[j], pf, inv_sq) & 0xFFu) << (8 * j);
+    return w;
+}
+
+struct I8Query {
+    float pf;
+    float s_q;
+    float inv_sq;
+    float qnorm;
+    float qrel;
+    bool regular;
+};
+inline I8Query i8_query_quant(const float* q, uint32_t dim, bool cosine, float q_inv, int8_t* q8) {
+    double n2[4] = {0.0, 0.0, 0.0, 0.0};
+    float amax = 0.0f;
+    for (uint32_t i = 0; i < dim; i++) {
+        n2[i & 3] += (double)q[i] * q[i];
+        const float a = fabsf(q[i]);
+        if (a > amax) amax = a;
+    }
+    I8Query x;
+    x.qnorm = (float)(sqrt((n2[0] + n2[1]) + (n2[2] + n2[3])) * (1.0 + 1e-6));
+    x.regular = query_regular(x.qnorm);
+    x.pf = cosine ? q_inv : 1.0f;
+    const float e_max = amax * x.pf;
+    x.s_q = (e_max > 0.0f && e_max < __builtin_inff()) ? e_max / 127.0f : 1.0f;
+    x.inv_sq = 1.0f / x.s_q;
+    double se4[4] = {0.0, 0.0, 0.0, 0.0}, sx4[4] = {0.0, 0.0, 0.0, 0.0};
+    for (uint32_t i = 0; i < dim; i++) {
+        const int32_t t = i8_quant_elem(q[i], x.pf, x.inv_sq);
+        if (q8) q8[i] = (int8_t)t;
+        const float xe = q[i] * x.pf;
+        const double df = (double)xe - (double)x.s_q * (double)t;
+        se4[i & 3] += df * df;
+        sx4[i & 3] += (double)xe * (double)xe;
+    }
+    const double se = (se4[0] + se4[1]) + (se4[2] + se4[3]), sx = (sx4[0] + sx4[1]) + (sx4[2] + sx4[3]);
+    x.qrel = sx > 0.0 ? (float)(sqrt(se / sx) * 1.0001) : 0.0f;
+    if (!(x.qrel <= 1.0f)) x.qrel = 1.0f;
+    return x;
+}
+
+struct I8CheckEps {
+    bool ok;
+    float eps;
+};
+inline I8CheckEps i8_check_eps(uint32_t dim, uint32_t metric, int eps_scale_ppm, float plane_rel, const I8Query& x, float vn_max) {
+    const I8CheckEps off{false, 0.0f};
+    if (metric != OTT_METRIC_COSINE && metric != OTT_METRIC_DOT) return off;
+    const ErrorModel em = error_model(2, false, dim, metric, true, eps_scale_ppm, plane_rel);
+    if (!x.regular || !(x.qrel <= em.qrel_cap) || !(plane_rel >= 0.0f)) return off;
+    double e = (double)em.eps_c + (double)em.eps_r + 1.001 * (double)x.qrel * (double)em.eps_scale;
+    if (metric == OTT_METRIC_DOT) e *= (double)x.qnorm * (double)vn_max;
+    const float eps = prune_f32_up(e * (1.0 + 1e-6));
+    if (!(eps >= 0.0f && eps < __builtin_inff())) return off;
+    return I8CheckEps{true, eps};
+}
+
+OTT_PRUNE_HD inline float i8_row_factor(bool cosine, float vinv, float s_v, float s_q) { return ((cosine ? vinv : 1.0f) * s_v) * s_q; }
+OTT_PRUNE_HD inline float i8_approx_score(int32_t idot, float row_factor) { return (float)idot * row_factor; }
+
+OTT_PRUNE_HD inline float i8_check_edge(float approx, float eps, bool take_max) {
+    return take_max ? prune_next_up(approx + eps) : prune_next_down(approx - eps);
+}
+OTT_PRUNE_HD inline uint32_t i8_check_ord(float f, bool take_max) {
+    const uint32_t b = prune_f2u(f);
+    const uint32_t k = (b & 0x80000000u) ? ~b : (b | 0x80000000u);
+    return take_max ? k : ~k;
+}
+OTT_PRUNE_HD inline bool i8_check_drops(float approx, float eps, bool take_max, uint32_t gate, bool outside) {
+    const float b = i8_check_edge(approx, eps, take_max);
+    return !outside && approx - approx == 0.0f && b == b && i8_check_ord(b, take_max) < gate;
+}
+
+}
diff --git a/otters_amd/csrc/ott_internal.h b/otters_amd/csrc/ott_internal.h
--- a/otters_amd/csrc/ott_internal.h
+++ b/otters_amd/csrc/ott_internal.h
@@ -84,6 +84,7 @@
     int exact_sketch = -1;
     int exact_sketch_bits = 4;
     int exact_sketch_head = -1;
+    int exact_i8_check = -1;
     int force_fallback = 0;
     bool mfma_f32 = false;
     bool no_hi_pass = false;
@@ -206,6 +207,8 @@
     ott::DevBuf d_prune;
     ott::DevBuf d_tails;
     uint64_t tails_seen = 0;
+    uint64_t fin_seen = 0;
+    std::atomic<uint64_t> exact_finished{0};
     ott::DevBuf d_minpos;
     ott::DevBuf m_Q, m_qinv, m_qnorm, m_tau, m_cntA, m_cntB, m_candA, m_candB, m_over, m_out, m_outcnt, m_uncert, m_prefix;
     ott::DevBuf l_keysA, l_keysB, l_qA, l_qB, l_tmp, l_cursor, l_hist, l_gate;
@@ -297,6 +300,7 @@
 int multi_prepare_batch(ott_store* ms);
 int multi_sync(ott_store* ms);
 int multi_batch_ready(ott_store* ms);
+uint64_t multi_exact_finished(ott_store* ms);
 int multi_add_column(ott_store* ms, uint32_t dtype, const void* values_host, const uint64_t* nulls, uint64_t n, uint32_t* out_column_id);
 int multi_eval_row_mask(ott_store* ms, const ott_leaf* leaves, uint32_t n_leaves, uint32_t n_clauses, uint64_t* out_host);
 int multi_zone_stats(ott_store* ms, uint32_t column, uint64_t chunk_size, void* out_min, void* out_max, uint64_t* out_non_null);
@@ -345,6 +349,7 @@
 PlaneSnapshot plane_snapshot(const ott_store* s);
 int ensure_i8_plane(ott_store* ctx, const int8_t** img_out, const float** scale_out, float* rel_max_out);
 bool i8_plane_ready(ott_store* ctx);
+bool i8_plane_peek(ott_store* ctx, const int8_t** img_out, const float** scale_out, float* rel_max_out);
 int launch_i8_rows(hipStream_t stream, const float* rows, uint32_t ld, uint32_t dim, uint32_t ld8, uint64_t first, uint64_t n, int8_t* out,
                    const float* pre, float common_scale, float* scale_out, float* rel_out, uint32_t* rel_max, const uint8_t* flag, float rel_flag,
                    uint8_t* flag_rw, int n_cu);
@@ -434,6 +439,8 @@
     float prune_qscale, prune_qinv_scale;
     int32_t prune_qsum;
     uint32_t seed_est, seed_keep;
+    const int8_t* chk_plane;
+    float chk_eps;
     float qemb[OTT_QEMB_MAX];
 };
 static_assert(sizeof(ExactParams) <= 4096, "kernel arguments are limited to 4 KB");
diff --git a/otters_amd/csrc/ott_mfma.hip b/otters_amd/csrc/ott_mfma.hip
--- a/otters_amd/csrc/ott_mfma.hip
+++ b/otters_amd/csrc/ott_mfma.hip
@@ -11,6 +11,7 @@
 #include <vector>
 
 #include "ott_internal.h"
+#include "ott_i8_check.h"
 
 namespace ott {
 
@@ -1562,35 +1563,14 @@
 
     const float* q = d->queries;
     const float q_inv = host_inv_norm_exact(q, dim);
-    double n2 = 0.0;
-    float amax = 0.0f;
-    for (uint32_t i = 0; i < dim; i++) {
-        n2 += (double)q[i] * q[i];
-        amax = fmaxf(amax, fabsf(q[i]));
-    }
-    const float qnorm = (float)(sqrt(n2) * (1.0 + 1e-6));
+    int8_t q8[OTT_QEMB_MAX * 4];
+    memset(q8, 0, ld8);
+    const I8Query iq = i8_query_quant(q, dim, cosine, q_inv, q8);
+    const float qnorm = iq.qnorm, s_q = iq.s_q, qrel = iq.qrel;
     out.assign(1, {});
     uncertified.assign(1, 1u);
     st.path_used = OTT_PATH_MFMA;
-    if (!query_regular(qnorm)) return OTT_OK;
-    const float pf = cosine ? q_inv : 1.0f;
-    const float e_max = amax * pf;
-    const float s_q = (e_max > 0.0f && e_max < __builtin_inff()) ? e_max / 127.0f : 1.0f;
-    const float inv_sq = 1.0f / s_q;
-    int8_t q8[OTT_QEMB_MAX * 4];
-    memset(q8, 0, ld8);
-    double se = 0.0, sx = 0.0;
-    for (uint32_t i = 0; i < dim; i++) {
-        const float xe = q[i] * pf;
-        float t = rintf(xe * inv_sq);
-        t = t == t ? fminf(fmaxf(t, -127.0f), 127.0f) : 0.0f;
-        q8[i] = (int8_t)(int)t;
-        const double df = (double)xe - (double)s_q * (double)(int)t;
-        se += df * df;
-        sx += (double)xe * (double)xe;
-    }
-    float qrel = sx > 0.0 ? (float)(sqrt(se / sx) * 1.0001) : 0.0f;
-    if (!(qrel <= 1.0f)) qrel = 1.0f;
+    if (!iq.regular) return OTT_OK;
 
     const ErrorModel em = error_model(level, false, dim, d->metric, true, s->opt.eps_scale_ppm, i8_rel);
     const float mx_norm = max_norm(s->min_pos_inv);
diff --git a/otters_amd/csrc/ott_multi.hip b/otters_amd/csrc/ott_multi.hip
--- a/otters_amd/csrc/ott_multi.hip
+++ b/otters_amd/csrc/ott_multi.hip
@@ -1030,6 +1030,13 @@
     return ms->n ? 1 : 0;
 }
 
+uint64_t multi_exact_finished(ott_store* ms) {
+    ott::host::SharedLock rd(ms->rw);
+    uint64_t total = 0;
+    for (ott_store* s : ms->multi->shards) total += ott_store_exact_finished(s);
+    return total;
+}
+
 int multi_sync(ott_store* ms) {
     for (ott_store* s : ms->multi->shards) {
         const int rc = ott_store_sync(s);
diff --git a/otters_amd/csrc/ott_planes.hip b/otters_amd/csrc/ott_planes.hip
--- a/otters_amd/csrc/ott_planes.hip
+++ b/otters_amd/csrc/ott_planes.hip
@@ -466,6 +466,16 @@
 }
 bool hi_plane_ready(ott_store* ctx) { return plane_ready(owner_of(ctx), owner_of(ctx)->planes.hi); }
 bool i8_plane_ready(ott_store* ctx) { return plane_ready(owner_of(ctx), owner_of(ctx)->planes.i8); }
+bool i8_plane_peek(ott_store* ctx, const int8_t** img_out, const float** scale_out, float* rel_max_out) {
+    ott_store* own = owner_of(ctx);
+    const PlaneSet& p = own->planes;
+    std::lock_guard<std::mutex> g(own->planes.mu);
+    if (!(p.i8.d != nullptr && !p.i8.off && !p.split.off && own->n != 0 && p.i8.rows == own->n && p.d_i8_scale != nullptr)) return false;
+    *img_out = (const int8_t*)p.i8.d;
+    *scale_out = p.d_i8_scale;
+    *rel_max_out = p.i8.rel;
+    return true;
+}
 
 bool first_plane_ready(ott_store* ctx) {
     ott_store* own = owner_of(ctx);
diff --git a/otters_amd/csrc/ott_store.hip b/otters_amd/csrc/ott_store.hip
--- a/otters_amd/csrc/ott_store.hip
+++ b/otters_amd/csrc/ott_store.hip
@@ -29,18 +29,18 @@
                              {"mfma_f32", 0},        {"no_hi_pass", 0},      {"no_batch_image", 0},       {"force_fallback", 2},      {"eps_scale_ppm", 2},
                              {"multi_fake_distinct", 0}, {"exact_prune", 1},            {"exact_sketch", 1},
                              {"id_gather", 1},       {"exact_sketch_bits", 2},   {"group_gather", 1},         {"exact_sketch_head", 1},
-                             {"masks_sweep", 2},     {"fuse_device", 1},         {"sparse_table", 1},
+                             {"masks_sweep", 2},     {"fuse_device", 1},         {"sparse_table", 1},         {"exact_i8_check", 1},
 #ifdef OTT_MFMA_DEBUG_BUILD
                              {"mfma_wg", 2},         {"mfma_growth", 2},     {"mfma_debug", 0},           {"mfma_abl", 2},            {"hi_tmin", 2},
                              {"mfma_no_dense", 0},   {"mfma_coop", 1},       {"mfma_spec", 1},            {"large_k_pre", 1},         {"merge_walk", 0},
                              {"merge_rank1", 1},     {"maxsim_fold", 1},
 #endif
 };
-static_assert(sizeof(kOptNames) / sizeof(kOptNames[0]) <= 25
+static_assert(sizeof(kOptNames) / sizeof(kOptNames[0]) <= 26
 #ifdef OTT_MFMA_DEBUG_BUILD
                                                             + 12
 #endif
-              , "the product library's option table stays at twenty-five entries");
+              , "the product library's option table stays at twenty-six entries");
 }
 
 int option_set(Options& o, const char* name, long long v) {
@@ -77,6 +77,7 @@
     if (n == "exact_sketch") return tri(o.exact_sketch);
     if (n == "exact_sketch_bits") { if (v != 1 && v != 3 && v != 4) return -1; o.exact_sketch_bits = (int)v; return 0; }
     if (n == "exact_sketch_head") return tri(o.exact_sketch_head);
+    if (n == "exact_i8_check") return tri(o.exact_i8_check);
     if (n == "id_gather") return tri(o.id_gather);
     if (n == "group_gather") return tri(o.group_gather);
     if (n == "fuse_device") return tri(o.fuse_device);
@@ -1094,6 +1095,11 @@
 }
 
 uint64_t ott_store_len(const ott_store* s) { return s ? store_rows(s) : 0; }
+uint64_t ott_store_exact_finished(const ott_store* s) {
+    if (!s) return 0;
+    if (s->multi) return multi_exact_finished(const_cast<ott_store*>(s));
+    return s->exact_finished.load(std::memory_order_relaxed);
+}
 uint32_t ott_store_dim(const ott_store* s) { return s ? s->dim : 0; }
 int ott_store_device(const ott_store* s) { return s ? s->device : -1; }
 
diff --git a/otters_amd/vec.py b/otters_amd/vec.py
--- a/otters_amd/vec.py
+++ b/otters_amd/vec.py
@@ -1409,6 +1409,9 @@
     def batch_ready(self) -> bool:
         return bool(self._n) and bool(N.lib().ott_store_batch_ready(self._handle()))
 
+    def exact_finished(self) -> int:
+        return int(N.lib().ott_store_exact_finished(self._handle()))
+
     def set_option(self, name: str, value: int) -> None:
         self._options[name] = int(value)
         if self._h is not None:
```

Result: faster. 39650 GB/s, median of 6 (+5.5%).
